# crowdbotp/socialways

Hardware: AMD Instinct MI355X
Metric: GAN train steps/sec (256 scenes x 8 agents x 8+12 T per GPU step; fp32; social block on) (higher is better)
Workload: dtype f32; 1 GPU; m1: 256 scenes x 8 agents x (8 obs + 12 pred) per GPU step = reference --batch-size 2048; use_social=True, n_unrolling_steps=1, info loss on; full=False, global_batch_scenes=256, parallelism=dp1, steps_per_graph_launch=32, settle_steps=992, rehearsal_regions=2, step_alg_bytes=5527040, inputs=z drawn on the host every step

## Files before the change

### include/socialways_hip.h

```cpp
#ifndef SOCIALWAYS_HIP_H
#define SOCIALWAYS_HIP_H
#include <stddef.h>
#include <stdint.h>

#ifdef __cplusplus
extern "C" {
#endif

#define SW_OK 0
#define SW_EARG -1
#define SW_ESHAPE -2
#define SW_EHIP -3

#define SW_H 64
#define SW_Z 32

enum { SW_GRP_ENC = 0, SW_GRP_EMB = 1, SW_GRP_ATT = 2, SW_GRP_DEC = 3, SW_GRP_DISC = 4 };

enum {
  SW_WS_GSAVE = 0,
  SW_WS_GDELTA = 1,
  SW_WS_DSAVE = 2,
  SW_WS_DDELTA = 3,
  SW_WS_WGRAD = 4,
// ... 33 lines not shown
                       const int* big_blocks , int NB, float* wh_ws, float* ml , void* stream);
int sw_social_pool_fwd_aux(const float* obsv, int To, const float* h, const int* scene_off, int S, int B, int Amax,
                           const float* emb_w, const float* att_w, float* S_out, float* attn, const int* big_blocks,
                           int NB, float* wh_ws, float* ml, const float* aux_src, float* aux_dst, long long aux_n,
                           void* stream);
int sw_social_features(const float* x4_last , int B, float* feat , void* stream);
int sw_embed_features(const float* feat , long long R, const float* emb_w, float* out ,
                      void* stream);
int sw_attention_pool_dense(const float* f , const float* h , const int* scene_off,
                            int S, int B, const float* att_w, float* S_out , void* stream);
int sw_rows_gemm(const float* x, int ldx, const float* w, int w_rs, int w_cs, const float* bias, long long R, int K, int N,
                 float* y, int ldy, int accumulate, void* stream);
int sw_linear_wgrad(const float* delta, int ldd, const float* act, int lda, int R, int N, int K, float* dW, int ldw,
                    float* db, float* wgrad_ws, int accumulate, void* stream);
int sw_embed_features_bwd(const float* feat , long long R, const float* emb_w, const float* dout ,
                          float* rows, float* dfeat, void* stream);
int sw_attention_dense_fwd(const float* f, const float* h, const float* wh, const int* scene_off, int S, int B, float* attn,
                           float* S_out, void* stream);
int sw_attention_dense_bwd(const float* f, const float* h, const float* wh, const float* attn, const float* dS,
                           const int* scene_off, int S, int B, float* dsig, float* df, float* dwh, float* dh, void* stream);
int sw_enc_lstm_wgrad(const float* enc_w, const float* act, const float* x4s, const float* h0, const float* dgates, int B,
                      int T, float* d_enc_w, float* wgrad_ws, float* tmp, void* stream);
int sw_dec_fc_wgrad(const float* dec_w, const float* gsave, const float* gdelta, const float* h, const float* s,
                    const float* z, int B, int To, float* d_dec_w, float* wgrad_ws, float* tmp, void* stream);

int sw_dec_fc_dz(const float* dec_w, const float* gdelta, int B, int To, float* dz, void* stream);

typedef struct sw_wgrad_batch sw_wgrad_batch;
sw_wgrad_batch* sw_wgrad_batch_new(void);
void sw_wgrad_batch_free(sw_wgrad_batch* h);

int sw_social_pool_bwd(const float* obsv, int To, const float* h, const int* scene_off,
                       const long long* pair_off, int S, int B, int Amax, long long P,
                       const float* emb_w, const float* att_w, const float* attn, const float* dS,
                       float* dh, float* d_emb_w, float* d_att_w, float* pair_ws, float* wgrad_ws,
                       const int* big_blocks , int NB, const float* wh_ws, const float* ml,
                       const float* S_pool, float* big_part_ws,
                       sw_wgrad_batch* defer ,
                       void* stream);

int sw_dec_rollout_fwd(const float* obsv , int To, const float* z ,
                       const float* S_pool , const float* hT, const float* cT,
                       const float* enc_w, const float* dec_w, int B, int Tp,
                       float* pred4 , float* h_end, float* c_end ,
                       float* gsave ,
                       const float* gt , float inv_ss, float* ade_part ,
                       void* stream);
int sw_dec_rollout_fwd_aux(const float* obsv, int To, const float* z, const float* S_pool, const float* hT,
                           const float* cT, const float* enc_w, const float* dec_w, int B, int Tp, float* pred4,
                           float* h_end, float* c_end, float* gsave, const float* gt, float inv_ss, float* ade_part,
                           const float* d_w , float* dsave , void* stream);
int sw_dec_sample_fwd(const float* obsv , int To, const float* z ,
                      const float* S_pool , const float* hT, const float* cT ,
                      const float* enc_w, const float* dec_w, int B, int K, int Tp, float* pred4, const float* gt ,
                      float inv_ss, float* err, void* stream);
int sw_sample_reduce(const float* err , int B, int K, float* per_agent , int* best ,
                     void* stream);
int sw_sample_rank(const float* score , const float* err , const int* best ,
                   int B, int K, int M, int* order , float* per_agent , void* stream);
int sw_scene_clearance(const float* pos, int pstride, const float* start , int sstride, const int* scene_off,
                       int S, int B, int K, int Tp, float inv_ss, float* clear , void* stream);
int sw_scene_reduce(const float* err , const float* clear , const int* scene_off, int S, int B,
                    int K, float coll_dist, float* per_scene , int* best , void* stream);
int sw_sample_nms(const float* pos, int pstride, const float* score , const int* scene_off , int S,
                  int B, int K, int Tp, int M, int metric, float inv_ss, float radius, const float* err ,
                  const int* best , int* order , int* count , float* weight ,
                  int* assign , float* per_row , void* stream);
int sw_dec_rollout_bwd(const float* dpred4 , const float* enc_w, const float* dec_w,
                       const float* gsave, int B, int To, int Tp, float* gdelta,
                       float* dhT, float* dcT, float* dS_pool , void* stream);
int sw_dec_rollout_bwd_aux(const float* dpred4, const float* enc_w, const float* dec_w, const float* gsave, int B,
                           int To, int Tp, float* gdelta, float* dhT, float* dcT, float* dS_pool,
                           const float* aux_src, float* aux_dst, const float* aux_mask, long long aux_n, void* stream);
int sw_gen_wgrad(const float* enc_w, const float* dec_w, const float* gsave, const float* gdelta, const float* z,
                 const float* S_pool, int B, int To, int Tp, float* d_enc_w, float* d_dec_w, int part,
                 float* wgrad_ws, float* tmp ,
                 sw_wgrad_batch* pending ,
                 void* stream);
int sw_gen_wgrad_adam(const float* enc_w, const float* dec_w, const float* gsave, const float* gdelta,
                      const float* z, const float* S_pool, int B, int To, int Tp, float* d_enc_w, float* d_dec_w,
                      float* wgrad_ws, float* tmp , sw_wgrad_batch* pending , float* adam_w,
                      float* adam_m, float* adam_v, const float* adam_g, long long adam_n, const float* adam_step,
                      double lr, double beta1, double beta2, double eps, void* stream);

int sw_disc_fwd(const float* obsv, int To, int x_mode, const float* const* pred4 ,
                int nb, const float* d_w, int B, int Tp, float* const* label ,
                float* const* code , float* dsave ,
                int save_lstm ,
                float* w_snapshot ,
                void* stream);
int sw_disc_bwd(const float* d_w, const float* dsave, const float* const* dlabel,
                const float* const* dcode, int nb, int B, int To, int Tp, float* ddelta,
                float* d_d_w, float* const* dpred4, float* wgrad_ws, void* stream);

int sw_disc_bwd_gan(const float* d_w, const float* dsave, const float* const* label,
                    const float* const* code, const float* targets, int t0, int t1, const float* z ,
                    float g_label, float g_code, int nb, int B, int To, int Tp, float* ddelta,
                    float* d_d_w, float* const* dpred4, float* wgrad_ws,
                    float* loss_part ,
                    void* stream);
int sw_disc_bwd_gan_adam(const float* d_w, const float* dsave, const float* const* label, const float* const* code,
                         const float* targets, int t0, int t1, const float* z, float g_label, float g_code, int nb,
                         int B, int To, int Tp, float* ddelta, float* d_d_w, float* const* dpred4, float* wgrad_ws,
                         float* loss_part, float* adam_w, float* adam_m, float* adam_v, const float* adam_step,
                         double lr, double beta1, double beta2, double eps, void* stream);

int sw_disc_update_supported(const float* d_w, int B, int To, int Tp);
int sw_disc_update(const float* obsv , int To, const float* const* pred4 , const float* d_w, int B,
                   int Tp, float* const* label, float* const* code, float* dsave, int obs_pre, float* w_snapshot ,
                   const float* targets, int t0, int t1, const float* z, float g_label, float g_code, float* ddelta,
                   float* d_d_w, float* wgrad_ws, float* loss_part , float* adam_w , float* adam_m,
                   float* adam_v, const float* adam_step, double lr, double beta1, double beta2, double eps, void* stream);

int sw_disc_dpred_supported(int Tp);
int sw_disc_dpred(const float* obsv, int To, int x_mode, const float* pred4 , const float* d_w, int B, int Tp,
                  const float* targets, int t_idx, const float* z , float g_label, float g_code,
                  float* dpred4 , float* label , float* code ,
                  float* loss_part , void* stream);

int sw_disc_score(const float* obsv, int To, int x_mode, const float* pred4 , const float* d_w, int B, int K,
                  int Tp, float* score , float* code , void* stream);

int sw_disc_score_ragged(const float* obsv, int To, int x_mode, const int* obs_len ,
                         const float* pred4 , const float* d_w, int B, int K, int Tp, float* score ,
                         float* code , void* stream);

int sw_disc_fwd_ragged(const float* obsv, int To, int x_mode, const int* obs_len ,
                       const float* const* pred4 , int nb, const float* d_w, int B, int Tp,
                       float* const* label , float* const* code , float* dsave ,
                       int save_lstm , float* w_snapshot , void* stream);
int sw_disc_dpred_ragged(const float* obsv, int To, int x_mode, const int* obs_len ,
                         const float* pred4 , const float* d_w, int B, int Tp, const float* targets, int t_idx,
                         const float* z , float g_label, float g_code, float* dpred4 ,
                         float* label , float* code , float* loss_part ,
                         void* stream);

#define SW_RED_BLOCKS 64
int sw_gan_loss(const float* label_a, const float* targets , int ia,
                const float* code_a, const float* z , const float* label_b, int ib, int B,
                float g_label, float g_code, float* out_sums , float* dlabel_a, float* dcode_a,
                float* dlabel_b, float* dcode_b, float* scratch , void* stream);

int sw_l2_grad(const float* pred4_hat , const float* gt , int B, int Tp, int row0, int row1,
               float scale, float* dpred4 , void* stream);

int sw_variety_grad(const float* pred4_hat_K , const float* gt , int K, int B, int Tp,
                    float scale, float* dpred4_K , int* kmin, float* l2min, void* stream);

int sw_traj_dist(const float* a , const float* b , int Na, int Nb, int nPed, int T,
                 int t0, float* D , void* stream);

#define SW_STAGE_HEADER 8
int sw_stage_step(const float* slot, int B, int To, int Tp, float* obsv_dst , float* pred_dst ,
                  float* pred4_dst , float* targets_dst , float* z_dst ,
                  float* steps_dst , int n_d_updates, void* stream);

int sw_gen_image_floats(void);
int sw_gen_images(const float* enc_w, const float* dec_w, const float* emb_w , const float* att_w ,
                  float* img, void* stream);
int sw_stage_step_img(const float* slot, int B, int To, int Tp, float* obsv_dst, float* pred_dst, float* pred4_dst,
                      float* targets_dst, float* z_dst, float* steps_dst, int n_d_updates, const float* enc_w,
                      const float* dec_w, const float* emb_w , const float* att_w , float* img,
                      const float* d_w , float* d_img , const int* d_tab , void* stream);
int sw_stage_step_zdev(const float* slot, int B, int To, int Tp, float* obsv_dst, float* pred_dst, float* pred4_dst,
                       float* targets_dst, float* z_dst, float* steps_dst, int n_d_updates, const float* enc_w,
                       const float* dec_w, const float* emb_w, const float* att_w, float* img, const float* d_w, float* d_img,
// ... 95 lines not shown
```

### socialways_amd/_lib.py

```python
import ctypes
import os

import torch

_HERE = os.path.dirname(os.path.abspath(__file__))
LIB_PATH = os.environ.get("SW_LIB_PATH") or os.path.join(_HERE, "libsocialways_hip.so")

GRP_ENC, GRP_EMB, GRP_ATT, GRP_DEC, GRP_DISC = 0, 1, 2, 3, 4
WS_GSAVE, WS_GDELTA, WS_DSAVE, WS_DDELTA, WS_WGRAD, WS_PAIRS = 0, 1, 2, 3, 4, 5
AMAX = 64
RED_BLOCKS = 64

_vp, _i, _f, _ll = ctypes.c_void_p, ctypes.c_int, ctypes.c_float, ctypes.c_longlong

PROTOTYPES = {
    "sw_version": (_i, []),
    "sw_last_error": (ctypes.c_char_p, []),
    "sw_param_count": (_i, [_i, _i]),
    "sw_param_offset": (_i, [_i, _i, _i]),
    "sw_param_tensors": (_i, [_i]),
    "sw_workspace_floats": (ctypes.c_size_t, [_i, _i, _i, _i, _i, _ll]),
    "sw_traj_4d": (_i, [_vp, _vp, _i, _i, _i, _vp, _vp, _vp]),
    "sw_enc_lstm_fwd": (_i, [_vp, _i, _vp, _vp, _vp, _i, _i, _vp, _vp, _vp, _vp, _vp, _i, _vp]),
    "sw_enc_lstm_fwd_aux": (_i, [_vp, _i, _vp, _vp, _vp, _i, _i, _vp, _vp, _vp, _vp, _vp, _i, _vp, _vp, _ll, _vp]),
    "sw_enc_lstm_fwd_ragged": (_i, [_vp, _i, _vp, _vp, _i, _i, _vp, _vp, _vp]),
    "sw_enc_lstm_fwd_ragged_save": (_i, [_vp, _i, _vp, _vp, _i, _i, _vp, _vp, _vp, _vp, _vp]),
    "sw_enc_lstm_bwd": (_i, [_vp, _vp, _vp, _vp, _vp, _vp, _i, _i, _i, _vp, _vp, _vp, _vp]),
    "sw_social_pool_fwd": (_i, [_vp, _i, _vp, _vp, _i, _i, _i, _vp, _vp, _vp, _vp, _vp, _i, _vp, _vp, _vp]),
    "sw_social_pool_fwd_aux": (_i, [_vp, _i, _vp, _vp, _i, _i, _i, _vp, _vp, _vp, _vp, _vp, _i, _vp, _vp, _vp, _vp, _ll, _vp]),
    "sw_social_features": (_i, [_vp, _i, _vp, _vp]),
    "sw_embed_features": (_i, [_vp, _ll, _vp, _vp, _vp]),
    "sw_attention_pool_dense": (_i, [_vp, _vp, _vp, _i, _i, _vp, _vp, _vp]),
    "sw_social_pool_bwd": (_i, [_vp, _i, _vp, _vp, _vp, _i, _i, _i, _ll, _vp, _vp, _vp, _vp, _vp, _vp, _vp,
                                _vp, _vp, _vp, _i, _vp, _vp, _vp, _vp, _vp, _vp]),
    "sw_dec_rollout_fwd": (_i, [_vp, _i, _vp, _vp, _vp, _vp, _vp, _vp, _i, _i, _vp, _vp, _vp, _vp, _vp, _f, _vp, _vp]),
    "sw_dec_rollout_fwd_aux": (_i, [_vp, _i, _vp, _vp, _vp, _vp, _vp, _vp, _i, _i, _vp, _vp, _vp, _vp, _vp, _f, _vp, _vp, _vp, _vp]),
    "sw_dec_sample_fwd": (_i, [_vp, _i, _vp, _vp, _vp, _vp, _vp, _vp, _i, _i, _i, _vp, _vp, _f, _vp, _vp]),
    "sw_sample_reduce": (_i, [_vp, _i, _i, _vp, _vp, _vp]),
    "sw_sample_rank": (_i, [_vp, _vp, _vp, _i, _i, _i, _vp, _vp, _vp]),
    "sw_scene_clearance": (_i, [_vp, _i, _vp, _i, _vp, _i, _i, _i, _i, _f, _vp, _vp]),
    "sw_scene_reduce": (_i, [_vp, _vp, _vp, _i, _i, _i, _f, _vp, _vp, _vp]),
    "sw_sample_nms": (_i, [_vp, _i, _vp, _vp, _i, _i, _i, _i, _i, _i, _f, _f, _vp, _vp, _vp, _vp, _vp, _vp, _vp, _vp]),
    "sw_dec_rollout_bwd": (_i, [_vp, _vp, _vp, _vp, _i, _i, _i, _vp, _vp, _vp, _vp, _vp]),
    "sw_dec_rollout_bwd_aux": (_i, [_vp, _vp, _vp, _vp, _i, _i, _i, _vp, _vp, _vp, _vp, _vp, _vp, _vp, _ll, _vp]),
    "sw_gen_wgrad": (_i, [_vp, _vp, _vp, _vp, _vp, _vp, _i, _i, _i, _vp, _vp, _i, _vp, _vp, _vp, _vp]),
    "sw_gen_wgrad_adam": (_i, [_vp, _vp, _vp, _vp, _vp, _vp, _i, _i, _i, _vp, _vp, _vp, _vp, _vp, _vp, _vp, _vp, _vp,
                               ctypes.c_longlong, _vp, ctypes.c_double, ctypes.c_double, ctypes.c_double, ctypes.c_double, _vp]),
    "sw_enc_lstm_bwd_aux": (_i, [_vp, _vp, _vp, _vp, _vp, _vp, _i, _i, _i, _vp, _vp, _vp, _vp, _vp, _vp, _ll, _vp]),
    "sw_dec_rollout_bwd_dfuse": (_i, [_vp, _vp, _vp, _vp, _i, _vp, _f, _f, _vp, _vp, _vp, _vp, _vp, _i, _i, _i, _vp, _vp, _vp, _vp,
                                      _vp]),
    "sw_rows_gemm": (_i, [_vp, _i, _vp, _i, _i, _vp, ctypes.c_longlong, _i, _i, _vp, _i, _i, _vp]),
    "sw_linear_wgrad": (_i, [_vp, _i, _vp, _i, _i, _i, _i, _vp, _i, _vp, _vp, _i, _vp]),
    "sw_embed_features_bwd": (_i, [_vp, ctypes.c_longlong, _vp, _vp, _vp, _vp, _vp]),
    "sw_attention_dense_fwd": (_i, [_vp, _vp, _vp, _vp, _i, _i, _vp, _vp, _vp]),
    "sw_attention_dense_bwd": (_i, [_vp, _vp, _vp, _vp, _vp, _vp, _i, _i, _vp, _vp, _vp, _vp, _vp]),
    "sw_enc_lstm_wgrad": (_i, [_vp, _vp, _vp, _vp, _vp, _i, _i, _vp, _vp, _vp, _vp]),
    "sw_dec_fc_dz": (_i, [_vp, _vp, _i, _i, _vp, _vp]),
    "sw_dec_fc_wgrad": (_i, [_vp, _vp, _vp, _vp, _vp, _vp, _i, _i, _vp, _vp, _vp, _vp]),
    "sw_wgrad_batch_new": (_vp, []),
    "sw_wgrad_batch_free": (None, [_vp]),
    "sw_disc_fwd": (_i, [_vp, _i, _i, _vp, _i, _vp, _i, _i, _vp, _vp, _vp, _i, _vp, _vp]),
    "sw_disc_bwd": (_i, [_vp, _vp, _vp, _vp, _i, _i, _i, _i, _vp, _vp, _vp, _vp, _vp]),
    "sw_disc_bwd_gan": (_i, [_vp, _vp, _vp, _vp, _vp, _i, _i, _vp, _f, _f, _i, _i, _i, _i, _vp, _vp, _vp, _vp, _vp, _vp]),
    "sw_disc_bwd_gan_adam": (_i, [_vp, _vp, _vp, _vp, _vp, _i, _i, _vp, _f, _f, _i, _i, _i, _i, _vp, _vp, _vp, _vp, _vp,
                                  _vp, _vp, _vp, _vp, ctypes.c_double, ctypes.c_double, ctypes.c_double, ctypes.c_double, _vp]),
    "sw_disc_update_supported": (_i, [_vp, _i, _i, _i]),
    "sw_disc_dpred_supported": (_i, [_i]),
    "sw_disc_update": (_i, [_vp, _i, _vp, _vp, _i, _i, _vp, _vp, _vp, _i, _vp, _vp, _i, _i, _vp, _f, _f, _vp, _vp, _vp, _vp,
                            _vp, _vp, _vp, _vp, ctypes.c_double, ctypes.c_double, ctypes.c_double, ctypes.c_double, _vp]),
    "sw_disc_dpred": (_i, [_vp, _i, _i, _vp, _vp, _i, _i, _vp, _i, _vp, _f, _f, _vp, _vp, _vp, _vp, _vp]),
    "sw_disc_score": (_i, [_vp, _i, _i, _vp, _vp, _i, _i, _i, _vp, _vp, _vp]),
    "sw_disc_score_ragged": (_i, [_vp, _i, _i, _vp, _vp, _vp, _i, _i, _i, _vp, _vp, _vp]),
    "sw_disc_fwd_ragged": (_i, [_vp, _i, _i, _vp, _vp, _i, _vp, _i, _i, _vp, _vp, _vp, _i, _vp, _vp]),
    "sw_disc_dpred_ragged": (_i, [_vp, _i, _i, _vp, _vp, _vp, _i, _i, _vp, _i, _vp, _f, _f, _vp, _vp, _vp, _vp, _vp]),
    "sw_gan_loss": (_i, [_vp, _vp, _i, _vp, _vp, _vp, _i, _i, _f, _f, _vp, _vp, _vp, _vp, _vp, _vp, _vp]),
    "sw_l2_grad": (_i, [_vp, _vp, _i, _i, _i, _i, _f, _vp, _vp]),
    "sw_variety_grad": (_i, [_vp, _vp, _i, _i, _i, _f, _vp, _vp, _vp, _vp]),
    "sw_traj_dist": (_i, [_vp, _vp, _i, _i, _i, _i, _i, _vp, _vp]),
    "sw_stage_step": (_i, [_vp, _i, _i, _i, _vp, _vp, _vp, _vp, _vp, _vp, _i, _vp]),
    "sw_gen_image_floats": (_i, []),
    "sw_gen_images": (_i, [_vp, _vp, _vp, _vp, _vp, _vp]),
    "sw_stage_step_img": (_i, [_vp, _i, _i, _i, _vp, _vp, _vp, _vp, _vp, _vp, _i, _vp, _vp, _vp, _vp, _vp, _vp, _vp, _vp, _vp]),
    "sw_stage_step_zdev": (_i, [_vp, _i, _i, _i, _vp, _vp, _vp, _vp, _vp, _vp, _i, _vp, _vp, _vp, _vp, _vp, _vp, _vp, _vp, _i, _vp]),
    "sw_disc_image_floats": (_i, [_i]),
    "sw_disc_image_table": (_i, [_i, _vp]),
    "sw_disc_images": (_i, [_vp, _vp, _vp, _i, _vp]),
    "sw_ade_fde": (_i, [_vp, _vp, _i, _i, _f, _vp, _vp, _vp]),
    "sw_lstm_point_fwd": (_i, [_vp, _vp, _i, _i, _vp, _vp, _vp, _vp]),
    "sw_lstm_point_bwd": (_i, [_vp, _vp, _vp, _vp, _vp, _i, _i, _vp, _vp, _vp]),
    "sw_act_fwd": (_i, [_vp, _ll, _i, _vp, _vp]),
    "sw_act_bwd": (_i, [_vp, _vp, _ll, _i, _vp, _vp]),
    "sw_sqdiff": (_i, [_vp, _i, _vp, _i, _vp, _i, _ll, _i, _f, _vp, _vp, _i, _vp]),
    "sw_pair_features": (_i, [_vp, _vp, _vp, _i, _vp, _vp]),
    "sw_attn_pairs_fwd": (_i, [_vp, _vp, _vp, _vp, _vp, _i, _i, _i, _i, _vp, _vp, _vp]),
    "sw_attn_pairs_bwd": (_i, [_vp, _vp, _vp, _vp, _vp, _vp, _vp, _i, _i, _i, _i, _vp, _vp, _vp, _vp, _vp]),
    "sw_adam_packed": (_i, [_vp, _vp, _vp, _vp, _ll, _vp, ctypes.c_double, ctypes.c_double, ctypes.c_double,
                            ctypes.c_double, _i, _vp]),
    "sw_wide_gemm": (_i, [_vp, _ll, _i, _vp, _ll, _i, _vp, _vp, _i, _vp, _i, _ll, _i, _i, _vp, _i, _i, _vp]),
    "sw_wide_lstm_fwd": (_i, [_vp, _i, _vp, _i, _vp, _vp, _vp, _vp, _vp, _i, _i, _vp, _vp, _vp, _i, _vp, _i, _vp]),
    "sw_wide_lstm_bwd": (_i, [_vp, _i, _vp, _i, _vp, _vp, _vp, _vp, _vp, _vp, _i, _i, _vp, _vp, _vp]),
    "sw_wide_out_fwd": (_i, [_vp, _i, _vp, _vp, _vp, _i, _vp, _i, _vp, _vp]),
    "sw_wide_out_bwd": (_i, [_vp, _i, _vp, _vp, _i, _vp, _i, _vp, _vp, _i, _vp, _vp]),
    "sw_wide_sum_steps": (_i, [_vp, _ll, _i, _i, _ll, _i, _vp, _i, _vp]),
    "sw_wide_wgrad": (_i, [_vp, _i, _vp, _vp]),
    "sw_wide_transpose": (_i, [_vp, _vp, _i, _i, _vp, _vp]),
    "sw_wide_dec_loop_supported": (_i, [_i]),
    "sw_wide_dec_loop_fwd": (_i, [_vp] * 13 + [_i] + [_vp] * 9 + [_i, _i, _i, _i, _vp]),
    "sw_wide_dec_loop_bwd": (_i, [_vp] * 18 + [_i, _i, _i, _i, _vp]),
    "sw_wide_disc_heads_supported": (_i, [_i, _i, _i]),
    "sw_wide_disc_heads_fwd": (_i, [_vp, _vp]),
    "sw_wide_disc_heads_bwd": (_i, [_vp, _vp]),
    "sw_wide_opimage": (_i, [_vp, _vp, _i, _ll, _vp, _vp]),
    "sw_wide_lstm_seq_supported": (_i, [_i]),
    "sw_wide_lstm_seq_fwd": (_i, [_vp, _vp, _vp, _vp, _vp, _i, _i, _i, _vp, _vp, _vp, _vp, _i, _vp]),
    "sw_wide_lstm_seq_bwd": (_i, [_vp, _i, _vp, _i, _vp, _vp, _vp, _vp, _vp, _i, _i, _i, _vp, _vp]),
    "sw_comm_bytes": (_ll, [_i, _ll]),
    "sw_comm_alloc": (_i, [_ll, _vp]),
    "sw_comm_free": (_i, [_vp]),
    "sw_comm_ipc_export": (_i, [_vp, _vp]),
    "sw_comm_ipc_import": (_i, [_vp, _vp]),
    "sw_comm_ipc_close": (_i, [_vp]),
    "sw_comm_status": (_i, [_vp, _vp]),
    "sw_allreduce_direct": (_i, [_vp, _i, _i, _ll, _vp, _ll, _vp]),
    "sw_allreduce_direct_adam": (_i, [_vp, _i, _i, _ll, _vp, _ll, _vp, _vp, _vp, _vp, ctypes.c_double, ctypes.c_double,
                                      ctypes.c_double, ctypes.c_double, _i, _vp]),
    "sw_noise_uniform": (_i, [ctypes.c_ulonglong, _i, ctypes.c_uint, _i, ctypes.c_uint, _i, ctypes.c_uint, _i, _i, _i, _vp, _vp]),
}

DEBUG_PROTOTYPES = {
    "sw_kernel_timing": (_i, [_i]),
# ... 81 lines not shown
```

### socialways_amd/csrc/sw_lstm.hip

```cpp
#include "../../include/socialways_hip.h"
#include "sw_lstm_dev.h"
#include <cstdlib>

template <int XMODE, bool ACT, bool Y, bool X4S>
__global__ __launch_bounds__(SW_THREADS) void enc_lstm_fwd_kernel(
    const float* __restrict__ x, const float* __restrict__ enc_w, const float* __restrict__ h0,
    const float* __restrict__ c0, int B, int T, float* __restrict__ hT, float* __restrict__ cT,
    float* __restrict__ y, float* __restrict__ act, float* __restrict__ x4s, int t0, const float* __restrict__ aux_src,
    float* __restrict__ aux_dst, long long aux_n, const float* __restrict__ gimg) {
  const int tiles = (B + SW_TILE - 1) / SW_TILE;
  const int extra = (int)gridDim.x - tiles;
  if ((int)blockIdx.x < extra) {
    const long long n4 = aux_n >> 2, stride = (long long)extra * SW_THREADS;
    long long i = (long long)blockIdx.x * SW_THREADS + threadIdx.x;
    for (; i + 3 * stride < n4; i += 4 * stride) {
      const f32x4 v0 = ld4(aux_src + 4 * i), v1 = ld4(aux_src + 4 * (i + stride));
      const f32x4 v2 = ld4(aux_src + 4 * (i + 2 * stride)), v3 = ld4(aux_src + 4 * (i + 3 * stride));
      st4(aux_dst + 4 * i, v0);
      st4(aux_dst + 4 * (i + stride), v1);
      st4(aux_dst + 4 * (i + 2 * stride), v2);
      st4(aux_dst + 4 * (i + 3 * stride), v3);
    }
    for (; i < n4; i += stride) st4(aux_dst + 4 * i, ld4(aux_src + 4 * i));
    return;
  }
  constexpr int HS = ACT ? SW_ALD : SW_HLD, HO = ACT ? 320 : 0;
  __shared__ __attribute__((aligned(16))) float hbuf[2][SW_TILE * HS];
  __shared__ __attribute__((aligned(16))) float wx_lds[256 * 4];
  __shared__ __attribute__((aligned(16))) float bx_lds[256];
  const int lane = sw_lane(), wave = sw_wave(), ln = lane & 15, lg = lane >> 4;
  const int u0 = wave * 16;
  const int a0 = ((int)blockIdx.x - extra) * SW_TILE;
  const int b = min(a0 + ln, B - 1);
  LstmW W;
  if (gimg) {
    lstm_load_img(W, gimg, wave, lane);
  } else {
    lstm_load_whh(W, enc_w + swp::ENC_WHH, u0, ln, lg);
    lstm_prep_rows(enc_w + swp::ENC_EMB_W, enc_w + swp::ENC_EMB_B, enc_w + swp::ENC_WIH, enc_w + swp::ENC_BIH,
                   enc_w + swp::ENC_BHH, true, wx_lds, bx_lds);
  }
  f32x4 c = {0.f, 0.f, 0.f, 0.f}, h = {0.f, 0.f, 0.f, 0.f};
  if (h0) h = ld4(h0 + (size_t)b * 64 + u0 + 4 * lg);
  if (c0) c = ld4(c0 + (size_t)b * 64 + u0 + 4 * lg);
  st4(&hbuf[0][ln * HS + HO + u0 + 4 * lg], h);
  sw_barrier();
  if (!gimg) lstm_load_wx(W, wx_lds, bx_lds, u0, ln, lg);

  float xa, xq = 0.f;
  auto load_x = [&](int t) {
    if constexpr (XMODE == 0) obs_x4_load(x, b, t, T, lg, xa, xq);
    else xa = x[((size_t)b * T + t) * 4 + lg];
  };
  load_x(0);
  asm volatile("" : "+v"(xa), "+v"(xq));
  float* yrow = Y ? y + (size_t)b * T * 64 + u0 + 4 * lg : nullptr;
  float* xrow = X4S ? x4s + ((size_t)t0 * B + b) * 4 + lg : nullptr;
  auto step = [&](int t, auto hp) {
    const float xb = XMODE == 0 ? xa - (lg >= 2 ? xq : 0.f) : xa;
    load_x(min(t + 1, T - 1));
    f32x4 gate[4];
    lstm_cell<decltype(hp)::value>(W, xb, &hbuf[t & 1][ln * HS + HO + 4 * lg], gate, c, h);
    if constexpr (ACT) lstm_put_act_tile(hbuf[(t + 1) & 1], gate, c, h, ln, lg, u0);
    else st4(&hbuf[(t + 1) & 1][ln * HS + u0 + 4 * lg], h);
    if constexpr (Y) {
      st4(yrow, h);
      yrow += 64;
    }
    if constexpr (X4S) {
      *xrow = xb;
      xrow += (size_t)B * 4;
    }
    sw_barrier();
    if constexpr (ACT) lstm_store_act_tile(hbuf[(t + 1) & 1], act + (size_t)(t0 + t) * B * 384, a0, B, wave, lane);
    asm volatile("" : "+v"(xa), "+v"(xq));
  };
  if (h0) step(0, std::true_type{});
  else step(0, std::false_type{});
  for (int t = 1; t < T; ++t) step(t, std::true_type{});
  st4(hT + (size_t)b * 64 + u0 + 4 * lg, h);
  st4(cT + (size_t)b * 64 + u0 + 4 * lg, c);
}

__global__ __launch_bounds__(512) void enc_lstm_fwd8_kernel(
    const float* __restrict__ x, const float* __restrict__ h0, const float* __restrict__ c0, int B, int T,
    float* __restrict__ hT, float* __restrict__ cT, float* __restrict__ act, float* __restrict__ x4s, int t0,
    const float* __restrict__ aux_src, float* __restrict__ aux_dst, long long aux_n, const float* __restrict__ gimg) {
  const int tiles = (B + SW_TILE - 1) / SW_TILE;
  const int extra = (int)gridDim.x - tiles;
  if ((int)blockIdx.x < extra) {
    const long long n4 = aux_n >> 2, stride = (long long)extra * 512;
    long long i = (long long)blockIdx.x * 512 + threadIdx.x;
    for (; i + stride < n4; i += 2 * stride) {
      const f32x4 v0 = ld4(aux_src + 4 * i), v1 = ld4(aux_src + 4 * (i + stride));
      st4(aux_dst + 4 * i, v0);
      st4(aux_dst + 4 * (i + stride), v1);
    }
    for (; i < n4; i += stride) st4(aux_dst + 4 * i, ld4(aux_src + 4 * i));
    return;
  }
  __shared__ __attribute__((aligned(16))) float hbuf[2][SW_TILE * SW_ALD];
  const int lane = sw_lane(), wave = sw_wave(), ln = lane & 15, lg = lane >> 4;
  const int ub = 8 * wave + 2 * lg;
  const int a0 = ((int)blockIdx.x - extra) * SW_TILE;
  const int b = min(a0 + ln, B - 1);
  f32x4 whh[2][4], bias[2];
  float wx[2];
#pragma unroll
  for (int tl = 0; tl < 2; ++tl) {
#pragma unroll
    for (int j = 0; j < 4; ++j) whh[tl][j] = ld4(gimg + swimg::OP_WHH8 + ((((size_t)wave * 2 + tl) * 4 + j) * 64 + lane) * 4);
    const int rowA = (2 * tl + ((ln & 3) >> 1)) * 64 + 8 * wave + 2 * (ln >> 2) + (ln & 1);
    wx[tl] = gimg[swimg::WX + rowA * 4 + lg];
#pragma unroll
    for (int r = 0; r < 4; ++r) bias[tl][r] = gimg[swimg::BX + (2 * tl + (r >> 1)) * 64 + ub + (r & 1)];
  }
  float2 c = {0.f, 0.f}, h = {0.f, 0.f};
  if (h0) h = *reinterpret_cast<const float2*>(h0 + (size_t)b * 64 + ub);
  if (c0) c = *reinterpret_cast<const float2*>(c0 + (size_t)b * 64 + ub);
  *reinterpret_cast<float2*>(&hbuf[0][ln * SW_ALD + 320 + ub]) = h;
  sw_barrier();
  float xa, xq = 0.f;
  obs_x4_load(x, b, 0, T, lg, xa, xq);
  asm volatile("" : "+v"(xa), "+v"(xq));
  float* xrow = x4s + ((size_t)t0 * B + b) * 4 + lg;
  auto step = [&](int t, auto hp) {
    const float xb = xa - (lg >= 2 ? xq : 0.f);
    obs_x4_load(x, b, min(t + 1, T - 1), T, lg, xa, xq);
    f32x4 acc0 = SW_MFMA(wx[0], xb, bias[0]), acc1 = SW_MFMA(wx[1], xb, bias[1]);
    if constexpr (decltype(hp)::value) {
      const float* hrow = &hbuf[t & 1][ln * SW_ALD + 320 + 4 * lg];
      f32x4 bq[4];
#pragma unroll
      for (int j = 0; j < 4; ++j) bq[j] = ld4(hrow + 16 * j);
#pragma unroll
      for (int j = 0; j < 4; ++j)
#pragma unroll
        for (int r = 0; r < 4; ++r) {
          acc0 = SW_MFMA(whh[0][j][r], bq[j][r], acc0);
          acc1 = SW_MFMA(whh[1][j][r], bq[j][r], acc1);
        }
    }
    float2 gi, gf, gg, go;
#pragma unroll
    for (int e = 0; e < 2; ++e) {
      const float i_ = sw_sigmoid(acc0[e]), f_ = sw_sigmoid(acc0[2 + e]), g_ = sw_tanh(acc1[e]), o_ = sw_sigmoid(acc1[2 + e]);
      const float cp = e ? c.y : c.x;
      const float cn = fmaf(f_, cp, i_ * g_);
      const float hn = o_ * sw_tanh(cn);
      if (e) { gi.y = i_; gf.y = f_; gg.y = g_; go.y = o_; c.y = cn; h.y = hn; }
      else   { gi.x = i_; gf.x = f_; gg.x = g_; go.x = o_; c.x = cn; h.x = hn; }
    }
    float* row = &hbuf[(t + 1) & 1][ln * SW_ALD + ub];
    *reinterpret_cast<float2*>(row) = gi;
    *reinterpret_cast<float2*>(row + 64) = gf;
    *reinterpret_cast<float2*>(row + 128) = gg;
    *reinterpret_cast<float2*>(row + 192) = go;
    *reinterpret_cast<float2*>(row + 256) = c;
    *reinterpret_cast<float2*>(row + 320) = h;
    *xrow = xb;
    xrow += (size_t)B * 4;
    sw_barrier();
    {
      float* rows_t = act + (size_t)(t0 + t) * B * 384;
#pragma unroll
      for (int k = 0; k < 3; ++k) {
        const int f = k * 512 + (int)threadIdx.x, a = f / 96, c4 = f - a * 96;
        const f32x4 v = ld4(&hbuf[(t + 1) & 1][a * SW_ALD + 4 * c4]);
        st4g(rows_t + (size_t)min(a0 + a, B - 1) * 384 + 4 * c4, v);
      }
    }
    asm volatile("" : "+v"(xa), "+v"(xq));
  };
  if (h0) step(0, std::true_type{});
  else step(0, std::false_type{});
  for (int t = 1; t < T; ++t) step(t, std::true_type{});
  *reinterpret_cast<float2*>(hT + (size_t)b * 64 + ub) = h;
  *reinterpret_cast<float2*>(cT + (size_t)b * 64 + ub) = c;
}

template <bool DY>
__global__ __launch_bounds__(SW_THREADS) void enc_lstm_bwd_kernel(
    const float* __restrict__ whh, const float* __restrict__ act, const float* __restrict__ c0,
    const float* __restrict__ dhT, const float* __restrict__ dcT, const float* __restrict__ dy, int B, int T,
    int t0, float* __restrict__ dgates, float* __restrict__ dh0, float* __restrict__ dc0, const float* __restrict__ gimg,
    const float* __restrict__ aux_src, float* __restrict__ aux_dst, const float* __restrict__ aux_mask, long long aux_n) {
  if (sw_aux_masked_copy(B, aux_src, aux_dst, aux_mask, aux_n)) return;
  __shared__ __attribute__((aligned(16))) float dgbuf[2][SW_TILE * SW_GLD];
  const int lane = sw_lane(), wave = sw_wave(), ln = lane & 15, lg = lane >> 4;
  const int u0 = wave * 16;
  const int a0 = blockIdx.x * SW_TILE;
  const int b = min(a0 + ln, B - 1);
  LstmWT W;
  lstm_load_whhT(W, gimg, swimg::OP_WHHT, whh, wave, lane);
  const float* act_b = act + ((size_t)t0 * B + b) * 384 + u0 + 4 * lg;
  f32x4 dh = ld4(dhT ? dhT + (size_t)b * 64 + u0 + 4 * lg : act_b);
  f32x4 dc = ld4(dcT ? dcT + (size_t)b * 64 + u0 + 4 * lg : act_b);
  if (!dhT) dh = f32x4{0.f, 0.f, 0.f, 0.f};
  if (!dcT) dc = f32x4{0.f, 0.f, 0.f, 0.f};
  const float* cstart = t0 > 0 ? act_b - (size_t)B * 384 + 256 : c0 ? c0 + (size_t)b * 64 + u0 + 4 * lg : nullptr;
  const LstmBptt S{act_b, cstart, dgbuf[0], dgates + ((size_t)t0 * B + a0) * 256, nullptr, a0, B};
  const float* dyp = DY ? dy + ((size_t)b * T + T - 1) * 64 + u0 + 4 * lg : nullptr;
  lstm_bptt_rows<true>(W, S, T, dh, dc, [&](f32x4& d) {
    if constexpr (DY) {
      d += ld4(dyp);
      dyp -= 64;
    }
  });
  if (dh0) st4(dh0 + (size_t)b * 64 + u0 + 4 * lg, dh);
  if (dc0) st4(dc0 + (size_t)b * 64 + u0 + 4 * lg, dc);
}

__global__ void traj4d_kernel(const float* __restrict__ obsv, const float* __restrict__ pred, int B, int To,
                              int Tp, float* __restrict__ o4, float* __restrict__ p4) {
  int i = blockIdx.x * blockDim.x + threadIdx.x;
  int n_o = B * To, n_p = pred ? B * Tp : 0;
  if (i < n_o) {
    int b = i / To, t = i - b * To;
    f32x4 v;
    v[0] = obs_x4(obsv, b, t, To, 0);
    v[1] = obs_x4(obsv, b, t, To, 1);
    v[2] = obs_x4(obsv, b, t, To, 2);
    v[3] = obs_x4(obsv, b, t, To, 3);
    st4(o4 + (size_t)i * 4, v);
  } else if (i < n_o + n_p) {
    int k = i - n_o, b = k / Tp, t = k - b * Tp;
    const float* p = pred + ((size_t)b * Tp + t) * 2;
    const float* q = t == 0 ? obsv + ((size_t)b * To + To - 1) * 2 : p - 2;
    f32x4 v = {p[0], p[1], p[0] - q[0], p[1] - q[1]};
    st4(p4 + (size_t)k * 4, v);
  }
}

extern "C" int sw_traj_4d(const float* obsv, const float* pred, int B, int To, int Tp, float* obsv4,
                          float* pred4, void* stream) {
  if (!obsv || !obsv4 || B < 0 || To < 2 || (pred && (!pred4 || Tp < 1))) return SW_EARG;
  if (B == 0) return SW_OK;
  int n = B * To + (pred ? B * Tp : 0);
  SW_LAUNCH(traj4d_kernel, dim3((n + 255) / 256), dim3(256), 0, (hipStream_t)stream, obsv, pred, B,
                     To, Tp, obsv4, pred4);
  SW_CHECK_LAUNCH("traj4d_kernel");
  return SW_OK;
}

extern "C" int sw_enc_lstm_fwd_aux(const float* x, int x_mode, const float* enc_w, const float* h0,
                                   const float* c0, int B, int T, float* hT, float* cT, float* y, float* act,
                                   float* x4s, int t0, const float* aux_src, float* aux_dst, long long aux_n,
                                   void* stream) {
  if (!x || !enc_w || !hT || !cT || B < 0 || T < 1 || t0 < 0 || (x_mode != 0 && x_mode != 1)) return SW_EARG;
  if (aux_n < 0 || (aux_n & 3) || (aux_n > 0 && (!aux_src || !aux_dst))) return SW_EARG;
  if (x_mode == 0 && T < 2) return SW_ESHAPE;
  if (B == 0) return SW_OK;
  const float* gimg = sw_gen_images_for(enc_w, nullptr);
  const int tiles = (B + SW_TILE - 1) / SW_TILE;
  int extra = aux_n > 0 ? (int)((aux_n / 4 + SW_THREADS - 1) / SW_THREADS) : 0;
  if (extra > 64) extra = 64;
  static const int enc8_env = getenv("SW_ENC8") ? atoi(getenv("SW_ENC8")) : -1;
  const bool enc8 = enc8_env >= 0 ? enc8_env != 0 : tiles <= 256;
  if (enc8 && gimg && x_mode == 0 && act && x4s && !y) {
    SW_LAUNCH(enc_lstm_fwd8_kernel, dim3(tiles + extra), dim3(512), 0, (hipStream_t)stream, x, h0, c0, B, T, hT, cT, act, x4s, t0,
              aux_src, aux_dst, aux_n, gimg);
    SW_CHECK_LAUNCH("enc_lstm_fwd8_kernel");
    return SW_OK;
  }
#define SW_ENC_FWD(XM, A, Y_, X4)                                                                                   \
  SW_LAUNCH((enc_lstm_fwd_kernel<XM, A, Y_, X4>), dim3(tiles + extra), dim3(SW_THREADS), 0, (hipStream_t)stream,    \
            x, enc_w, h0, c0, B, T, hT, cT, y, act, x4s, t0, aux_src, aux_dst, aux_n, gimg)
  switch ((x_mode ? 8 : 0) | (act ? 4 : 0) | (y ? 2 : 0) | (x4s ? 1 : 0)) {
    case 0: SW_ENC_FWD(0, false, false, false); break;
    case 1: SW_ENC_FWD(0, false, false, true); break;
    case 2: SW_ENC_FWD(0, false, true, false); break;
    case 3: SW_ENC_FWD(0, false, true, true); break;
    case 4: SW_ENC_FWD(0, true, false, false); break;
    case 5: SW_ENC_FWD(0, true, false, true); break;
    case 6: SW_ENC_FWD(0, true, true, false); break;
    case 7: SW_ENC_FWD(0, true, true, true); break;
    case 8: SW_ENC_FWD(1, false, false, false); break;
    case 9: SW_ENC_FWD(1, false, false, true); break;
    case 10: SW_ENC_FWD(1, false, true, false); break;
    case 11: SW_ENC_FWD(1, false, true, true); break;
    case 12: SW_ENC_FWD(1, true, false, false); break;
    case 13: SW_ENC_FWD(1, true, false, true); break;
    case 14: SW_ENC_FWD(1, true, true, false); break;
    default: SW_ENC_FWD(1, true, true, true); break;
  }
#undef SW_ENC_FWD
  SW_CHECK_LAUNCH("enc_lstm_fwd_kernel");
  return SW_OK;
}
extern "C" int sw_enc_lstm_fwd(const float* x, int x_mode, const float* enc_w, const float* h0,
                               const float* c0, int B, int T, float* hT, float* cT, float* y, float* act,
                               float* x4s, int t0, void* stream) {
  return sw_enc_lstm_fwd_aux(x, x_mode, enc_w, h0, c0, B, T, hT, cT, y, act, x4s, t0, nullptr, nullptr, 0, stream);
}

template <int XMODE>
__global__ __launch_bounds__(SW_THREADS) void enc_lstm_fwd_ragged_kernel(
    const float* __restrict__ x, const float* __restrict__ enc_w, const int* __restrict__ obs_len, int B, int T,
    float* __restrict__ hT, float* __restrict__ cT, const float* __restrict__ gimg) {
  __shared__ __attribute__((aligned(16))) float hbuf[2 * SW_TILE * SW_HLD];
  __shared__ __attribute__((aligned(16))) float wx_lds[256 * 4];
  __shared__ __attribute__((aligned(16))) float bx_lds[256];
  const int lane = sw_lane(), wave = sw_wave(), ln = lane & 15, lg = lane >> 4;
  const int u0 = wave * 16;
  const int b = min((int)blockIdx.x * SW_TILE + ln, B - 1);
  LstmW W;
  if (gimg) {
    lstm_load_img(W, gimg, wave, lane);
  } else {
    lstm_load_whh(W, enc_w + swp::ENC_WHH, u0, ln, lg);
    lstm_prep_rows(enc_w + swp::ENC_EMB_W, enc_w + swp::ENC_EMB_B, enc_w + swp::ENC_WIH, enc_w + swp::ENC_BIH,
                   enc_w + swp::ENC_BHH, true, wx_lds, bx_lds);
  }
  const int s = obs_start(obs_len, b, T, XMODE);
  f32x4 c = {0.f, 0.f, 0.f, 0.f}, h = {0.f, 0.f, 0.f, 0.f};
  st4(&hbuf[ln * SW_HLD + u0 + 4 * lg], h);
  sw_barrier();
  if (!gimg) lstm_load_wx(W, wx_lds, bx_lds, u0, ln, lg);
  lstm_obs_loop_ragged<XMODE>(W, hbuf, x, T, b, s, c, h);
  st4(hT + (size_t)b * 64 + u0 + 4 * lg, h);
  st4(cT + (size_t)b * 64 + u0 + 4 * lg, c);
}

extern "C" int sw_enc_lstm_fwd_ragged(const float* x, int x_mode, const float* enc_w, const int* obs_len, int B, int T,
                                      float* hT, float* cT, void* stream) {
  if (!x || !enc_w || !hT || !cT || B < 0 || T < 1 || (x_mode != 0 && x_mode != 1) || (x_mode == 0 && T < 2)) return SW_EARG;
  if (B == 0) return SW_OK;
  const float* gimg = sw_gen_images_for(enc_w, nullptr);
  const int tiles = (B + SW_TILE - 1) / SW_TILE;
  if (x_mode == 0)
    SW_LAUNCH(enc_lstm_fwd_ragged_kernel<0>, dim3(tiles), dim3(SW_THREADS), 0, (hipStream_t)stream, x, enc_w, obs_len, B, T, hT, cT,
              gimg);
  else
    SW_LAUNCH(enc_lstm_fwd_ragged_kernel<1>, dim3(tiles), dim3(SW_THREADS), 0, (hipStream_t)stream, x, enc_w, obs_len, B, T, hT, cT,
              gimg);
  SW_CHECK_LAUNCH("enc_lstm_fwd_ragged_kernel");
  return SW_OK;
}

template <int XMODE>
__global__ __launch_bounds__(SW_THREADS) void enc_lstm_fwd_ragged_save_kernel(
    const float* __restrict__ x, const float* __restrict__ enc_w, const int* __restrict__ obs_len, int B, int T,
    float* __restrict__ hT, float* __restrict__ cT, float* __restrict__ act, float* __restrict__ x4s,
    const float* __restrict__ gimg) {
  __shared__ __attribute__((aligned(16))) float hbuf[2 * SW_TILE * SW_ALD];
  __shared__ __attribute__((aligned(16))) float wx_lds[256 * 4];
  __shared__ __attribute__((aligned(16))) float bx_lds[256];
  const int lane = sw_lane(), wave = sw_wave(), ln = lane & 15, lg = lane >> 4;
  const int u0 = wave * 16;
  const int a0 = (int)blockIdx.x * SW_TILE;
  const int b = min(a0 + ln, B - 1);
  LstmW W;
  if (gimg) {
    lstm_load_img(W, gimg, wave, lane);
  } else {
    lstm_load_whh(W, enc_w + swp::ENC_WHH, u0, ln, lg);
    lstm_prep_rows(enc_w + swp::ENC_EMB_W, enc_w + swp::ENC_EMB_B, enc_w + swp::ENC_WIH, enc_w + swp::ENC_BIH,
                   enc_w + swp::ENC_BHH, true, wx_lds, bx_lds);
  }
  const int s = obs_start(obs_len, b, T, XMODE);
  f32x4 c = {0.f, 0.f, 0.f, 0.f}, h = {0.f, 0.f, 0.f, 0.f};
  st4(&hbuf[ln * SW_ALD + 320 + u0 + 4 * lg], h);
  sw_barrier();
  if (!gimg) lstm_load_wx(W, wx_lds, bx_lds, u0, ln, lg);
  lstm_obs_loop_ragged<XMODE, SAVE_TILE>(W, hbuf, x, T, b, s, c, h, act, x4s, B, a0);
  st4(hT + (size_t)b * 64 + u0 + 4 * lg, h);
  st4(cT + (size_t)b * 64 + u0 + 4 * lg, c);
}

extern "C" int sw_enc_lstm_fwd_ragged_save(const float* x, int x_mode, const float* enc_w, const int* obs_len, int B, int T,
                                           float* hT, float* cT, float* act, float* x4s, void* stream) {
  if (!x || !enc_w || !hT || !cT || !act || !x4s || B < 0 || T < 1 || (x_mode != 0 && x_mode != 1) || (x_mode == 0 && T < 2))
// ... 40 lines not shown
```

### socialways_amd/csrc/sw_lstm_dev.h

```cpp
#pragma once
#include <type_traits>
#include "sw_common.h"

#define SW_HLD 68
#define SW_GLD 260

struct LstmW {
  f32x4 whh[4][4];
  float wx[4];
  f32x4 bias[4];
};

__device__ __forceinline__ void lstm_prep_rows(const float* We, const float* be, const float* Wih,
                                               const float* bih, const float* bhh, bool composed,
                                               float* wx_lds, float* bx_lds) {
  int row = threadIdx.x;
  if (composed) {
    f32x4 w[16];
    const float* wr = Wih + (size_t)row * 64;
#pragma unroll
    for (int e = 0; e < 16; ++e) w[e] = ld4(wr + 4 * e);
    float a0 = 0.f, a1 = 0.f, a2 = 0.f, a3 = 0.f, ab = 0.f;
#pragma unroll
    for (int e = 0; e < 16; ++e) {
// ... 313 lines not shown
}

__device__ __forceinline__ int obs_start(const int* __restrict__ obs_len, int b, int T, int xmode) {
  const int n = obs_len ? min(max(obs_len[b], xmode == 0 ? 2 : 1), T) : T;
  return T - n;
}
__device__ __forceinline__ void obs_x4_load_from(const float* pos, int b, int t, int s, int T, int comp, float& a, float& q) {
  const float* p = pos + (size_t)b * T * 2;
  const int c = comp & 1, te = max(t, s), tt = te == s ? s + 1 : te;
  const bool vel = comp >= 2;
  a = p[(vel ? tt : te) * 2 + c];
  q = p[(vel ? tt - 1 : te) * 2 + c];
}
enum { SAVE_NONE = 0, SAVE_ROWS = 1, SAVE_TILE = 2 };
template <int XMODE, int SAVE = SAVE_NONE>
__device__ __forceinline__ void lstm_obs_loop_ragged(const LstmW& W, float* hbuf, const float* __restrict__ x, int T, int b, int s,
                                                     f32x4& c, f32x4& h, float* __restrict__ act = nullptr,
                                                     float* __restrict__ x4s = nullptr, int B = 0, int a0 = 0) {
  const int lane = sw_lane(), wave = sw_wave(), ln = lane & 15, lg = lane >> 4;
  const int u0 = wave * 16;
  constexpr int HS = SAVE == SAVE_TILE ? SW_ALD : SW_HLD, HO = SAVE == SAVE_TILE ? 320 : 0;
  float xa, xq = 0.f;
  auto load_x = [&](int t) {
    if constexpr (XMODE == 0) obs_x4_load_from(x, b, t, s, T, lg, xa, xq);
    else xa = x[((size_t)b * T + max(t, s)) * 4 + lg];
  };
  load_x(0);
  asm volatile("" : "+v"(xa), "+v"(xq));
  float* arow = SAVE == SAVE_ROWS ? act + (size_t)b * 384 + u0 + 4 * lg : nullptr;
  float* xrow = SAVE != SAVE_NONE ? x4s + (size_t)b * 4 + lg : nullptr;
  for (int t = 0; t < T; ++t) {
    const float xb = XMODE == 0 ? xa - (lg >= 2 ? xq : 0.f) : xa;
    load_x(min(t + 1, T - 1));
    f32x4 gate[4];
    lstm_cell(W, xb, &hbuf[(t & 1) * 16 * HS + ln * HS + HO + 4 * lg], gate, c, h);
    const bool on = t >= s;
#pragma unroll
    for (int r = 0; r < 4; ++r) {
      c[r] = on ? c[r] : 0.f;
      h[r] = on ? h[r] : 0.f;
    }
    if constexpr (SAVE != SAVE_NONE) {
#pragma unroll
      for (int g = 0; g < 4; ++g)
#pragma unroll
        for (int r = 0; r < 4; ++r) gate[g][r] = on ? gate[g][r] : 0.f;
      *xrow = on ? xb : 0.f;
      xrow += (size_t)B * 4;
    }
    if constexpr (SAVE == SAVE_TILE) lstm_put_act_tile(hbuf + ((t + 1) & 1) * 16 * HS, gate, c, h, ln, lg, u0);
    else st4(&hbuf[((t + 1) & 1) * 16 * HS + ln * HS + u0 + 4 * lg], h);
    if constexpr (SAVE == SAVE_ROWS) {
#pragma unroll
      for (int g = 0; g < 4; ++g) st4g(arow + g * 64, gate[g]);
      st4g(arow + 256, c);
      st4g(arow + 320, h);
      arow += (size_t)B * 384;
    }
    sw_barrier();
    if constexpr (SAVE == SAVE_TILE) lstm_store_act_tile(hbuf + ((t + 1) & 1) * 16 * HS, act + (size_t)t * B * 384, a0, B, wave, lane);
    asm volatile("" : "+v"(xa), "+v"(xq));
  }
}

__device__ __forceinline__ void disc_obs_lstm_tile(float* smem, const float* __restrict__ obsv, int To, int x_mode,
                                                   const float* wih, const float* whh, const float* bih, const float* bhh,
                                                   int B, int a0, float* __restrict__ act, float* __restrict__ x4s) {
  float* hbuf = smem;
  float* wx_lds = smem + 2 * 16 * SW_HLD;
  float* bx_lds = wx_lds + 1024;
  const int lane = sw_lane(), wave = sw_wave(), ln = lane & 15, lg = lane >> 4;
  const int u0 = wave * 16;
  const int b = min(a0 + ln, B - 1);
  LstmW W;
  lstm_load_whh(W, whh, u0, ln, lg);
  lstm_prep_rows(nullptr, nullptr, wih, bih, bhh, false, wx_lds, bx_lds);
  f32x4 c = {0.f, 0.f, 0.f, 0.f}, h = {0.f, 0.f, 0.f, 0.f};
  st4(&hbuf[ln * SW_HLD + u0 + 4 * lg], h);
  sw_barrier();
  lstm_load_wx(W, wx_lds, bx_lds, u0, ln, lg);
  if (x_mode == 0) lstm_obs_loop<0, true>(W, hbuf, obsv, To, B, b, c, h, act, x4s);
  else lstm_obs_loop<1, true>(W, hbuf, obsv, To, B, b, c, h, act, x4s);
}
```

### socialways_amd/csrc/sw_misc.hip

```cpp
#include "../../include/socialways_hip.h"
#include "sw_common.h"
#include "sw_lstm_dev.h"
#include <stdlib.h>
#include "sw_wgrad.h"
#include <stdio.h>
#include <string.h>

static thread_local char g_err[256] = "";
void sw_set_error(const char* what, hipError_t e) {
  snprintf(g_err, sizeof(g_err), "%s: %s", what, hipGetErrorString(e));
}
extern "C" const char* sw_last_error(void) { return g_err; }

int sw_set_lds(const void* fn, int bytes, int& have) {
  if (have >= bytes) return SW_OK;
  hipError_t e = hipFuncSetAttribute(fn, hipFuncAttributeMaxDynamicSharedMemorySize, bytes);
  if (e != hipSuccess) {
    sw_set_error("hipFuncSetAttribute(MaxDynamicSharedMemorySize)", e);
    return SW_EHIP;
  }
  have = bytes;
  return SW_OK;
}

// ... 102 lines not shown
    const DiscImages di = sw_disc_images_for(w, disc_Tp);
    ad.img = const_cast<float*>(di.img);
    ad.tab = di.tab;
  }
  int blocks = (int)((n + 255) / 256);
  if (blocks > 512) blocks = 512;
  SW_LAUNCH(adam_packed_kernel, dim3(blocks), dim3(256), 0, (hipStream_t)stream, ad, n);
  SW_CHECK_LAUNCH("adam_packed_kernel");
  return SW_OK;
}
extern "C" int sw_version(void) { return 3; }

size_t sw_dsave_floats(int B, int To, int Tp, int nb);
size_t sw_ddelta_floats(int B, int To, int Tp, int nb);

static int group_offsets(int grp, int Tp, int* off, int* count) {
  using namespace swp;
  switch (grp) {
    case SW_GRP_ENC: {
      const int o[] = {ENC_EMB_W, ENC_EMB_B, ENC_WIH, ENC_WHH, ENC_BIH, ENC_BHH};
      memcpy(off, o, sizeof(o));
      *count = ENC_N;
      return 6;
    }
    case SW_GRP_EMB: {
      const int o[] = {EMB_W0, EMB_B0, EMB_W1, EMB_B1, EMB_W2, EMB_B2};
      memcpy(off, o, sizeof(o));
      *count = EMB_N;
      return 6;
    }
    case SW_GRP_ATT: {
      const int o[] = {ATT_W, ATT_B};
      memcpy(off, o, sizeof(o));
      *count = ATT_N;
      return 2;
    }
    case SW_GRP_DEC: {
      const int o[] = {DEC_W1, DEC_B1, DEC_W2, DEC_B2, DEC_W3, DEC_B3, DEC_W4, DEC_B4};
      memcpy(off, o, sizeof(o));
      *count = DEC_N;
      return 8;
    }
    case SW_GRP_DISC: {
      if (Tp < 1) return -1;
      Disc d = disc(Tp);
      const int o[] = {d.wih,  d.whh,  d.bih,  d.bhh,  d.of0w, d.of0b, d.of1w, d.of1b, d.pe0w, d.pe0b,
                       d.pe1w, d.pe1b, d.cl0w, d.cl0b, d.cl1w, d.cl1b, d.la0w, d.la0b, d.la1w, d.la1b};
      memcpy(off, o, sizeof(o));
      *count = d.n;
      return 20;
    }
  }
  return -1;
}
extern "C" int sw_param_tensors(int grp) {
  int off[32], n;
  return group_offsets(grp, 1, off, &n);
}
extern "C" int sw_param_count(int grp, int Tp) {
  int off[32], n = -1;
  if (group_offsets(grp, Tp, off, &n) < 0) return SW_EARG;
  return n;
}
extern "C" int sw_param_offset(int grp, int idx, int Tp) {
  int off[32], n;
  int k = group_offsets(grp, Tp, off, &n);
  if (k < 0 || idx < 0 || idx >= k) return SW_EARG;
  return off[idx];
}

extern "C" size_t sw_workspace_floats(int ws_id, int B, int To, int Tp, int nb, long long P) {
  if (B < 0 || To < 1 || Tp < 1) return 0;
  switch (ws_id) {
    case SW_WS_GSAVE: return gsave_layout(B, To, Tp).total;
    case SW_WS_GDELTA: return gdelta_layout(B, To, Tp).total;
    case SW_WS_DSAVE: return sw_dsave_floats(B, To, Tp, nb < 1 ? 1 : nb);
    case SW_WS_DDELTA: return sw_ddelta_floats(B, To, Tp, nb < 1 ? 1 : nb);
    case SW_WS_WGRAD: return SW_WG_WS_FLOATS;
    case SW_WS_PAIRS: return (size_t)B * 200 + (size_t)(P < 0 ? 0 : P) * 196;
  }
  return 0;
}

#define SW_DEC_COMPOSE_BLOCKS 13
__device__ __forceinline__ void compose_bwd_block(const int blk, const float* __restrict__ enc_w,
                                                  const float* __restrict__ dWx, const float* __restrict__ dbx,
                                                  float* __restrict__ d_enc_w, const float* __restrict__ dec_w,
                                                  const float* __restrict__ Ms, float* __restrict__ d_dec_w,
                                                  const WgAdam& ad, const float* __restrict__ snap) {
  using namespace swp;
  float bc1 = 1.f, bc2s = 1.f;
  if (ad.w) wg_adam_bc(ad, bc1, bc2s);
  auto put = [&](float* dst, float g) {
    *dst = g;
    if (ad.w) wg_adam1(ad, bc1, bc2s, dst, g);
  };
  if (blk >= 128) {
    const int o = (blk - 128) * 256 + threadIdx.x;
    const float* M = Ms;
    const float* sv = Ms + 160;
    const float* W3 = snap ? snap + swimg::RAW_W3 : dec_w + DEC_W3;
    const float* W4 = snap ? snap + swimg::RAW_W4 : dec_w + DEC_W4;
    const float* b3 = snap ? snap + swimg::RAW_B3 : dec_w + DEC_B3;
    if (o < 3200) {
      const int m = o / 80, k = o - m * 80;
      put(d_dec_w + DEC_W3 + o, fmaf(W4[m], M[k], W4[40 + m] * M[80 + k]));
    } else if (o < 3240) {
      const int m = o - 3200;
      put(d_dec_w + DEC_B3 + m, fmaf(W4[m], sv[0], W4[40 + m] * sv[1]));
    } else if (o < 3320) {
      const int c = (o - 3240) / 40, m = (o - 3240) - c * 40;
      float v = sv[c] * b3[m];
      for (int k = 0; k < 80; ++k) v = fmaf(M[c * 80 + k], W3[m * 80 + k], v);
      put(d_dec_w + DEC_W4 + c * 40 + m, v);
    } else if (o < 3322) {
      put(d_dec_w + DEC_B4 + (o - 3320), sv[o - 3320]);
    }
    return;
  }
  const float* We = snap ? snap + swimg::RAW_WE : enc_w + ENC_EMB_W;
  const float* be = snap ? snap + swimg::RAW_BE : enc_w + ENC_EMB_B;
  const float* Wih = snap ? snap + swimg::RAW_WIH : enc_w + ENC_WIH;
  const int t = threadIdx.x;
  if (blk < 64) {
    int i = blk * 256 + t;
    int row = i >> 6, e = i & 63;
    f32x4 g = ld4(dWx + row * 4), w = ld4(We + e * 4);
    float v = dbx[row] * be[e];
    v = fmaf(g[0], w[0], v); v = fmaf(g[1], w[1], v); v = fmaf(g[2], w[2], v); v = fmaf(g[3], w[3], v);
    put(d_enc_w + ENC_WIH + i, v);
    if (blk == 0) {
      put(d_enc_w + ENC_BIH + t, dbx[t]);
      put(d_enc_w + ENC_BHH + t, dbx[t]);
    }
    return;
  }
  __shared__ float red[5][256];
  const int e = blk - 64;
  float w = Wih[t * 64 + e];
  f32x4 g = ld4(dWx + t * 4);
  red[0][t] = w * g[0]; red[1][t] = w * g[1]; red[2][t] = w * g[2]; red[3][t] = w * g[3]; red[4][t] = w * dbx[t];
  __syncthreads();
  for (int o = 128; o > 0; o >>= 1) {
    if (t < o) {
#pragma unroll
      for (int c = 0; c < 5; ++c) red[c][t] += red[c][t + o];
    }
    __syncthreads();
  }
  if (t < 4) put(d_enc_w + ENC_EMB_W + e * 4 + t, red[t][0]);
  if (t == 4) put(d_enc_w + ENC_EMB_B + e, red[4][0]);
}

__global__ __launch_bounds__(256) void enc_compose_bwd_kernel(const float* __restrict__ enc_w,
                                                              const float* __restrict__ dWx,
                                                              const float* __restrict__ dbx,
                                                              float* __restrict__ d_enc_w,
                                                              const float* __restrict__ dec_w,
                                                              const float* __restrict__ Ms,
                                                              float* __restrict__ d_dec_w, WgAdam ad,
                                                              const float* __restrict__ snap) {
  compose_bwd_block((int)blockIdx.x, enc_w, dWx, dbx, d_enc_w, dec_w, Ms, d_dec_w, ad, snap);
}
__global__ __launch_bounds__(256) void compose_bwd_part_kernel(const float* __restrict__ enc_w, const float* __restrict__ dWx,
                                                               const float* __restrict__ dbx, float* __restrict__ d_enc_w,
                                                               const float* __restrict__ dec_w, const float* __restrict__ Ms,
                                                               float* __restrict__ d_dec_w, int block0) {
  compose_bwd_block((int)blockIdx.x + block0, enc_w, dWx, dbx, d_enc_w, dec_w, Ms, d_dec_w, WgAdam(), nullptr);
}

static int gen_wgrad_impl(const float* enc_w, const float* dec_w, const float* gsave, const float* gdelta, const float* z,
                          const float* S_pool, int B, int To, int Tp, float* d_enc_w, float* d_dec_w, int part,
                          float* wgrad_ws, float* tmp, sw_wgrad_batch* pending, void* stream, WgAdam ad,
                          const float* snap) {
  if (!enc_w || !dec_w || !gsave || !gdelta || !z || !S_pool || !d_enc_w || !d_dec_w || !wgrad_ws || !tmp || B < 1 || To < 2 ||
      Tp < 1 || part < 0 || part > 2)
    return SW_EARG;
  using namespace swp;
  const GSave gs = gsave_layout(B, To, Tp);
  const GDelta gd = gdelta_layout(B, To, Tp);
  const int Ta = To + Tp - 1;
  float* dWx = tmp;
  float* dbx = tmp + 1024;
  float* dM = tmp + 1280;
  hipStream_t st = (hipStream_t)stream;
  WgBatch wb;
  if (pending) {
    wb = *wg_pending(pending);
    *wg_pending(pending) = WgBatch();
  }
  int rc_add = 0;
  const int t_lo = part == 1 ? To : 0, t_hi = part == 2 ? To : Ta;
  const int acc = part == 2 ? 1 : 0;
  if (t_hi > t_lo)
    rc_add |= wg_add_tail(wb, gdelta + gd.dgates + (size_t)t_lo * B * 256, 256,
                          gsave + gs.act + ((ptrdiff_t)t_lo - 1) * B * 384 + 320, 384, (t_hi - t_lo) * B, 256, 64,
                          d_enc_w + ENC_WHH, 64, gsave + gs.x4s + (size_t)t_lo * B * 4, 4, 4, dWx, 4,
                          t_lo < 1 ? B : 0 , dbx, nullptr, acc);
  if (part != 2) {
    rc_add |= wg_add(wb, gdelta + gd.dz1, 160, gsave + gs.act + (size_t)(To - 1) * B * 384 + 320, 384, Tp * B, 160, 64,
                     d_dec_w + DEC_W1, 160, nullptr, nullptr, 0);
    rc_add |= wg_add(wb, gdelta + gd.du, 160, S_pool, 64, B, 160, 64, d_dec_w + DEC_W1 + 64, 160, nullptr, nullptr, 0);
    rc_add |= wg_add(wb, gdelta + gd.du, 160, z, 32, B, 160, 32, d_dec_w + DEC_W1 + 128, 160, d_dec_w + DEC_B1, nullptr, 0);
    rc_add |= wg_add(wb, gdelta + gd.dz2, 80, gsave + gs.a1, 160, Tp * B, 80, 160, d_dec_w + DEC_W2, 160, d_dec_w + DEC_B2,
                     nullptr, 0);
    rc_add |= wg_add(wb, gdelta + gd.dv, 4, gsave + gs.a2, 80, Tp * B, 2, 80, dM, 80, dM + 160, nullptr, 0);
  }
  if (rc_add) return SW_ESHAPE;
  if (int rc = ad.w ? wg_launch_adam(wb, wgrad_ws, ad, st) : wg_launch(wb, wgrad_ws, st)) return rc;
  if (part != 1) {
    SW_LAUNCH(enc_compose_bwd_kernel, dim3(128 + SW_DEC_COMPOSE_BLOCKS), dim3(256), 0, st, enc_w, dWx, dbx, d_enc_w,
                       dec_w, dM, d_dec_w, ad, snap);
    SW_CHECK_LAUNCH("enc_compose_bwd_kernel");
  }
  return SW_OK;
}
extern "C" int sw_gen_wgrad(const float* enc_w, const float* dec_w, const float* gsave, const float* gdelta, const float* z,
                            const float* S_pool, int B, int To, int Tp, float* d_enc_w, float* d_dec_w, int part,
                            float* wgrad_ws, float* tmp, sw_wgrad_batch* pending, void* stream) {
  return gen_wgrad_impl(enc_w, dec_w, gsave, gdelta, z, S_pool, B, To, Tp, d_enc_w, d_dec_w, part, wgrad_ws, tmp, pending,
                        stream, WgAdam(), nullptr);
}
extern "C" int sw_gen_wgrad_adam(const float* enc_w, const float* dec_w, const float* gsave, const float* gdelta,
                                 const float* z, const float* S_pool, int B, int To, int Tp, float* d_enc_w, float* d_dec_w,
                                 float* wgrad_ws, float* tmp, sw_wgrad_batch* pending, float* adam_w, float* adam_m,
                                 float* adam_v, const float* adam_g, long long adam_n, const float* adam_step, double lr,
                                 double beta1, double beta2, double eps, void* stream) {
  if (!adam_w || !adam_m || !adam_v || !adam_g || !adam_step || adam_n < 1 || !enc_w || !dec_w || !d_enc_w || !d_dec_w)
    return SW_EARG;
  if (enc_w - adam_w != d_enc_w - adam_g || dec_w - adam_w != d_dec_w - adam_g || enc_w < adam_w ||
      dec_w + swp::DEC_N > adam_w + adam_n || enc_w + swp::ENC_N > adam_w + adam_n || dec_w < adam_w)
    return SW_EARG;
  const float* img = sw_gen_images_for(enc_w, dec_w);
  if (!img) return SW_EARG;
  WgAdam ad;
  ad.w = adam_w; ad.m = adam_m; ad.v = adam_v; ad.g0 = adam_g; ad.step = adam_step; ad.n = (size_t)adam_n;
  ad.lr = lr; ad.beta1 = beta1; ad.beta2 = beta2; ad.eps = eps;
  return gen_wgrad_impl(enc_w, dec_w, gsave, gdelta, z, S_pool, B, To, Tp, d_enc_w, d_dec_w, 0, wgrad_ws, tmp, pending, stream,
                        ad, img);
}

extern "C" int sw_enc_lstm_wgrad(const float* enc_w, const float* act, const float* x4s, const float* h0, const float* dgates,
                                 int B, int T, float* d_enc_w, float* wgrad_ws, float* tmp, void* stream) {
  if (!enc_w || !act || !x4s || !dgates || !d_enc_w || !wgrad_ws || !tmp || B < 1 || T < 1) return SW_EARG;
  using namespace swp;
  hipStream_t st = (hipStream_t)stream;
  float* dWx = tmp;
  float* dbx = tmp + 1024;
  WgBatch wb;
  if (wg_add_tail(wb, dgates, 256, act - (ptrdiff_t)B * 384 + 320, 384, T * B, 256, 64, d_enc_w + ENC_WHH, 64, x4s, 4, 4, dWx, 4,
                  B, dbx, nullptr, 0))
    return SW_ESHAPE;
  if (int rc = wg_launch(wb, wgrad_ws, st)) return rc;
  if (h0) {
    WgBatch w0;
    if (wg_add(w0, dgates, 256, h0, 64, B, 256, 64, d_enc_w + ENC_WHH, 64, nullptr, nullptr, 1)) return SW_ESHAPE;
    if (int rc = wg_launch(w0, wgrad_ws, st)) return rc;
  }
  SW_LAUNCH(compose_bwd_part_kernel, dim3(128), dim3(256), 0, st, enc_w, dWx, dbx, d_enc_w, nullptr, nullptr, nullptr, 0);
  SW_CHECK_LAUNCH("compose_bwd_part_kernel");
  return SW_OK;
}
extern "C" int sw_dec_fc_wgrad(const float* dec_w, const float* gsave, const float* gdelta, const float* h, const float* s,
                               const float* z, int B, int To, float* d_dec_w, float* wgrad_ws, float* tmp, void* stream) {
  if (!dec_w || !gsave || !gdelta || !h || !z || !d_dec_w || !wgrad_ws || !tmp || B < 1 || To < 2) return SW_EARG;
  using namespace swp;
  hipStream_t st = (hipStream_t)stream;
  const GSave gs = gsave_layout(B, To, 1);
  const GDelta gd = gdelta_layout(B, To, 1);
  float* dM = tmp + 1280;
  WgBatch wb;
  int rc = 0;
  rc |= wg_add(wb, gdelta + gd.dz1, 160, h, 64, B, 160, 64, d_dec_w + DEC_W1, 160, nullptr, nullptr, 0);
  if (s) rc |= wg_add(wb, gdelta + gd.dz1, 160, s, 64, B, 160, 64, d_dec_w + DEC_W1 + 64, 160, nullptr, nullptr, 0);
  rc |= wg_add(wb, gdelta + gd.dz1, 160, z, 32, B, 160, 32, d_dec_w + DEC_W1 + 128, 160, d_dec_w + DEC_B1, nullptr, 0);
  rc |= wg_add(wb, gdelta + gd.dz2, 80, gsave + gs.a1, 160, B, 80, 160, d_dec_w + DEC_W2, 160, d_dec_w + DEC_B2, nullptr, 0);
  rc |= wg_add(wb, gdelta + gd.dv, 4, gsave + gs.a2, 80, B, 2, 80, dM, 80, dM + 160, nullptr, 0);
  if (rc) return SW_ESHAPE;
  if (int r2 = wg_launch(wb, wgrad_ws, st)) return r2;
  if (!s) {
    if (hipMemset2DAsync(d_dec_w + DEC_W1 + 64, 160 * sizeof(float), 0, 64 * sizeof(float), 160, st) != hipSuccess) return SW_EHIP;
  }
  SW_LAUNCH(compose_bwd_part_kernel, dim3(SW_DEC_COMPOSE_BLOCKS), dim3(256), 0, st, nullptr, nullptr, nullptr, nullptr,
                     dec_w, dM, d_dec_w, 128);
  SW_CHECK_LAUNCH("compose_bwd_part_kernel");
  return SW_OK;
}

__device__ __forceinline__ void block_sum3(float& a, float& b, float& c, float (*red)[16]) {
#pragma unroll
  for (int o = 32; o > 0; o >>= 1) {
    a += __shfl_xor(a, o);
    b += __shfl_xor(b, o);
    c += __shfl_xor(c, o);
  }
  int w = threadIdx.x >> 6, l = threadIdx.x & 63;
  if (l == 0) { red[0][w] = a; red[1][w] = b; red[2][w] = c; }
  __syncthreads();
  if (w == 0) {
    a = l < 16 ? red[0][l] : 0.f;
    b = l < 16 ? red[1][l] : 0.f;
    c = l < 16 ? red[2][l] : 0.f;
#pragma unroll
    for (int o = 8; o > 0; o >>= 1) {
      a += __shfl_xor(a, o);
      b += __shfl_xor(b, o);
      c += __shfl_xor(c, o);
    }
  }
}

__global__ __launch_bounds__(1024) void gan_loss_kernel(
    const float* __restrict__ label_a, const float* __restrict__ targets, int ia, const float* __restrict__ code_a,
    const float* __restrict__ z, const float* __restrict__ label_b, int ib, int B, float g_label, float g_code,
    float* __restrict__ out, float* __restrict__ dlabel_a, float* __restrict__ dcode_a, float* __restrict__ dlabel_b,
    float* __restrict__ dcode_b) {
  __shared__ float red[3][16];
  const float t_a = targets[ia], t_b = targets[ib];
  float s0 = 0.f, s1 = 0.f, s2 = 0.f;
  for (int b = blockIdx.x * blockDim.x + threadIdx.x; b < B; b += gridDim.x * blockDim.x) {
    float e = label_a[b] - t_a;
    s0 = fmaf(e, e, s0);
// ... 213 lines not shown
                                                           int* __restrict__ order, float* __restrict__ per_agent) {
  extern __shared__ __attribute__((aligned(16))) float rank_s[];
  const int wave = threadIdx.x >> 6, lane = threadIdx.x & 63;
  const int a = min((int)blockIdx.x * 4 + wave, B - 1);
  const bool live = (int)blockIdx.x * 4 + wave < B;
  float* s = rank_s + wave * K;
  for (int k = lane; k < K; k += 64) s[k] = score[(size_t)k * B + a];
  __syncthreads();
  const float2* e = reinterpret_cast<const float2*>(err);
  const float inf = __builtin_inff();
  float ma = inf, mf = inf;
  int k0 = -1, rb = 0;
  const int kb = best ? best[a] : -1;
  for (int k = lane; k < K; k += 64) {
    const float v = s[k];
    int r = 0;
    for (int j = 0; j < K; ++j) {
      const float u = s[j];
      r += (u > v || (u == v && j < k)) ? 1 : 0;
    }
    if (r < M) {
      if (live) order[(size_t)a * M + r] = k;
      if (per_agent) {
        const float2 ek = e[(size_t)k * B + a];
        ma = fminf(ma, ek.x);
        mf = fminf(mf, ek.y);
      }
    }
    if (r == 0) k0 = k;
    if (k == kb) rb = r;
  }
  if (!per_agent) return;
#pragma unroll
  for (int o = 32; o > 0; o >>= 1) {
    ma = fminf(ma, __shfl_xor(ma, o));
    mf = fminf(mf, __shfl_xor(mf, o));
    k0 = max(k0, __shfl_xor(k0, o));
    rb = max(rb, __shfl_xor(rb, o));
  }
  if (lane == 0 && live) {
    const float2 e0 = e[(size_t)max(k0, 0) * B + a];
    float* p = per_agent + (size_t)a * 5;
    p[0] = e0.x; p[1] = e0.y; p[2] = ma; p[3] = mf; p[4] = (float)rb;
  }
}
extern "C" int sw_sample_rank(const float* score, const float* err, const int* best, int B, int K, int M, int* order,
                              float* per_agent, void* stream) {
  if (!score || !order || B < 0 || K < 1 || M < 1 || M > K || (per_agent && !err)) return SW_EARG;
  if (K > SW_RANK_MAXK) return SW_ESHAPE;
  if (B == 0) return SW_OK;
  SW_LAUNCH(sample_rank_kernel, dim3((B + 3) / 4), dim3(256), 4 * K * sizeof(float), (hipStream_t)stream, score, err, best, B, K,
            M, order, per_agent);
  SW_CHECK_LAUNCH("sample_rank_kernel");
  return SW_OK;
}

__global__ __launch_bounds__(256) void traj_dist_kernel(const float* __restrict__ a, const float* __restrict__ b, int Na,
                                                         int Nb, int nPed, int T, int t0, float* __restrict__ D) {
  const long long n = (long long)nPed * Na * Nb;
  for (long long e = (long long)blockIdx.x * 256 + threadIdx.x; e < n; e += (long long)gridDim.x * 256) {
    const int j = (int)(e % Nb), i = (int)((e / Nb) % Na), k = (int)(e / ((long long)Nb * Na));
    const float2* pa = reinterpret_cast<const float2*>(a) + ((size_t)i * nPed + k) * T;
    const float2* pb = reinterpret_cast<const float2*>(b) + ((size_t)j * nPed + k) * T;
    float s = 0.f;
    for (int t = t0; t < T; ++t) {
      float2 x = pa[t], y = pb[t];
      float dx = x.x - y.x, dy = x.y - y.y;
      s += sqrtf(dx * dx + dy * dy);
    }
    D[e] = s / (float)(T - t0);
  }
}
extern "C" int sw_traj_dist(const float* a, const float* b, int Na, int Nb, int nPed, int T, int t0, float* D,
                            void* stream) {
  if (!a || !b || !D || Na < 1 || Nb < 1 || nPed < 1 || T < 1 || t0 < 0 || t0 >= T) return SW_EARG;
  long long n = (long long)nPed * Na * Nb;
  int blocks = (int)((n + 255) / 256);
  if (blocks > 2048) blocks = 2048;
  SW_LAUNCH(traj_dist_kernel, dim3(blocks), dim3(256), 0, (hipStream_t)stream, a, b, Na, Nb, nPed, T, t0, D);
  SW_CHECK_LAUNCH("traj_dist_kernel");
  return SW_OK;
}

#define SW_IMG_BLOCKS 64
__device__ __forceinline__ void gen_images_block(const float* __restrict__ enc_w, const float* __restrict__ dec_w,
                                                 const float* __restrict__ emb_w, const float* __restrict__ att_w,
                                                 float* __restrict__ img, int blk) {
  using namespace swp;
  if (blk == 0) {
    lstm_prep_rows(enc_w + ENC_EMB_W, enc_w + ENC_EMB_B, enc_w + ENC_WIH, enc_w + ENC_BIH, enc_w + ENC_BHH, true,
                   img + swimg::WX, img + swimg::BX);
    return;
  }
  if (blk == 1) {
    const int t = threadIdx.x;
    if (t < 160) {
      const int c = t / 80, k = t - c * 80;
      const float* w4 = dec_w + DEC_W4 + c * 40;
      float v0 = 0.f, v1 = 0.f, v2 = 0.f, v3 = 0.f;
#pragma unroll
      for (int m = 0; m < 40; m += 4) {
        v0 = fmaf(w4[m], dec_w[DEC_W3 + m * 80 + k], v0);
        v1 = fmaf(w4[m + 1], dec_w[DEC_W3 + (m + 1) * 80 + k], v1);
        v2 = fmaf(w4[m + 2], dec_w[DEC_W3 + (m + 2) * 80 + k], v2);
        v3 = fmaf(w4[m + 3], dec_w[DEC_W3 + (m + 3) * 80 + k], v3);
      }
      img[swimg::W43 + c * 80 + k] = (v0 + v1) + (v2 + v3);
    } else if (t < 162) {
      const int c = t - 160;
      float v = dec_w[DEC_B4 + c];
#pragma unroll
      for (int m = 0; m < 40; m += 4) {
        const f32x4 w = ld4(dec_w + DEC_W4 + c * 40 + m), bb = ld4(dec_w + DEC_B3 + m);
        v = fmaf(w[0], bb[0], fmaf(w[1], bb[1], fmaf(w[2], bb[2], fmaf(w[3], bb[3], v))));
      }
      img[swimg::W43 + 160 + c] = v;
    }
    return;
  }
  const int nth = (SW_IMG_BLOCKS - 2) * 256, tid = (blk - 2) * 256 + threadIdx.x;
  for (int i = tid; i < (swimg::RAW_END - swimg::RAW_WIH) / 4; i += nth) {
    const int o = swimg::RAW_WIH + 4 * i;
    const float* src = o < swimg::RAW_WE   ? enc_w + ENC_WIH + (o - swimg::RAW_WIH)
                       : o < swimg::RAW_BE ? enc_w + ENC_EMB_W + (o - swimg::RAW_WE)
                       : o < swimg::RAW_W3 ? enc_w + ENC_EMB_B + (o - swimg::RAW_BE)
                       : o < swimg::RAW_B3 ? dec_w + DEC_W3 + (o - swimg::RAW_W3)
                       : o < swimg::RAW_W4 ? dec_w + DEC_B3 + (o - swimg::RAW_B3)
                                           : dec_w + DEC_W4 + (o - swimg::RAW_W4);
    st4(img + o, ld4(src));
  }
  auto op_image = [&](int dst0, const float* W, int ldw, int c0, int KJ, int ntile) {
    for (int f = tid; f < ntile * KJ * 64; f += nth) {
      const int t = f / (KJ * 64), rem = f - t * (KJ * 64), j = rem >> 6, l = rem & 63;
      st4(img + dst0 + 4 * (size_t)f, ld4(W + (size_t)(16 * t + (l & 15)) * ldw + c0 + 16 * j + 4 * (l >> 4)));
    }
  };
  auto op_image_T = [&](int dst0, const float* W, int ldw, int KJ, int ntile) {
    for (int f = tid; f < ntile * KJ * 64; f += nth) {
      const int t = f / (KJ * 64), rem = f - t * (KJ * 64), j = rem >> 6, l = rem & 63;
      const float* col = W + (size_t)(16 * j + 4 * (l >> 4)) * ldw + 16 * t + (l & 15);
      st4(img + dst0 + 4 * (size_t)f, f32x4{col[0], col[ldw], col[2 * ldw], col[3 * ldw]});
    }
  };
  op_image(swimg::OP_WHH, enc_w + ENC_WHH, 64, 0, 4, 16);
  op_image(swimg::OP_W1H, dec_w + DEC_W1, 160, 0, 4, 10);
  op_image(swimg::OP_W1SZ, dec_w + DEC_W1, 160, 64, 6, 10);
  op_image(swimg::OP_W2, dec_w + DEC_W2, 160, 0, 10, 5);
  op_image_T(swimg::OP_WHHT, enc_w + ENC_WHH, 64, 16, 4);
  op_image_T(swimg::OP_W2T, dec_w + DEC_W2, 160, 5, 10);
  op_image_T(swimg::OP_W1HT, dec_w + DEC_W1, 160, 10, 4);
  for (int f = tid; f < 8 * 2 * 4 * 64; f += nth) {
    const int l = f & 63, j = (f >> 6) & 3, tile = (f >> 8) & 1, w = f >> 9, m = l & 15;
    const int row = (2 * tile + ((m & 3) >> 1)) * 64 + 8 * w + 2 * (m >> 2) + (m & 1);
    st4(img + swimg::OP_WHH8 + 4 * (size_t)f, ld4(enc_w + ENC_WHH + (size_t)row * 64 + 16 * j + 4 * (l >> 4)));
  }
  if (emb_w) {
    op_image(swimg::OP_E1, emb_w + EMB_W1, 32, 0, 2, 4);
    op_image(swimg::OP_E2, emb_w + EMB_W2, 64, 0, 4, 4);
    op_image_T(swimg::OP_E1T, emb_w + EMB_W1, 32, 4, 2);
    op_image_T(swimg::OP_E2T, emb_w + EMB_W2, 64, 4, 4);
    op_image_T(swimg::OP_ATT_T, att_w + ATT_W, 64, 4, 4);
  }
}
__global__ __launch_bounds__(256) void gen_images_kernel(const float* __restrict__ enc_w, const float* __restrict__ dec_w,
                                                          const float* __restrict__ emb_w, const float* __restrict__ att_w,
                                                          float* __restrict__ img) {
  gen_images_block(enc_w, dec_w, emb_w, att_w, img, blockIdx.x);
}
static thread_local const float *g_img_enc = nullptr, *g_img_dec = nullptr, *g_img_emb = nullptr, *g_img_att = nullptr,
                                *g_img = nullptr;
const float* sw_soc_images_for(const float* emb_w, const float* att_w) {
  return (g_img && emb_w && emb_w == g_img_emb && att_w == g_img_att) ? g_img : nullptr;
}
const float* sw_gen_images_for(const float* enc_w, const float* dec_w) {
  return (g_img && enc_w == g_img_enc && (!dec_w || dec_w == g_img_dec)) ? g_img : nullptr;
}
extern "C" int sw_gen_image_floats(void) { return swimg::N; }
static void gen_images_register(const float* enc_w, const float* dec_w, const float* emb_w, const float* att_w,
                                const float* img) {
  g_img_enc = enc_w; g_img_dec = dec_w; g_img_emb = emb_w; g_img_att = att_w; g_img = img;
}
extern "C" int sw_gen_images(const float* enc_w, const float* dec_w, const float* emb_w, const float* att_w, float* img,
                             void* stream) {
  if (!img) {
    gen_images_register(nullptr, nullptr, nullptr, nullptr, nullptr);
    return SW_OK;
  }
  if (!enc_w || !dec_w || ((emb_w != nullptr) != (att_w != nullptr))) return SW_EARG;
  SW_LAUNCH(gen_images_kernel, dim3(SW_IMG_BLOCKS), dim3(256), 0, (hipStream_t)stream, enc_w, dec_w, emb_w, att_w, img);
  SW_CHECK_LAUNCH("gen_images_kernel");
  gen_images_register(enc_w, dec_w, emb_w, att_w, img);
  return SW_OK;
}

__global__ __launch_bounds__(256) void stage_step_kernel(const float* __restrict__ slot, int B, int To, int Tp,
                                                          float* __restrict__ obsv_dst, float* __restrict__ pred_dst,
                                                          float* __restrict__ pred4_dst, float* __restrict__ targets_dst,
                                                          float* __restrict__ z_dst, float* __restrict__ steps_dst,
                                                          int n_d_updates, const float* __restrict__ enc_w,
                                                          const float* __restrict__ dec_w, const float* __restrict__ emb_w,
                                                          const float* __restrict__ att_w, float* __restrict__ img,
                                                          int img_blocks, const float* __restrict__ d_w,
                                                          float* __restrict__ d_img, const int* __restrict__ d_tab, int d_n,
                                                          int dimg_blocks, int z_device) {
  if ((int)blockIdx.x >= (int)gridDim.x - img_blocks) {
    gen_images_block(enc_w, dec_w, emb_w, att_w, img, (int)blockIdx.x - ((int)gridDim.x - img_blocks));
    return;
  }
  if ((int)blockIdx.x >= (int)gridDim.x - img_blocks - dimg_blocks) {
    disc_images_scatter(d_w, d_img, d_tab, d_n, (int)blockIdx.x - ((int)gridDim.x - img_blocks - dimg_blocks), dimg_blocks);
    return;
  }
  const unsigned long long* ptrs = reinterpret_cast<const unsigned long long*>(slot);
  const float* obsv = reinterpret_cast<const float*>(ptrs[0]);
  const float* pred = reinterpret_cast<const float*>(ptrs[1]);
  const int gid = blockIdx.x * 256 + threadIdx.x, gsz = ((int)gridDim.x - img_blocks - dimg_blocks) * 256;
  if (z_dst) {
    const float* zs = z_device ? reinterpret_cast<const float*>(ptrs[4]) : slot + 8;
    for (int i = gid; i < B * SW_Z / 4; i += gsz) st4(z_dst + 4 * (size_t)i, ld4(zs + 4 * (size_t)i));
  }
  if (gid < 2) targets_dst[gid] = slot[4 + gid];
  if (steps_dst && gid <= n_d_updates) steps_dst[gid] = gid < n_d_updates ? slot[6] + 1.0f + (float)gid : slot[7] + 1.0f;
  for (int i = gid; i < B * To; i += gsz)
    *reinterpret_cast<float2*>(obsv_dst + 2 * (size_t)i) = *reinterpret_cast<const float2*>(obsv + 2 * (size_t)i);
  for (int k = gid; k < B * Tp; k += gsz) {
    const int b = k / Tp, t = k - b * Tp;
    const float2 p = *reinterpret_cast<const float2*>(pred + 2 * (size_t)k);
    const float2 q = *reinterpret_cast<const float2*>(t == 0 ? obsv + ((size_t)b * To + To - 1) * 2 : pred + 2 * (size_t)k - 2);
    *reinterpret_cast<float2*>(pred_dst + 2 * (size_t)k) = p;
    st4(pred4_dst + 4 * (size_t)k, f32x4{p.x, p.y, p.x - q.x, p.y - q.y});
  }
}
#define SW_DIMG_BLOCKS 16
extern "C" int sw_stage_step_zdev(const float* slot, int B, int To, int Tp, float* obsv_dst, float* pred_dst,
                                  float* pred4_dst, float* targets_dst, float* z_dst, float* steps_dst, int n_d_updates,
                                  const float* enc_w, const float* dec_w, const float* emb_w, const float* att_w, float* img,
                                  const float* d_w, float* d_img, const int* d_tab, int z_device, void* stream) {
  if (z_device && !z_dst) return SW_EARG;
  if (!slot || !obsv_dst || !pred_dst || !pred4_dst || !targets_dst || B < 1 || To < 2 || Tp < 1 ||
      n_d_updates < 0 || n_d_updates > 254)
    return SW_EARG;
  if (img && (!enc_w || !dec_w || ((emb_w != nullptr) != (att_w != nullptr)))) return SW_EARG;
  if (d_img && (!d_w || !d_tab || Tp > 64)) return SW_EARG;
  int n = z_dst ? B * SW_Z / 4 : B * (To > Tp ? To : Tp);
  int blocks = (n + 255) / 256;
  if (blocks > 1024) blocks = 1024;
  const int ib = img ? SW_IMG_BLOCKS : 0, db = d_img ? SW_DIMG_BLOCKS : 0;
  SW_LAUNCH(stage_step_kernel, dim3(blocks + ib + db), dim3(256), 0, (hipStream_t)stream, slot, B, To, Tp, obsv_dst,
                     pred_dst, pred4_dst, targets_dst, z_dst, steps_dst, n_d_updates, enc_w, dec_w, emb_w, att_w, img, ib,
                     d_w, d_img, d_tab, d_img ? swp::disc(Tp).n : 0, db, z_device ? 1 : 0);
  SW_CHECK_LAUNCH("stage_step_kernel");
  if (img) gen_images_register(enc_w, dec_w, emb_w, att_w, img);
  if (d_img) sw_disc_images_register(d_w, d_img, d_tab, Tp);
  return SW_OK;
}
extern "C" int sw_stage_step_img(const float* slot, int B, int To, int Tp, float* obsv_dst, float* pred_dst,
                                 float* pred4_dst, float* targets_dst, float* z_dst, float* steps_dst, int n_d_updates,
                                 const float* enc_w, const float* dec_w, const float* emb_w, const float* att_w, float* img,
                                 const float* d_w, float* d_img, const int* d_tab, void* stream) {
  return sw_stage_step_zdev(slot, B, To, Tp, obsv_dst, pred_dst, pred4_dst, targets_dst, z_dst, steps_dst, n_d_updates, enc_w,
                            dec_w, emb_w, att_w, img, d_w, d_img, d_tab, 0, stream);
}
extern "C" int sw_stage_step(const float* slot, int B, int To, int Tp, float* obsv_dst, float* pred_dst,
                             float* pred4_dst, float* targets_dst, float* z_dst, float* steps_dst, int n_d_updates,
                             void* stream) {
  return sw_stage_step_img(slot, B, To, Tp, obsv_dst, pred_dst, pred4_dst, targets_dst, z_dst, steps_dst, n_d_updates, nullptr,
                           nullptr, nullptr, nullptr, nullptr, nullptr, nullptr, nullptr, stream);
}
```

### socialways_amd/ops.py

```python
import os

import numpy as np
import torch

from . import _lib as L
from .data import check_obs_len


class SceneIndex:

    def __init__(self, sub_batches, B, device):
        sb = np.asarray(sub_batches, dtype=np.int64).reshape(-1, 2)
        if len(sb) == 0:
            sb = np.array([[0, B]], dtype=np.int64)
        if sb[0, 0] != 0 or sb[-1, 1] != B or (sb[1:, 0] != sb[:-1, 1]).any():
            raise ValueError("sub_batches must tile [0, B) contiguously")
        n = sb[:, 1] - sb[:, 0]
        if (n <= 0).any():
            raise ValueError("empty scene in sub_batches")
        self.S = len(sb)
        self.B = int(B)
        small = n <= L.AMAX
        self.amax = int(n[small].max()) if small.any() else 0
        pairs = np.where((n > 1) & small, n * n, 0)
# ... 8 lines not shown
        self.big_blocks = torch.tensor(recs, dtype=torch.int32).reshape(-1, 8).to(device) if recs else None
        poff = np.concatenate([[0], np.cumsum(pairs)]).astype(np.int64)
        self.P = int(poff[-1])
        off = np.concatenate([sb[:, 0], [B]]).astype(np.int32)
        self.scene_off = torch.from_numpy(off).to(device)
        self.pair_off = torch.from_numpy(poff).to(device)
        self.sizes = n

    _cache = {}

    @classmethod
    def get(cls, sub_batches, B, device):
        sb = np.ascontiguousarray(np.asarray(sub_batches, dtype=np.int64))
        key = (sb.tobytes(), int(B), str(device))
        hit = cls._cache.get(key)
        if hit is None:
            if len(cls._cache) > 4096:
                cls._cache.clear()
            hit = cls._cache[key] = cls(sb, B, device)
            hit.key = key
        return hit


class Workspaces:

    def __init__(self, device):
        self.device = device
        self.buf = {}
        self._wgb = None
        self.retired = []
        self.version = 0

    @property
    def wgrad_batch(self):
        if self._wgb is None:
            lib = L.load()
            self._wgb, self._free = lib.sw_wgrad_batch_new(), lib.sw_wgrad_batch_free
        return self._wgb

    def __del__(self):
        if getattr(self, "_wgb", None):
            self._free(self._wgb)
            self._wgb = None

    def get(self, name, nfloats):
        t = self.buf.get(name)
        if t is None or t.numel() < nfloats:
            if t is not None:
                self.retired.append(t)
                self.version += 1
            n = max(int(nfloats), 1) if t is None else max(int(nfloats), int(1.25 * t.numel()))
            t = torch.empty(n, dtype=torch.float32, device=self.device)
            self.buf[name] = t
        return t

    def release_retired(self):
        self.retired.clear()


_default_ws = {}


def default_ws(device):
    key = str(device)
    if key not in _default_ws:
        _default_ws[key] = Workspaces(device)
    return _default_ws[key]


class GenCtx:
    __slots__ = ("obsv", "noise", "scenes", "hT", "cT", "S", "attn", "gsave", "B", "To", "Tp", "use_social", "wh", "ml")


def _ragged_arg(obs_len, B, device, noise_src=None, d_obs=None):
    if obs_len is None:
        return None
    if noise_src is not None:
        raise ValueError("obs_len: the ragged encoder launch pulls no z - noise_src must be None (the caller copies z)")
    if d_obs is not None:
        raise ValueError("obs_len: there is no precomputed observation pass for ragged rows - d_obs must be None")
    return _check_obs_len_tensor(obs_len, B, device)


def _enc_save(obsv, enc_w, B, To, hT, cT, gsave, x4s_ptr, obs_len, aux, st):
    if obs_len is None:
        L.call("sw_enc_lstm_fwd_aux", L.ptr(obsv), 0, L.ptr(enc_w), None, None, B, To, L.ptr(hT), L.ptr(cT), None,
               L.ptr(gsave), x4s_ptr, 0, aux[0], aux[1], aux[2], st)
    elif gsave is None:
        L.call("sw_enc_lstm_fwd_ragged", L.ptr(obsv), 0, L.ptr(enc_w), L.ptr(obs_len), B, To, L.ptr(hT), L.ptr(cT), st)
    else:
        L.call("sw_enc_lstm_fwd_ragged_save", L.ptr(obsv), 0, L.ptr(enc_w), L.ptr(obs_len), B, To, L.ptr(hT), L.ptr(cT),
               L.ptr(gsave), x4s_ptr, st)


def gen_forward(enc_w, emb_w, att_w, dec_w, obsv, noise, scenes, n_next, use_social, save, ws=None, tag="g", ade=None,
                noise_src=None, d_obs=None, obs_len=None):
    obs_len = _ragged_arg(obs_len, obsv.shape[0], obsv.device, noise_src, d_obs)
    L.require_gpu(obsv)
    obsv = obsv.contiguous()
    noise = noise.contiguous()
    B, To = obsv.shape[0], obsv.shape[1]
    if noise.shape != (B, 32):
        raise ValueError("noise must be (B, 32)")
    dev = obsv.device
    st = L.stream()
    hT = torch.empty(B, 64, device=dev)
    cT = torch.empty(B, 64, device=dev)
    pred4 = torch.empty(B, n_next, 4, device=dev)
    gsave = None
    if save:
        nfl = L.workspace_floats(L.WS_GSAVE, B, To, n_next)
        gsave = ws.get(tag + ".gsave", nfl) if ws is not None else torch.empty(nfl, device=dev)
    x4s_off = (To + n_next - 1) * B * 384
    z_in_enc, z_in_soc, n_enc = noise_src, None, noise.numel() if noise_src else 0
    _enc_save(obsv, enc_w, B, To, hT, cT, gsave, (gsave.data_ptr() + 4 * x4s_off) if save else None, obs_len,
              (z_in_enc, L.ptr(noise) if z_in_enc else None, n_enc), st)
    attn = wh = ml = None
    if use_social:
        S = torch.empty(B, 64, device=dev)
        attn = torch.empty(B, L.AMAX, device=dev) if save else None
        if scenes.NB:
            wh = torch.empty(B * 132, device=dev)
            ml = torch.empty(B, 2, device=dev) if save else None
        L.call("sw_social_pool_fwd_aux", L.ptr(obsv), To, L.ptr(hT), L.ptr(scenes.scene_off), scenes.S, B, scenes.amax,
               L.ptr(emb_w), L.ptr(att_w), L.ptr(S), L.ptr(attn), L.ptr(scenes.big_blocks), scenes.NB, L.ptr(wh), L.ptr(ml),
               z_in_soc, (noise.data_ptr() + 4 * n_enc) if z_in_soc else None, (noise.numel() - n_enc) if z_in_soc else 0, st)
    else:
        S = torch.zeros(B, 64, device=dev)
    L.call("sw_dec_rollout_fwd_aux", L.ptr(obsv), To, L.ptr(noise), L.ptr(S), L.ptr(hT), L.ptr(cT), L.ptr(enc_w),
           L.ptr(dec_w), B, n_next, L.ptr(pred4), None, None, L.ptr(gsave),
           L.ptr(ade[0]) if ade else None, float(ade[1]) if ade else 0.0, L.ptr(ade[2]) if ade else None,
           L.ptr(d_obs[0]) if d_obs else None, L.ptr(d_obs[1]) if d_obs else None, st)
    if not save:
        return pred4, None
    ctx = GenCtx()
    ctx.obsv, ctx.noise, ctx.scenes, ctx.hT, ctx.cT, ctx.S, ctx.attn = obsv, noise, scenes, hT, cT, S, attn
    ctx.gsave, ctx.B, ctx.To, ctx.Tp, ctx.use_social = gsave, B, To, n_next, use_social
    ctx.wh, ctx.ml = wh, ml
    return pred4, ctx


DFUSE = True


def gen_backward(enc_w, emb_w, att_w, dec_w, ctx, dpred4, d_enc, d_emb, d_att, d_dec, ws=None, tag="g", aux=None, adam=None,
                 dfuse=None):
    dev = ctx.obsv.device
    ws = ws or default_ws(dev)
    B, To, Tp = ctx.B, ctx.To, ctx.Tp
    gdelta = ws.get(tag + ".gdelta", L.workspace_floats(L.WS_GDELTA, B, To, Tp))
    wgrad = ws.get("wgrad", L.workspace_floats(L.WS_WGRAD, B, To, Tp))
    tmp = ws.get(tag + ".dwx", 2048)
    dhT = torch.empty(B, 64, device=dev)
    dcT = torch.empty(B, 64, device=dev)
    dS = torch.empty(B, 64, device=dev)
    aux_late = None
    if dfuse is not None:
        d_w, pred_hat, targets, t_idx, z, g_label, g_code, loss_part = dfuse
        dscr = ws.get(tag + ".dpred", B * Tp * 4)
        L.call("sw_dec_rollout_bwd_dfuse", L.ptr(ctx.obsv), L.ptr(pred_hat), L.ptr(d_w), L.ptr(targets), int(t_idx), L.ptr(z),
               g_label, g_code, L.ptr(loss_part), L.ptr(dscr), L.ptr(enc_w), L.ptr(dec_w), L.ptr(ctx.gsave), B, To, Tp,
               L.ptr(gdelta), L.ptr(dhT), L.ptr(dcT), L.ptr(dS), L.stream())
        aux_late = aux
    else:
        dpred4 = dpred4.contiguous()
        L.call("sw_dec_rollout_bwd_aux", L.ptr(dpred4), L.ptr(enc_w), L.ptr(dec_w), L.ptr(ctx.gsave), B, To, Tp,
               L.ptr(gdelta), L.ptr(dhT), L.ptr(dcT), L.ptr(dS), L.ptr(aux[0]) if aux else None, L.ptr(aux[1]) if aux else None,
               L.ptr(aux[2]) if aux else None, aux[1].numel() if aux else 0, L.stream())
    pending = None
    if ctx.use_social and (ctx.scenes.P > 0 or ctx.scenes.NB > 0):
        sc = ctx.scenes
        pending = ws.wgrad_batch
        pws = ws.get("pairs", L.workspace_floats(L.WS_PAIRS, B, To, Tp, 1, sc.P))
        bigp = ws.get("bigpart", sc.big_rows * 132) if sc.NB else None
        L.call("sw_social_pool_bwd", L.ptr(ctx.obsv), To, L.ptr(ctx.hT), L.ptr(sc.scene_off), L.ptr(sc.pair_off), sc.S,
               B, sc.amax, sc.P, L.ptr(emb_w), L.ptr(att_w), L.ptr(ctx.attn), L.ptr(dS), L.ptr(dhT), L.ptr(d_emb),
               L.ptr(d_att), L.ptr(pws), L.ptr(wgrad), L.ptr(sc.big_blocks), sc.NB, L.ptr(ctx.wh), L.ptr(ctx.ml),
               L.ptr(ctx.S), L.ptr(bigp), pending, L.stream())
    else:
        d_emb.zero_()
        d_att.zero_()
    L.call("sw_enc_lstm_bwd_aux", L.ptr(enc_w), L.ptr(ctx.gsave), None, L.ptr(dhT), L.ptr(dcT), None, B, To, 0,
           L.ptr(gdelta), None, None, L.ptr(aux_late[0]) if aux_late else None, L.ptr(aux_late[1]) if aux_late else None,
           L.ptr(aux_late[2]) if aux_late else None, aux_late[1].numel() if aux_late else 0, L.stream())
    if adam is not None:
        w_all, g_all, m, v, step, lr, b1, b2, eps = adam
        L.call("sw_gen_wgrad_adam", L.ptr(enc_w), L.ptr(dec_w), L.ptr(ctx.gsave), L.ptr(gdelta), L.ptr(ctx.noise), L.ptr(ctx.S),
               B, To, Tp, L.ptr(d_enc), L.ptr(d_dec), L.ptr(wgrad), L.ptr(tmp), pending, L.ptr(w_all), L.ptr(m), L.ptr(v),
               L.ptr(g_all), w_all.numel(), L.ptr(step), lr, b1, b2, eps, L.stream())
        return
    L.call("sw_gen_wgrad", L.ptr(enc_w), L.ptr(dec_w), L.ptr(ctx.gsave), L.ptr(gdelta), L.ptr(ctx.noise), L.ptr(ctx.S), B, To, Tp,
           L.ptr(d_enc), L.ptr(d_dec), 0, L.ptr(wgrad), L.ptr(tmp), pending, L.stream())


class GenCtxK:
    __slots__ = ("one", "K", "obsv_k", "noise_k", "S_k", "gsave_k")


def gen_forward_k(enc_w, emb_w, att_w, dec_w, obsv, noise_k, scenes, n_next, use_social, K, ws, tag="gv", obs_len=None):
    obs_len = _ragged_arg(obs_len, obsv.shape[0], obsv.device)
    L.require_gpu(obsv)
    obsv = obsv.contiguous()
    noise_k = noise_k.contiguous()
    B, To = obsv.shape[0], obsv.shape[1]
    KB = K * B
    if noise_k.shape != (KB, 32):
        raise ValueError("noise must be (K * B, 32)")
    dev = obsv.device
    st = L.stream()
    hT, cT = torch.empty(B, 64, device=dev), torch.empty(B, 64, device=dev)
    gsave_1 = ws.get(tag + ".gsave1", L.workspace_floats(L.WS_GSAVE, B, To, n_next))
    gsave_k = ws.get(tag + ".gsave", L.workspace_floats(L.WS_GSAVE, KB, To, n_next))
    Ta = To + n_next - 1
    _enc_save(obsv, enc_w, B, To, hT, cT, gsave_1, gsave_1.data_ptr() + 4 * Ta * B * 384, obs_len, (None, None, 0), st)
    attn = wh = ml = None
    if use_social:
        S = torch.empty(B, 64, device=dev)
        attn = torch.empty(B, L.AMAX, device=dev)
        if scenes.NB:
            wh, ml = torch.empty(B * 132, device=dev), torch.empty(B, 2, device=dev)
        L.call("sw_social_pool_fwd_aux", L.ptr(obsv), To, L.ptr(hT), L.ptr(scenes.scene_off), scenes.S, B, scenes.amax,
               L.ptr(emb_w), L.ptr(att_w), L.ptr(S), L.ptr(attn), L.ptr(scenes.big_blocks), scenes.NB, L.ptr(wh), L.ptr(ml),
               None, None, 0, st)
    else:
        S = torch.zeros(B, 64, device=dev)
    obsv_k, hT_k, cT_k, S_k = obsv.repeat(K, 1, 1), hT.repeat(K, 1), cT.repeat(K, 1), S.repeat(K, 1)
    row = gsave_1[(To - 1) * B * 384: To * B * 384].view(1, B, 384)
    gsave_k[(To - 1) * KB * 384: To * KB * 384].view(K, B, 384).copy_(row.expand(K, B, 384))
    pred4 = torch.empty(KB, n_next, 4, device=dev)
    L.call("sw_dec_rollout_fwd_aux", L.ptr(obsv_k), To, L.ptr(noise_k), L.ptr(S_k), L.ptr(hT_k), L.ptr(cT_k), L.ptr(enc_w),
           L.ptr(dec_w), KB, n_next, L.ptr(pred4), None, None, L.ptr(gsave_k), None, 0.0, None, None, None, st)
    one = GenCtx()
    one.obsv, one.noise, one.scenes, one.hT, one.cT, one.S, one.attn = obsv, noise_k[:B], scenes, hT, cT, S, attn
    one.gsave, one.B, one.To, one.Tp, one.use_social, one.wh, one.ml = gsave_1, B, To, n_next, use_social, wh, ml
    ctx = GenCtxK()
    ctx.one, ctx.K, ctx.obsv_k, ctx.noise_k, ctx.S_k, ctx.gsave_k = one, K, obsv_k, noise_k, S_k, gsave_k
    return pred4, ctx


def gen_backward_k(enc_w, emb_w, att_w, dec_w, ctx, dpred4_k, d_enc, d_emb, d_att, d_dec, ws, tag="gv", aux=None):
    one, K = ctx.one, ctx.K
    dev = dpred4_k.device
    B, To, Tp = one.B, one.To, one.Tp
    KB = K * B
    dpred4_k = dpred4_k.contiguous()
    gdelta_k = ws.get(tag + ".gdelta", L.workspace_floats(L.WS_GDELTA, KB, To, Tp))
    gdelta_1 = ws.get(tag + ".gdelta1", L.workspace_floats(L.WS_GDELTA, B, To, Tp))
    wgrad = ws.get("wgrad", L.workspace_floats(L.WS_WGRAD, B, To, Tp))
    tmp = ws.get(tag + ".dwx", 2048)
    dh_k, dc_k, dS_k = (torch.empty(KB, 64, device=dev) for _ in range(3))
    L.call("sw_dec_rollout_bwd_aux", L.ptr(dpred4_k), L.ptr(enc_w), L.ptr(dec_w), L.ptr(ctx.gsave_k), KB, To, Tp,
           L.ptr(gdelta_k), L.ptr(dh_k), L.ptr(dc_k), L.ptr(dS_k), L.ptr(aux[0]) if aux else None,
           L.ptr(aux[1]) if aux else None, L.ptr(aux[2]) if aux else None, aux[1].numel() if aux else 0, L.stream())
    dhT, dcT, dS = (t.view(K, B, 64).sum(0) for t in (dh_k, dc_k, dS_k))
    L.call("sw_gen_wgrad", L.ptr(enc_w), L.ptr(dec_w), L.ptr(ctx.gsave_k), L.ptr(gdelta_k), L.ptr(ctx.noise_k), L.ptr(ctx.S_k),
           KB, To, Tp, L.ptr(d_enc), L.ptr(d_dec), 1, L.ptr(wgrad), L.ptr(tmp), None, L.stream())
    pending = None
    if one.use_social and (one.scenes.P > 0 or one.scenes.NB > 0):
        sc = one.scenes
        pending = ws.wgrad_batch
        pws = ws.get("pairs", L.workspace_floats(L.WS_PAIRS, B, To, Tp, 1, sc.P))
        bigp = ws.get("bigpart", sc.big_rows * 132) if sc.NB else None
        L.call("sw_social_pool_bwd", L.ptr(one.obsv), To, L.ptr(one.hT), L.ptr(sc.scene_off), L.ptr(sc.pair_off), sc.S,
               B, sc.amax, sc.P, L.ptr(emb_w), L.ptr(att_w), L.ptr(one.attn), L.ptr(dS), L.ptr(dhT), L.ptr(d_emb),
               L.ptr(d_att), L.ptr(pws), L.ptr(wgrad), L.ptr(sc.big_blocks), sc.NB, L.ptr(one.wh), L.ptr(one.ml),
               L.ptr(one.S), L.ptr(bigp), pending, L.stream())
    else:
        d_emb.zero_()
        d_att.zero_()
    L.call("sw_enc_lstm_bwd", L.ptr(enc_w), L.ptr(one.gsave), None, L.ptr(dhT), L.ptr(dcT), None, B, To, 0,
           L.ptr(gdelta_1), None, None, L.stream())
    L.call("sw_gen_wgrad", L.ptr(enc_w), L.ptr(dec_w), L.ptr(one.gsave), L.ptr(gdelta_1), L.ptr(one.noise), L.ptr(one.S), B, To, Tp,
# ... 369 lines not shown
```

### socialways_amd/trainer.py

```python
import copy
import os
import sys
from types import SimpleNamespace

import numpy as np
import torch
import torch.optim as opt

from . import _lib as L
from . import ops
from .data import shard_scenes
from .model import Discriminator, Generator, get_traj_4d, predict_cv, refuse_obs_len
from .noise import EVAL, TRAIN, DeviceNoise


class PackedAdam:

    MIN_CHUNK, MAX_CHUNKS = 2048, 30

    def __init__(self, flat, gflat, slices, lr, betas=(0.9, 0.999), eps=1e-8, capturable=False, disc_tp=0):
        self.slices = slices
        self.flat = flat
        self.gflat = gflat
        self.native = flat.is_cuda
# ... 143 lines not shown
        if dn is not None and not isinstance(dn, DeviceNoise):
            raise TypeError("noise must be a DeviceNoise or None, got %s" % type(dn).__name__)
        return dn

    def _pad_z(self, z):
        return z if z.shape[-1] == self.Z_COLS else torch.nn.functional.pad(z, (0, self.Z_COLS - z.shape[-1]))

    def __init__(self, n_next, hidden_size=64, lr_g=1e-4, lr_d=1e-3, n_unrolling_steps=1, use_social=True,
                 use_info_loss=True, loss_info_w=0.5, n_latent_codes=2, device="cuda", process_group=None,
                 fused_adam=True, use_graph=None, use_l2_loss=False, use_variety_loss=False, loss_l2_w=0.5, variety_k=20):
        self.device = L.indexed_device(device)
        self.n_next = n_next
        self.noise_len = hidden_size // 2
        self.n_unrolling_steps = n_unrolling_steps
        self.use_info_loss = use_info_loss
        self.loss_info_w = loss_info_w
        if use_variety_loss not in (False, True, "fixed"):
            raise ValueError("use_variety_loss: False, True (train.py:527-536 as written) or 'fixed'")
        self.use_l2_loss, self.use_variety_loss, self.loss_l2_w = use_l2_loss, use_variety_loss, loss_l2_w
        self.variety_k = int(variety_k)
        self.last_variety = None
        self.G = Generator(hidden_size, 1, use_social=use_social, device=self.device)
        self.G.unify()
        self.world = 1 if process_group is None else torch.distributed.get_world_size(process_group)
        if use_graph is None:
            use_graph = self.device.type == "cuda" and fused_adam
        self.use_graph = bool(use_graph)
        self.max_graphs = int(os.environ.get("SW_MAX_GRAPHS", "8"))
        self._graphs = {}
        self._force_dist = os.environ.get("SW_FORCE_DIST", "") == "1"
        self._fuse_d_adam = True
        self._fuse_g_adam = True
        gc_env = os.environ.get("SW_GRAPH_COLLECTIVES", "")
        self._graph_collectives = True if gc_env == "1" else False if gc_env == "0" else None
        packed = fused_adam and self.device.type == "cuda"
        if packed:
            self.predictor_optimizer = PackedAdam(self.G._flat_all, self.G._gflat_all, self.G.packed_slices(), lr_g)
        else:
            self.predictor_optimizer = opt.Adam(self.G.predictor_params(), lr=lr_g, betas=(0.9, 0.999))
        self.D = Discriminator(n_next, hidden_size, n_latent_codes, device=self.device)
        if packed:
            self.D_optimizer = PackedAdam(self.D._flat, self.D._gflat,
                                          [(off, k, tuple(p.shape)) + (self.D._true[i] if self.D._true is not None else ())
                                           for i, ((off, k), p) in enumerate(zip(self.D._slices, self.D.parameters()))], lr_d,
                                          disc_tp=n_next)
        else:
            self.D_optimizer = opt.Adam(self.D.parameters(), lr=lr_d, betas=(0.9, 0.999))
        self.pg = process_group
        self.rank = 0 if process_group is None else torch.distributed.get_rank(process_group)
        self.epoch = 0
        if self.pg is not None and self.world > 1:
            self.sync_replicas()
        self._direct, self.exchange_probe = None, None
        mode = os.environ.get("SW_ALLREDUCE", "")
        if (self.pg is not None and (self.world > 1 or self._force_dist) and self.device.type == "cuda"
                and mode in ("direct", "auto")):
            from . import comm
            buckets = [self.D._gflat.numel(), self.G._gflat_all.numel()]
            if mode == "direct":
                self._direct = comm.DirectAllReduce(self.pg, self.device, max(buckets))
                if os.environ.get("SW_ALLREDUCE_CHECK", "1") != "0" and not self._direct.check(buckets):
                    self._direct.close()
                    self._direct = None
                    raise L.SocialWaysHipError("SW_ALLREDUCE=direct: the exchange disagrees with the process group's all-reduce "
                                               "on this node (or a wait timed out); use SW_ALLREDUCE=auto or unset it")
            else:
                self._direct, self.exchange_probe = comm.probe(self.pg, self.device, buckets)
            if self._direct is not None and self._graph_collectives is None:
                self._graph_collectives = bool(self.use_graph)
        self.ws = ops.Workspaces(self.device)
        self._ws_version = 0
        self._gimg = torch.empty(L.load().sw_gen_image_floats(), device=self.device) if self.device.type == "cuda" else None
        self._dimg = self._dtab = None
        if self.device.type == "cuda":
            lib = L.load()
            tab = np.empty((self.D._flat.numel(), 2), dtype=np.int32)
            if lib.sw_disc_image_table(n_next, tab.ctypes.data) != 0:
                raise L.SocialWaysHipError("sw_disc_image_table(%d)" % n_next)
            self._dtab = torch.from_numpy(tab).to(self.device)
            self._dimg = torch.zeros(lib.sw_disc_image_floats(n_next), device=self.device)
        self._lin_mask = None
        self._lin_maskf = None
        self._noise_src = None

    @property
    def use_social(self):
        return self.G.use_social

    def sync_replicas(self):
        dist = torch.distributed
        src = dist.get_global_rank(self.pg, 0)
        bufs = [self.G._flat_all, self.D._flat]
        for o in (self.predictor_optimizer, self.D_optimizer):
            if isinstance(o, PackedAdam):
                bufs += [o.m, o.v]
            else:
                for st in o.state.values():
                    bufs += [st["exp_avg"], st["exp_avg_sq"]]
        for b in bufs:
            dist.broadcast(b, src, group=self.pg)
        ts = torch.tensor([float(getattr(o, "t", 0)) for o in (self.predictor_optimizer, self.D_optimizer)] + [float(self.epoch)],
                          device=self.device if dist.get_backend(self.pg) == "nccl" else "cpu")
        dist.broadcast(ts, src, group=self.pg)
        for o, t in zip((self.predictor_optimizer, self.D_optimizer), ts.tolist()):
            if isinstance(o, PackedAdam):
                o.t = int(t)
                o.step_t.fill_(float(o.t))
        self.epoch = int(ts[2].item())

    def sync_rng(self):
        dist = torch.distributed
        obj = [(np.random.get_state(), torch.get_rng_state())] if self.rank == 0 else [None]
        dist.broadcast_object_list(obj, src=dist.get_global_rank(self.pg, 0), group=self.pg,
                                   device=self.device if dist.get_backend(self.pg) == "nccl" else None)
        if self.rank != 0:
            np.random.set_state(obj[0][0])
            torch.set_rng_state(obj[0][1])

    def _allreduce(self, flat):
        if self.pg is not None and (self.world > 1 or self._force_dist):
            d = self._direct
            if (d is not None and flat.is_cuda and flat.dtype == torch.float32 and flat.is_contiguous()
                    and 1024 <= flat.numel() <= d.max_floats):
                d(flat)
            else:
                torch.distributed.all_reduce(flat, op=torch.distributed.ReduceOp.SUM, group=self.pg)

    def _exchange_adam(self, opt, flat):
        return (self._direct is not None and (self.world > 1 or self._force_dist) and isinstance(opt, PackedAdam) and opt.native
                and opt.fusable and flat.numel() >= 1024)

    def _probe_graph_collectives(self):
        import ctypes
        import threading
        dev, W = self.device, self.world
        if torch.distributed.get_backend(self.pg) != "nccl":
            return False
        ok = 0.0
        guard = threading.Timer(180.0, lambda: (sys.stderr.write("socialways_amd: captured all-reduce probe hung; "
                                                                 "set SW_GRAPH_COLLECTIVES=0\n"), os._exit(3)))
        guard.daemon = True
        guard.start()
        x = torch.full((1024,), float(self.rank + 1), device=dev)
        y = torch.zeros_like(x)
        self._allreduce(y)
        torch.cuda.synchronize()
        side = torch.cuda.Stream(device=dev)
        try:
            g = torch.cuda.CUDAGraph()
            with torch.cuda.stream(side):
                g.capture_begin(capture_error_mode="thread_local")
                try:
                    y.copy_(x)
                    self._allreduce(y)
                except Exception:
                    try:
                        g.capture_end()
                    except Exception:
                        pass
                    hip, junk = ctypes.CDLL("libamdhip64.so"), ctypes.c_void_p()
                    hip.hipStreamEndCapture(ctypes.c_void_p(side.cuda_stream), ctypes.byref(junk))
                    hip.hipGetLastError()
                    raise
                g.capture_end()
                for _ in range(2):
                    g.replay()
# ... 20 lines not shown
        self._graphs.clear()
        self.ws.release_retired()
        self._ws_version = self.ws.version

    def close(self):
        self.release_graphs()
        d, self._direct = self._direct, None
        if d is not None:
            d.close()

    def _z_resident(self, batches):
        return all(nz.is_cuda and nz.dtype == torch.float32 and nz.is_contiguous() and nz.device == self.device
                   and tuple(nz.shape) == (b[0].shape[0], self.Z_COLS) for b in batches for nz in (b[4],))

    def _graph_key(self, scenes, To, ss, Bg, K, zdev=False):
        og, od = self.predictor_optimizer.param_groups[0], self.D_optimizer.param_groups[0]
        return (scenes.key, To, float(ss), float(Bg), self._row0, K, self.n_unrolling_steps, self.use_info_loss,
                self.loss_info_w, self.use_l2_loss, self.use_variety_loss, self.loss_l2_w, self.variety_k,
                og["lr"], tuple(og["betas"]), og["eps"], og.get("weight_decay", 0), od["lr"], tuple(od["betas"]), od["eps"],
                od.get("weight_decay", 0), bool(zdev))

    def _graphs_current(self):
        if self._ws_version != self.ws.version:
            self.release_graphs()

    def step(self, obsv, pred, sub_batches, zeros_val, ones_val, noise, ss=1.0, global_B=None, out=None, global_row0=0,
             variety_noise=None, obs_len=None):
        self._resolve_collectives()
        B = obsv.shape[0]
        self._obs_len = None
        if obs_len is not None:
            if obsv.shape[2] != 2:
                raise ValueError("step(obs_len=...) takes positions (B, To, 2)")
            obs_len = ops.obs_len_arg(obs_len, B, obsv.shape[1], 2, self.device)
        Bg = float(global_B if global_B is not None else B)
        dev = self.device
        self._row0 = int(global_row0)
        if self.use_variety_loss is True and Bg < 20:
            raise ValueError("use_variety_loss indexes agent 19 of the packed batch (train.py:531): batch of %d" % Bg)
        self._vnoise = None
        if self.use_variety_loss == "fixed":
            vn = variety_noise if variety_noise is not None else torch.rand((self.variety_k - 1) * B, self.noise_len)
            if vn.dim() != 2 or vn.shape[0] != (self.variety_k - 1) * B or vn.shape[1] not in (self.noise_len, self.Z_COLS):
                raise ValueError("variety_noise must be ((variety_k - 1) * B, %d)" % self.noise_len)
            self._vnoise = self._pad_z(vn.to(dev, non_blocking=True)).contiguous()
        part = None
        if not self._graphs and self.ws.retired:
            self.ws.release_retired()
        if self.use_graph and self.use_variety_loss != "fixed" and obs_len is None:
            scenes = ops.SceneIndex.get(sub_batches, B, dev)
            self._graphs_current()
            zdev = self._z_resident([(obsv, pred, zeros_val, ones_val, noise)])
            if self._graph_key(scenes, obsv.shape[1], ss, Bg, 1, zdev) in self._graphs or len(self._graphs) < self.max_graphs:
                part = self._step_graph([(obsv, pred, zeros_val, ones_val, noise)], sub_batches, float(ss), Bg)[0]
        if part is None:
            part = torch.zeros(self.n_unrolling_steps + 3, (B + 15) // 16, 3, device=dev)
            scenes = ops.SceneIndex.get(sub_batches, B, dev)
            noise = self._pad_z(noise.to(dev, non_blocking=True)).contiguous()
            targets = torch.tensor([float(zeros_val), float(ones_val)], dtype=torch.float32).to(dev, non_blocking=True)
            self._obs_len = obs_len
            try:
                self._step_impl(obsv.contiguous(), pred.contiguous(), None, scenes, targets, noise, float(ss), Bg, part)
            finally:
                self._obs_len = None
        if out is False:
            return part
        return part.sum(1, dtype=torch.float64)

    def step_many(self, batches, sub_batches, ss=1.0, global_B=None, out=None, global_row0=0):
        self._resolve_collectives()
        if not self.use_graph or len(batches) == 1 or self.use_variety_loss:
            return [self.step(o, p, sub_batches, zv, ov, nz, ss, global_B, out, global_row0) for o, p, zv, ov, nz in batches]
        B = batches[0][0].shape[0]
        Bg = float(global_B if global_B is not None else B)
        self._row0 = int(global_row0)
        scenes = ops.SceneIndex.get(sub_batches, B, self.device)
        self._graphs_current()
        key = self._graph_key(scenes, batches[0][0].shape[1], ss, Bg, len(batches), self._z_resident(batches))
        if key not in self._graphs and len(self._graphs) >= self.max_graphs:
            return [self.step(o, p, sub_batches, zv, ov, nz, ss, global_B, out, global_row0) for o, p, zv, ov, nz in batches]
        parts = self._step_graph(batches, sub_batches, float(ss), Bg)
        return parts if out is False else [q.sum(1, dtype=torch.float64) for q in parts]

    def _step_graph(self, batches, sub_batches, ss, Bg):
        K = len(batches)
        B, To, Tp = batches[0][0].shape[0], batches[0][0].shape[1], self.n_next
        dev = self.device
        scenes = ops.SceneIndex.get(sub_batches, B, dev)
        zdev = self._z_resident(batches)
        key = self._graph_key(scenes, To, ss, Bg, K, zdev)
        st = self._graphs.get(key)
        HDR = 8
        if st is None:
            st = self._graphs[key] = dict(
                n=0, graph=None, flip=0, scenes=scenes, obsv=torch.empty(B, To, 2, device=dev),
                pred=torch.empty(B, Tp, 2, device=dev), pred4=torch.empty(B, Tp, 4, device=dev),
                targets=torch.empty(4, device=dev), noise=torch.zeros(B, self.Z_COLS, device=dev),
                steps=torch.zeros(self.n_unrolling_steps + 2, device=dev),
                outs=[torch.zeros(self.n_unrolling_steps + 3, (B + 15) // 16, 3, device=dev) for _ in range(K)],
                slots=[[torch.zeros(HDR + B * self.Z_COLS, dtype=torch.float32).pin_memory() for _ in range(K)]
                       for _ in range(2)],
                done=[torch.cuda.Event(), torch.cuda.Event()], keep=[None, None])
        k = (st["flip"] ^ 1) if st["graph"] is not None else 0
        st["done"][k].synchronize()
        packed = isinstance(self.D_optimizer, PackedAdam)
        keep = []
        for j, (obsv, pred, zeros_val, ones_val, noise) in enumerate(batches):
            obsv, pred = obsv.contiguous(), pred.contiguous()
            keep.append((obsv, pred))
            hn = st["slots"][k][j].numpy()
            hn[:4].view(np.uint64)[:] = (obsv.data_ptr(), pred.data_ptr())
            hn[4], hn[5] = float(zeros_val), float(ones_val)
            if packed:
                hn[6], hn[7] = float(self.D_optimizer.t), float(self.predictor_optimizer.t)
                self.D_optimizer.t += self.n_unrolling_steps + 1
                self.predictor_optimizer.t += 1
            if zdev:
                hn[HDR:HDR + 2].view(np.uint64)[:] = noise.data_ptr()
                keep.append(noise)
                continue
            np.copyto(hn[HDR:].reshape(B, self.Z_COLS)[:, :self.noise_len], (noise.cpu() if noise.is_cuda else noise).numpy())
        st["keep"][k] = keep

        def stage(kk, j):
            slot = st["slots"][kk][j]
            L.call("sw_stage_step_zdev", slot.data_ptr(), B, To, Tp, L.ptr(st["obsv"]), L.ptr(st["pred"]),
                   L.ptr(st["pred4"]), L.ptr(st["targets"]), L.ptr(st["noise"]) if zdev else None, L.ptr(st["steps"]),
                   self.n_unrolling_steps + 1,
                   L.ptr(self.G.encoder._flat), L.ptr(self.G.decoder._flat), L.ptr(self.G.feature_embedder._flat),
                   L.ptr(self.G.attention._flat), L.ptr(self._gimg),
                   L.ptr(self.D._flat) if self._dimg is not None else None, L.ptr(self._dimg), L.ptr(self._dtab), int(zdev),
                   L.stream())
            self._noise_src = None if zdev else slot.data_ptr() + 4 * HDR

        def args(j):
            return (st["obsv"], st["pred"], st["pred4"], scenes, st["targets"], st["noise"], ss, Bg, st["outs"][j],
                    st["steps"] if packed else None)

        def body(kk):
            for j in range(K):
                yield from self._step_gen(*args(j), pre=lambda j=j: stage(kk, j))
        if st["graph"] is not None:
            st["flip"] = k
            for g, buf in st["graph"][k]:
                g.replay()
                if buf is not None:
                    self._allreduce(buf)
        elif st["n"] < 2:
            st["n"] += 1
            for j in range(K):
                stage(0, j)
                self._step_impl(*args(j))
        else:
            torch.cuda.synchronize()
            pool, sets = None, []
            for kk in range(2):
                gen = body(kk)
                graphs, fin = [], False
                while not fin:
                    g = torch.cuda.CUDAGraph()
                    with torch.cuda.graph(g, pool=pool, capture_error_mode="thread_local"):
                        while True:
                            try:
                                buf = next(gen)
                            except StopIteration:
                                buf, fin = None, True
                            if fin:
                                break
                            if self.world > 1 or self._force_dist:
                                if not self._graph_collectives:
                                    break
                                self._allreduce(buf)
                    graphs.append((g, buf))
                    pool = g.pool()
                sets.append(graphs)
            st["graph"], st["flip"] = sets, 0
            for g, buf in sets[0]:
                g.replay()
                if buf is not None:
                    self._allreduce(buf)
        st["done"][k].record()
        return st["outs"]

    def _step_impl(self, obsv, pred, pred4, scenes, targets, noise, ss, Bg, out, steps=None):
        for buf in self._step_gen(obsv, pred, pred4, scenes, targets, noise, ss, Bg, out, steps):
            self._allreduce(buf)
        return out

    def _step_gen(self, obsv, pred, pred4, scenes, targets, noise, ss, Bg, out, steps=None, pre=None):
        G, D = self.G, self.D
        B, Tp = obsv.shape[0], self.n_next
        dev = self.device
        ws = self.ws
        U = self.n_unrolling_steps
        g_label = 1.0 / Bg
        g_code = (self.loss_info_w if self.use_info_loss else 0.0) / (2.0 * Bg)
        if pre is not None:
            pre()
        else:
            if self._gimg is not None:
                L.call("sw_gen_images", L.ptr(G.encoder._flat), L.ptr(G.decoder._flat), L.ptr(G.feature_embedder._flat),
                       L.ptr(G.attention._flat), L.ptr(self._gimg), L.stream())
            self._disc_images()
        try:
            yield from self._step_body(obsv, pred, pred4, scenes, targets, noise, ss, Bg, out, steps)
        finally:
            if self._gimg is not None:
                L.call("sw_gen_images", None, None, None, None, None, None)
            if self._dimg is not None:
                L.call("sw_disc_images", None, None, None, 0, None)

    def _disc_images(self):
        if self._dimg is not None:
            L.call("sw_disc_images", L.ptr(self.D._flat), L.ptr(self._dimg), L.ptr(self._dtab), self.n_next, L.stream())

    def _step_body(self, obsv, pred, pred4, scenes, targets, noise, ss, Bg, out, steps):
        G, D = self.G, self.D
        B, Tp = obsv.shape[0], self.n_next
        dev = self.device
        ws = self.ws
        U = self.n_unrolling_steps
        g_label = 1.0 / Bg
        g_code = (self.loss_info_w if self.use_info_loss else 0.0) / (2.0 * Bg)
        noise_src, self._noise_src = self._noise_src, None
        ol = getattr(self, "_obs_len", None)
        if pred4 is None:
            pred4 = torch.empty(B, Tp, 4, device=dev)
            o4_scratch = ws.get("o4", B * obsv.shape[1] * 4)
            L.call("sw_traj_4d", L.ptr(obsv), L.ptr(pred), B, obsv.shape[1], Tp, L.ptr(o4_scratch), L.ptr(pred4), L.stream())
        enc, emb, att, dec = G.encoder, G.feature_embedder, G.attention, G.decoder
        KV = self.variety_k if self.use_variety_loss == "fixed" else 1
        if KV > 1:
            pred_hat_k, gctx = ops.gen_forward_k(enc._flat, emb._flat, att._flat, dec._flat, obsv,
                                                 torch.cat([noise, self._vnoise]), scenes, Tp, G.use_social, KV, ws=ws, obs_len=ol)
            pred_hat = pred_hat_k[:B]
            out[U + 2].zero_()
            L.call("sw_ade_fde", L.ptr(pred_hat), L.ptr(pred), B, Tp, 1.0 / float(ss), L.ptr(out[U + 2]),
                   L.ptr(ws.get("ade_scratch", 3 * L.RED_BLOCKS)), L.stream())
            d_pre = None
        else:
            d_pre = ops.d_obs_buffer(ws, B, obsv.shape[1], Tp) if obsv.shape[2] == 2 and ol is None else None
            pred_hat, gctx = ops.gen_forward(enc._flat, emb._flat, att._flat, dec._flat, obsv, noise, scenes, Tp,
                                             G.use_social, save=True, ws=ws, ade=(pred, 1.0 / float(ss), out[U + 2]),
                                             noise_src=noise_src, d_obs=(D._flat, d_pre) if d_pre is not None else None,
                                             obs_len=ol)
        d_gflat = D.grad_views()
        backup = None
        for u in range(self.n_unrolling_steps + 1):
            if u == 1:
                backup = ws.get("d_backup", D._flat.numel())
            fuse = (self._fuse_d_adam and isinstance(self.D_optimizer, PackedAdam) and self.D_optimizer.fusable
                    and not (self.world > 1 or self._force_dist))
            adam = self.D_optimizer.fused_args(None if steps is None else steps[u]) if fuse else None
            if ol is None and obsv.shape[2] == 2 and ops.disc_update_supported(D._flat, B, obsv.shape[1], Tp):
                ops.disc_update(D._flat, obsv, [pred_hat, pred4], targets, (0, 1), noise, g_label, g_code, d_gflat, ws,
                                obs_pre=(u == 0 and d_pre is not None), w_snapshot=backup if u == 1 else None,
                                loss_part=out[u], adam=adam)
            else:
                labels, codes, dctx = ops.disc_forward(D._flat, obsv, [pred_hat, pred4], save=True, ws=ws,
                                                       save_lstm=2 if (u == 0 and d_pre is not None) else 1,
                                                       w_snapshot=backup if u == 1 else None, obs_len=ol)
                ops.disc_backward_gan(D._flat, dctx, labels, codes, targets, (0, 1), noise, g_label, g_code, d_gflat, (), ws=ws,
                                      loss_part=out[u], adam=adam)
            if self._exchange_adam(self.D_optimizer, d_gflat):
                self._direct.adam(d_gflat, self.D_optimizer, None if steps is None else steps[u])
                continue
            yield d_gflat
            if not fuse:
                self.D_optimizer.step() if steps is None else self.D_optimizer.step(steps[u])
                if not getattr(self.D_optimizer, "keeps_images", False):
                    self._disc_images()
        dfuse = None
        one_pass = ops.disc_dpred_supported(Tp)
        if (ops.DFUSE and one_pass and KV == 1 and not self.use_l2_loss and self.use_variety_loss is False
                and obsv.shape[2] == 2 and ol is None):
            dfuse = (D._flat, pred_hat, targets, 1, noise, g_label, g_code, out[U + 1])
        dpred = None
        if dfuse is None and one_pass:
            dpred = ops.disc_dpred(D._flat, obsv, pred_hat, targets, 1, noise, g_label, g_code, loss_part=out[U + 1], obs_len=ol)
        elif dfuse is None:
            labels, codes, dctx = ops.disc_forward(D._flat, obsv, [pred_hat], save=True, ws=ws, save_lstm=0, obs_len=ol)
            dpred = ops.disc_backward_gan(D._flat, dctx, labels, codes, targets, (1,), noise, g_label, g_code, None, (True,),
                                          ws=ws, loss_part=out[U + 1])[0]
        if self.use_l2_loss:
            L.call("sw_l2_grad", L.ptr(pred_hat), L.ptr(pred), B, Tp, 0, B, self.loss_l2_w / (Bg * Tp), L.ptr(dpred), L.stream())
        if self.use_variety_loss is True:
            r = 19 - self._row0
            if 0 <= r < B:
                L.call("sw_l2_grad", L.ptr(pred_hat), L.ptr(pred), B, Tp, r, r + 1, self.loss_l2_w / Tp, L.ptr(dpred), L.stream())
        if KV > 1:
            dk = torch.zeros(KV * B, Tp, 4, device=dev)
            dk[:B].copy_(dpred)
            l2min, kmin = torch.empty(B, device=dev), torch.empty(B, dtype=torch.int32, device=dev)
            L.call("sw_variety_grad", L.ptr(pred_hat_k), L.ptr(pred), KV, B, Tp, self.loss_l2_w / (Bg * Tp), L.ptr(dk),
                   L.ptr(kmin), L.ptr(l2min), L.stream())
            self.last_variety = (l2min, kmin)
            dpred = dk
        restore = None
        if self.n_unrolling_steps > 0:
            if self._lin_maskf is None:
                self._lin_maskf = D.linear_mask().float().contiguous()
            restore = (backup[:D._flat.numel()], D._flat, self._lin_maskf)
        G.grad_views()
        fuse = (KV == 1 and self._fuse_g_adam and self._gimg is not None and isinstance(self.predictor_optimizer, PackedAdam)
                and self.predictor_optimizer.fusable and not (self.world > 1 or self._force_dist)
                and (not G.use_social or gctx.scenes.P > 0 or gctx.scenes.NB > 0))
        adam = None
        if fuse:
            opt = self.predictor_optimizer
            adam = (G._flat_all, G._gflat_all) + opt.fused_args(None if steps is None else steps[U + 1])
        if KV > 1:
            ops.gen_backward_k(enc._flat, emb._flat, att._flat, dec._flat, gctx, dpred, enc._gflat, emb._gflat, att._gflat,
                               dec._gflat, ws=ws, aux=restore)
        else:
            ops.gen_backward(enc._flat, emb._flat, att._flat, dec._flat, gctx, dpred, enc._gflat, emb._gflat, att._gflat,
                             dec._gflat, ws=ws, aux=restore, tag="g", adam=adam, dfuse=dfuse)
        if self._exchange_adam(self.predictor_optimizer, G._gflat_all):
            self._direct.adam(G._gflat_all, self.predictor_optimizer, None if steps is None else steps[U + 1])
        else:
            yield G._gflat_all
            if not fuse:
                self.predictor_optimizer.step() if steps is None else self.predictor_optimizer.step(steps[U + 1])
        self.last_pred_hat = pred_hat
        self.last_pred_hat_k = pred_hat_k if KV > 1 else None

    def losses_from(self, out, B_global, Tp=None, ss=1.0):
        o = out.detach().double().cpu().numpy()
        if o.ndim == 2:
            o = o[None]
        Bg = np.asarray(B_global, dtype=np.float64).reshape(-1, 1)
        U = self.n_unrolling_steps + 1
        Tp = Tp or self.n_next
        cols = []
        for u in range(U):
            cols += [o[:, u, 0:1] / Bg, o[:, u, 1:2] / (2 * Bg), o[:, u, 2:3] / Bg]
        cols += [o[:, U + 1, 2:3] * (ss * ss) / (2 * Tp * Bg), o[:, U, 0:1] / Bg, o[:, U, 1:2] / (2 * Bg)]
        return np.concatenate(cols, axis=1)

    def train_epoch(self, data, batch_size, draw=None):
        _refuse_ragged(data, "train_epoch()", "its graph-captured steps have no ragged form - train on the ragged windows with "
                       "train_epoch_ragged(), or on full windows (create_dataset) and evaluate the ragged ones with "
                       "evaluate*() / evaluate_history()")
        return self._train_epoch(data, batch_size, draw, None)

    def train_epoch_ragged(self, data, batch_size, draw=None):
        ol = getattr(data, "obs_len", None)
        if ol is None:
            raise L.SocialWaysHipError("train_epoch_ragged() needs a dataset with obs_len (create_dataset_ragged, "
                                       "SceneDataset(obs_len=...)): train a dataset of full windows with train_epoch()")
        return self._train_epoch(data, batch_size, draw, ol)

    def _train_epoch(self, data, batch_size, draw, obs_len):
        outs, sizes = [], []
        pend, pend_key = [], None
        dn = self._device_noise(None) if draw is None else None
        if self.world > 1 and draw is None:
            self.sync_rng()
        if self._direct is not None and self.world > 1:
            torch.distributed.barrier(group=self.pg)

        def flush():
            nonlocal pend, pend_key
            if pend:
                items = [p[0] for p in pend]
                if dn is not None:
                    r0 = pend[0][3]
                    z = dn.fill(items[0][0].shape[0], self.noise_len, domain=TRAIN, step=pend[0][4], n_steps=len(pend), row0=r0,
                                ld=self.Z_COLS, device=self.device)
                    items = [it[:4] + (z[j, 0],) for j, it in enumerate(items)]
                outs.extend(self.step_many(items, pend[0][1], data.ss, global_B=pend[0][2], global_row0=pend[0][3]))
                pend, pend_key = [], None
        for a, b, sb in data.packed_steps(batch_size):
            bs = b - a
            vn = step_i = None
            if draw is None:
                zv = np.random.uniform(0, 0.1)
                ov = np.random.uniform(0.9, 1.0)
                if dn is None:
                    noise = torch.rand(bs, self.noise_len)
                else:
                    noise, step_i = None, dn.step
                    dn.step += 1
            else:
                zv, ov, noise, *extra = draw(bs)
                vn = extra[0] if extra else None
            fixed = self.use_variety_loss == "fixed"
            if fixed and vn is None and dn is None:
                vn = torch.rand(self.variety_k - 1, bs, self.noise_len)
            sizes.append((bs, len(sb)))
            r0, r1, sbl = 0, bs, sb
            if self.world > 1:
                lo, hi = shard_scenes(sb, self.world)[self.rank]
                if hi <= lo:
                    flush()
                    outs.append(self._empty_step())
                    continue
                r0, r1 = int(sb[lo, 0]), int(sb[hi - 1, 1])
                sbl = sb[lo:hi] - r0
            item = (data.obsv[a + r0:a + r1], data.pred[a + r0:a + r1], zv, ov, noise[r0:r1] if noise is not None else None)
# ... 362 lines not shown
```

Before: 2801 steps/s.

## Fold next-step input staging and weight-image rebuild into fused generator Adam tail

Adds a tail variant of the fused generator wgrad+Adam launch that also rebuilds the generator and discriminator weight images and stages the next sub-step's inputs into a double-buffered set. A separate staging/image launch per sub-step inside the graph is no longer needed. The encoder forward kernel gains extra rider blocks that recompute its input projection from the raw weights and regenerate image slices, so the next step can tolerate stale images. This removes launch and serialization overhead in exchange for more complex cross-step dependencies and a risk of reading stale weights.

```diff
diff --git a/include/socialways_hip.h b/include/socialways_hip.h
--- a/include/socialways_hip.h
+++ b/include/socialways_hip.h
@@ -139,6 +139,19 @@
                       float* wgrad_ws, float* tmp , sw_wgrad_batch* pending , float* adam_w,
                       float* adam_m, float* adam_v, const float* adam_g, long long adam_n, const float* adam_step,
                       double lr, double beta1, double beta2, double eps, void* stream);
+int sw_gen_wgrad_adam_tail(const float* enc_w, const float* dec_w, const float* gsave, const float* gdelta,
+                           const float* z, const float* S_pool, int B, int To, int Tp, float* d_enc_w, float* d_dec_w,
+                           float* wgrad_ws, float* tmp , sw_wgrad_batch* pending , float* adam_w,
+                           float* adam_m, float* adam_v, const float* adam_g, long long adam_n, const float* adam_step,
+                           double lr, double beta1, double beta2, double eps, const float* emb_w, const float* att_w,
+                           float* img, const float* d_w, float* d_img, const int* d_tab,
+                           const float* slot_next, float* obsv_dst, float* pred_dst, float* pred4_dst, float* targets_dst,
+                           float* z_dst, float* steps_dst, int n_d_updates, int z_device, void* stream);
+int sw_enc_lstm_fwd_aux_img(const float* x, int x_mode, const float* enc_w, const float* h0, const float* c0, int B, int T,
+                            float* hT, float* cT, float* y, float* act, float* x4s, int t0, const float* aux_src,
+                            float* aux_dst, long long aux_n, const float* dec_w, float* img, void* stream);
+int sw_images_register(const float* enc_w, const float* dec_w, const float* emb_w , const float* att_w ,
+                       const float* img, const float* d_w, const float* d_img, const int* d_tab, int Tp);
 
 int sw_disc_fwd(const float* obsv, int To, int x_mode, const float* const* pred4 ,
                 int nb, const float* d_w, int B, int Tp, float* const* label ,
diff --git a/socialways_amd/_lib.py b/socialways_amd/_lib.py
--- a/socialways_amd/_lib.py
+++ b/socialways_amd/_lib.py
@@ -46,6 +46,11 @@
     "sw_gen_wgrad": (_i, [_vp, _vp, _vp, _vp, _vp, _vp, _i, _i, _i, _vp, _vp, _i, _vp, _vp, _vp, _vp]),
     "sw_gen_wgrad_adam": (_i, [_vp, _vp, _vp, _vp, _vp, _vp, _i, _i, _i, _vp, _vp, _vp, _vp, _vp, _vp, _vp, _vp, _vp,
                                ctypes.c_longlong, _vp, ctypes.c_double, ctypes.c_double, ctypes.c_double, ctypes.c_double, _vp]),
+    "sw_gen_wgrad_adam_tail": (_i, [_vp, _vp, _vp, _vp, _vp, _vp, _i, _i, _i, _vp, _vp, _vp, _vp, _vp, _vp, _vp, _vp, _vp,
+                                    ctypes.c_longlong, _vp, ctypes.c_double, ctypes.c_double, ctypes.c_double, ctypes.c_double,
+                                    _vp, _vp, _vp, _vp, _vp, _vp, _vp, _vp, _vp, _vp, _vp, _vp, _vp, _i, _i, _vp]),
+    "sw_enc_lstm_fwd_aux_img": (_i, [_vp, _i, _vp, _vp, _vp, _i, _i, _vp, _vp, _vp, _vp, _vp, _i, _vp, _vp, _ll, _vp, _vp, _vp]),
+    "sw_images_register": (_i, [_vp, _vp, _vp, _vp, _vp, _vp, _vp, _vp, _i]),
     "sw_enc_lstm_bwd_aux": (_i, [_vp, _vp, _vp, _vp, _vp, _vp, _i, _i, _i, _vp, _vp, _vp, _vp, _vp, _vp, _ll, _vp]),
     "sw_dec_rollout_bwd_dfuse": (_i, [_vp, _vp, _vp, _vp, _i, _vp, _f, _f, _vp, _vp, _vp, _vp, _vp, _i, _i, _i, _vp, _vp, _vp, _vp,
                                       _vp]),
diff --git a/socialways_amd/csrc/sw_lstm.hip b/socialways_amd/csrc/sw_lstm.hip
--- a/socialways_amd/csrc/sw_lstm.hip
+++ b/socialways_amd/csrc/sw_lstm.hip
@@ -1,6 +1,7 @@
 #include "../../include/socialways_hip.h"
 #include "sw_lstm_dev.h"
 #include <cstdlib>
+#define SW_ENC_IMG_RIDERS 6
 
 template <int XMODE, bool ACT, bool Y, bool X4S>
 __global__ __launch_bounds__(SW_THREADS) void enc_lstm_fwd_kernel(
@@ -85,9 +86,19 @@
 __global__ __launch_bounds__(512) void enc_lstm_fwd8_kernel(
     const float* __restrict__ x, const float* __restrict__ h0, const float* __restrict__ c0, int B, int T,
     float* __restrict__ hT, float* __restrict__ cT, float* __restrict__ act, float* __restrict__ x4s, int t0,
-    const float* __restrict__ aux_src, float* __restrict__ aux_dst, long long aux_n, const float* __restrict__ gimg) {
-  const int tiles = (B + SW_TILE - 1) / SW_TILE;
-  const int extra = (int)gridDim.x - tiles;
+    const float* __restrict__ aux_src, float* __restrict__ aux_dst, long long aux_n, const float* __restrict__ gimg,
+    const float* enc_w, const float* dec_w, float* img_out, int img_riders) {
+  const int tiles = (B + SW_TILE - 1) / SW_TILE;
+  const int extra = (int)gridDim.x - tiles - img_riders;
+  if ((int)blockIdx.x >= extra + tiles) {
+    const int r = (int)blockIdx.x - extra - tiles;
+    if (r < 2) {
+      if (threadIdx.x < 256) gen_images_block(enc_w, dec_w, nullptr, nullptr, img_out, r, false);
+    } else {
+      gen_images_raw(enc_w, dec_w, img_out, swimg::RAW_WIH, swimg::RAW_END, (r - 2) * 512 + (int)threadIdx.x, (img_riders - 2) * 512);
+    }
+    return;
+  }
   if ((int)blockIdx.x < extra) {
     const long long n4 = aux_n >> 2, stride = (long long)extra * 512;
     long long i = (long long)blockIdx.x * 512 + threadIdx.x;
@@ -110,10 +121,25 @@
   for (int tl = 0; tl < 2; ++tl) {
 #pragma unroll
     for (int j = 0; j < 4; ++j) whh[tl][j] = ld4(gimg + swimg::OP_WHH8 + ((((size_t)wave * 2 + tl) * 4 + j) * 64 + lane) * 4);
-    const int rowA = (2 * tl + ((ln & 3) >> 1)) * 64 + 8 * wave + 2 * (ln >> 2) + (ln & 1);
-    wx[tl] = gimg[swimg::WX + rowA * 4 + lg];
-#pragma unroll
-    for (int r = 0; r < 4; ++r) bias[tl][r] = gimg[swimg::BX + (2 * tl + (r >> 1)) * 64 + ub + (r & 1)];
+  }
+  auto load_wx = [&](const float* wxs, const float* bxs) {
+#pragma unroll
+    for (int tl = 0; tl < 2; ++tl) {
+      const int rowA = (2 * tl + ((ln & 3) >> 1)) * 64 + 8 * wave + 2 * (ln >> 2) + (ln & 1);
+      wx[tl] = wxs[rowA * 4 + lg];
+#pragma unroll
+      for (int r = 0; r < 4; ++r) bias[tl][r] = bxs[(2 * tl + (r >> 1)) * 64 + ub + (r & 1)];
+    }
+  };
+  if (img_riders > 0) {
+    float* wxl = &hbuf[1][0];
+    if (threadIdx.x < 256)
+      lstm_prep_rows(enc_w + swp::ENC_EMB_W, enc_w + swp::ENC_EMB_B, enc_w + swp::ENC_WIH, enc_w + swp::ENC_BIH,
+                     enc_w + swp::ENC_BHH, true, wxl, wxl + 1024);
+    sw_barrier();
+    load_wx(wxl, wxl + 1024);
+  } else {
+    load_wx(gimg + swimg::WX, gimg + swimg::BX);
   }
   float2 c = {0.f, 0.f}, h = {0.f, 0.f};
   if (h0) h = *reinterpret_cast<const float2*>(h0 + (size_t)b * 64 + ub);
@@ -243,10 +269,10 @@
   return SW_OK;
 }
 
-extern "C" int sw_enc_lstm_fwd_aux(const float* x, int x_mode, const float* enc_w, const float* h0,
-                                   const float* c0, int B, int T, float* hT, float* cT, float* y, float* act,
-                                   float* x4s, int t0, const float* aux_src, float* aux_dst, long long aux_n,
-                                   void* stream) {
+static int enc_lstm_fwd_aux_impl(const float* x, int x_mode, const float* enc_w, const float* h0,
+                                 const float* c0, int B, int T, float* hT, float* cT, float* y, float* act,
+                                 float* x4s, int t0, const float* aux_src, float* aux_dst, long long aux_n,
+                                 const float* dec_w, float* img, void* stream) {
   if (!x || !enc_w || !hT || !cT || B < 0 || T < 1 || t0 < 0 || (x_mode != 0 && x_mode != 1)) return SW_EARG;
   if (aux_n < 0 || (aux_n & 3) || (aux_n > 0 && (!aux_src || !aux_dst))) return SW_EARG;
   if (x_mode == 0 && T < 2) return SW_ESHAPE;
@@ -257,12 +283,14 @@
   if (extra > 64) extra = 64;
   static const int enc8_env = getenv("SW_ENC8") ? atoi(getenv("SW_ENC8")) : -1;
   const bool enc8 = enc8_env >= 0 ? enc8_env != 0 : tiles <= 256;
+  const int img_riders = img ? SW_ENC_IMG_RIDERS : 0;
   if (enc8 && gimg && x_mode == 0 && act && x4s && !y) {
-    SW_LAUNCH(enc_lstm_fwd8_kernel, dim3(tiles + extra), dim3(512), 0, (hipStream_t)stream, x, h0, c0, B, T, hT, cT, act, x4s, t0,
-              aux_src, aux_dst, aux_n, gimg);
+    SW_LAUNCH(enc_lstm_fwd8_kernel, dim3(tiles + extra + img_riders), dim3(512), 0, (hipStream_t)stream, x, h0, c0, B, T, hT, cT,
+              act, x4s, t0, aux_src, aux_dst, aux_n, gimg, enc_w, dec_w, img, img_riders);
     SW_CHECK_LAUNCH("enc_lstm_fwd8_kernel");
     return SW_OK;
   }
+  if (img) return SW_EARG;
 #define SW_ENC_FWD(XM, A, Y_, X4)                                                                                   \
   SW_LAUNCH((enc_lstm_fwd_kernel<XM, A, Y_, X4>), dim3(tiles + extra), dim3(SW_THREADS), 0, (hipStream_t)stream,    \
             x, enc_w, h0, c0, B, T, hT, cT, y, act, x4s, t0, aux_src, aux_dst, aux_n, gimg)
@@ -288,6 +316,21 @@
   SW_CHECK_LAUNCH("enc_lstm_fwd_kernel");
   return SW_OK;
 }
+extern "C" int sw_enc_lstm_fwd_aux(const float* x, int x_mode, const float* enc_w, const float* h0,
+                                   const float* c0, int B, int T, float* hT, float* cT, float* y, float* act,
+                                   float* x4s, int t0, const float* aux_src, float* aux_dst, long long aux_n,
+                                   void* stream) {
+  return enc_lstm_fwd_aux_impl(x, x_mode, enc_w, h0, c0, B, T, hT, cT, y, act, x4s, t0, aux_src, aux_dst, aux_n, nullptr, nullptr,
+                               stream);
+}
+extern "C" int sw_enc_lstm_fwd_aux_img(const float* x, int x_mode, const float* enc_w, const float* h0, const float* c0, int B,
+                                       int T, float* hT, float* cT, float* y, float* act, float* x4s, int t0,
+                                       const float* aux_src, float* aux_dst, long long aux_n, const float* dec_w, float* img,
+                                       void* stream) {
+  if (!img || !dec_w || !enc_w || img != sw_gen_images_for(enc_w, dec_w)) return SW_EARG;
+  return enc_lstm_fwd_aux_impl(x, x_mode, enc_w, h0, c0, B, T, hT, cT, y, act, x4s, t0, aux_src, aux_dst, aux_n, dec_w, img,
+                               stream);
+}
 extern "C" int sw_enc_lstm_fwd(const float* x, int x_mode, const float* enc_w, const float* h0,
                                const float* c0, int B, int T, float* hT, float* cT, float* y, float* act,
                                float* x4s, int t0, void* stream) {
diff --git a/socialways_amd/csrc/sw_lstm_dev.h b/socialways_amd/csrc/sw_lstm_dev.h
--- a/socialways_amd/csrc/sw_lstm_dev.h
+++ b/socialways_amd/csrc/sw_lstm_dev.h
@@ -419,3 +419,89 @@
   if (x_mode == 0) lstm_obs_loop<0, true>(W, hbuf, obsv, To, B, b, c, h, act, x4s);
   else lstm_obs_loop<1, true>(W, hbuf, obsv, To, B, b, c, h, act, x4s);
 }
+
+#define SW_IMG_BLOCKS 64
+__device__ __forceinline__ void gen_images_raw(const float* enc_w, const float* dec_w, float* img, int o_lo, int o_hi, int tid,
+                                               int nth) {
+  using namespace swp;
+  for (int i = tid; i < (o_hi - o_lo) / 4; i += nth) {
+    const int o = o_lo + 4 * i;
+    const float* src = o < swimg::RAW_WE   ? enc_w + ENC_WIH + (o - swimg::RAW_WIH)
+                       : o < swimg::RAW_BE ? enc_w + ENC_EMB_W + (o - swimg::RAW_WE)
+                       : o < swimg::RAW_W3 ? enc_w + ENC_EMB_B + (o - swimg::RAW_BE)
+                       : o < swimg::RAW_B3 ? dec_w + DEC_W3 + (o - swimg::RAW_W3)
+                       : o < swimg::RAW_W4 ? dec_w + DEC_B3 + (o - swimg::RAW_B3)
+                                           : dec_w + DEC_W4 + (o - swimg::RAW_W4);
+    st4(img + o, ld4(src));
+  }
+}
+__device__ __forceinline__ void gen_images_block(const float* __restrict__ enc_w, const float* __restrict__ dec_w,
+                                                 const float* __restrict__ emb_w, const float* __restrict__ att_w,
+                                                 float* __restrict__ img, int blk, bool raw) {
+  using namespace swp;
+  if (blk == 0) {
+    lstm_prep_rows(enc_w + ENC_EMB_W, enc_w + ENC_EMB_B, enc_w + ENC_WIH, enc_w + ENC_BIH, enc_w + ENC_BHH, true,
+                   img + swimg::WX, img + swimg::BX);
+    return;
+  }
+  if (blk == 1) {
+    const int t = threadIdx.x;
+    if (t < 160) {
+      const int c = t / 80, k = t - c * 80;
+      const float* w4 = dec_w + DEC_W4 + c * 40;
+      float v0 = 0.f, v1 = 0.f, v2 = 0.f, v3 = 0.f;
+#pragma unroll
+      for (int m = 0; m < 40; m += 4) {
+        v0 = fmaf(w4[m], dec_w[DEC_W3 + m * 80 + k], v0);
+        v1 = fmaf(w4[m + 1], dec_w[DEC_W3 + (m + 1) * 80 + k], v1);
+        v2 = fmaf(w4[m + 2], dec_w[DEC_W3 + (m + 2) * 80 + k], v2);
+        v3 = fmaf(w4[m + 3], dec_w[DEC_W3 + (m + 3) * 80 + k], v3);
+      }
+      img[swimg::W43 + c * 80 + k] = (v0 + v1) + (v2 + v3);
+    } else if (t < 162) {
+      const int c = t - 160;
+      float v = dec_w[DEC_B4 + c];
+#pragma unroll
+      for (int m = 0; m < 40; m += 4) {
+        const f32x4 w = ld4(dec_w + DEC_W4 + c * 40 + m), bb = ld4(dec_w + DEC_B3 + m);
+        v = fmaf(w[0], bb[0], fmaf(w[1], bb[1], fmaf(w[2], bb[2], fmaf(w[3], bb[3], v))));
+      }
+      img[swimg::W43 + 160 + c] = v;
+    }
+    return;
+  }
+  const int nth = (SW_IMG_BLOCKS - 2) * 256, tid = (blk - 2) * 256 + threadIdx.x;
+  if (raw) gen_images_raw(enc_w, dec_w, img, swimg::RAW_WIH, swimg::RAW_END, tid, nth);
+  auto op_image = [&](int dst0, const float* W, int ldw, int c0, int KJ, int ntile) {
+    for (int f = tid; f < ntile * KJ * 64; f += nth) {
+      const int t = f / (KJ * 64), rem = f - t * (KJ * 64), j = rem >> 6, l = rem & 63;
+      st4(img + dst0 + 4 * (size_t)f, ld4(W + (size_t)(16 * t + (l & 15)) * ldw + c0 + 16 * j + 4 * (l >> 4)));
+    }
+  };
+  auto op_image_T = [&](int dst0, const float* W, int ldw, int KJ, int ntile) {
+    for (int f = tid; f < ntile * KJ * 64; f += nth) {
+      const int t = f / (KJ * 64), rem = f - t * (KJ * 64), j = rem >> 6, l = rem & 63;
+      const float* col = W + (size_t)(16 * j + 4 * (l >> 4)) * ldw + 16 * t + (l & 15);
+      st4(img + dst0 + 4 * (size_t)f, f32x4{col[0], col[ldw], col[2 * ldw], col[3 * ldw]});
+    }
+  };
+  op_image(swimg::OP_WHH, enc_w + ENC_WHH, 64, 0, 4, 16);
+  op_image(swimg::OP_W1H, dec_w + DEC_W1, 160, 0, 4, 10);
+  op_image(swimg::OP_W1SZ, dec_w + DEC_W1, 160, 64, 6, 10);
+  op_image(swimg::OP_W2, dec_w + DEC_W2, 160, 0, 10, 5);
+  op_image_T(swimg::OP_WHHT, enc_w + ENC_WHH, 64, 16, 4);
+  op_image_T(swimg::OP_W2T, dec_w + DEC_W2, 160, 5, 10);
+  op_image_T(swimg::OP_W1HT, dec_w + DEC_W1, 160, 10, 4);
+  for (int f = tid; f < 8 * 2 * 4 * 64; f += nth) {
+    const int l = f & 63, j = (f >> 6) & 3, tile = (f >> 8) & 1, w = f >> 9, m = l & 15;
+    const int row = (2 * tile + ((m & 3) >> 1)) * 64 + 8 * w + 2 * (m >> 2) + (m & 1);
+    st4(img + swimg::OP_WHH8 + 4 * (size_t)f, ld4(enc_w + ENC_WHH + (size_t)row * 64 + 16 * j + 4 * (l >> 4)));
+  }
+  if (emb_w) {
+    op_image(swimg::OP_E1, emb_w + EMB_W1, 32, 0, 2, 4);
+    op_image(swimg::OP_E2, emb_w + EMB_W2, 64, 0, 4, 4);
+    op_image_T(swimg::OP_E1T, emb_w + EMB_W1, 32, 4, 2);
+    op_image_T(swimg::OP_E2T, emb_w + EMB_W2, 64, 4, 4);
+    op_image_T(swimg::OP_ATT_T, att_w + ATT_W, 64, 4, 4);
+  }
+}
diff --git a/socialways_amd/csrc/sw_misc.hip b/socialways_amd/csrc/sw_misc.hip
--- a/socialways_amd/csrc/sw_misc.hip
+++ b/socialways_amd/csrc/sw_misc.hip
@@ -208,7 +208,70 @@
   return 0;
 }
 
+__device__ __forceinline__ void stage_inputs_block(const float* __restrict__ slot, int B, int To, int Tp,
+                                                   float* __restrict__ obsv_dst, float* __restrict__ pred_dst,
+                                                   float* __restrict__ pred4_dst, float* __restrict__ targets_dst,
+                                                   float* __restrict__ z_dst, float* __restrict__ steps_dst, int n_d_updates,
+                                                   int z_device, int blk, int nblk) {
+  const unsigned long long* ptrs = reinterpret_cast<const unsigned long long*>(slot);
+  const float* obsv = reinterpret_cast<const float*>(ptrs[0]);
+  const float* pred = reinterpret_cast<const float*>(ptrs[1]);
+  const int gid = blk * 256 + threadIdx.x, gsz = nblk * 256;
+  if (z_dst) {
+    const float* zs = z_device ? reinterpret_cast<const float*>(ptrs[4]) : slot + 8;
+    for (int i = gid; i < B * SW_Z / 4; i += gsz) st4(z_dst + 4 * (size_t)i, ld4(zs + 4 * (size_t)i));
+  }
+  if (gid < 2) targets_dst[gid] = slot[4 + gid];
+  if (steps_dst && gid <= n_d_updates) steps_dst[gid] = gid < n_d_updates ? slot[6] + 1.0f + (float)gid : slot[7] + 1.0f;
+  for (int i = gid; i < B * To; i += gsz)
+    *reinterpret_cast<float2*>(obsv_dst + 2 * (size_t)i) = *reinterpret_cast<const float2*>(obsv + 2 * (size_t)i);
+  for (int k = gid; k < B * Tp; k += gsz) {
+    const int b = k / Tp, t = k - b * Tp;
+    const float2 p = *reinterpret_cast<const float2*>(pred + 2 * (size_t)k);
+    const float2 q = *reinterpret_cast<const float2*>(t == 0 ? obsv + ((size_t)b * To + To - 1) * 2 : pred + 2 * (size_t)k - 2);
+    *reinterpret_cast<float2*>(pred_dst + 2 * (size_t)k) = p;
+    st4(pred4_dst + 4 * (size_t)k, f32x4{p.x, p.y, p.x - q.x, p.y - q.y});
+  }
+}
+
 #define SW_DEC_COMPOSE_BLOCKS 13
+#define SW_DIMG_BLOCKS 16
+#define SW_TAIL_STAGE_BLOCKS 32
+struct StepTail {
+  float* img = nullptr;
+  const float* emb_w = nullptr;
+  const float* att_w = nullptr;
+  long long enc_off = 0, dec_off = 0, emb_off = 0, att_off = 0;
+  const float* d_w = nullptr;
+  float* d_img = nullptr;
+  const int* d_tab = nullptr;
+  int d_n = 0;
+  const float* slot = nullptr;
+  int B = 0, To = 0, Tp = 0, n_d_updates = 0, z_device = 0, stage_blocks = 0;
+  float *obsv_dst = nullptr, *pred_dst = nullptr, *pred4_dst = nullptr, *targets_dst = nullptr, *z_dst = nullptr,
+        *steps_dst = nullptr;
+};
+__device__ __forceinline__ void step_tail_rider(int r, const WgAdam& ad, const StepTail& tl) {
+  if (tl.img) {
+    if (r < SW_IMG_BLOCKS - 2) {
+      gen_images_block(ad.w + tl.enc_off, ad.w + tl.dec_off, tl.emb_w ? ad.w + tl.emb_off : nullptr,
+                       tl.att_w ? ad.w + tl.att_off : nullptr, tl.img, r + 2, false);
+      return;
+    }
+    r -= SW_IMG_BLOCKS - 2;
+  }
+  if (tl.d_img) {
+    if (r < SW_DIMG_BLOCKS) {
+      disc_images_scatter(tl.d_w, tl.d_img, tl.d_tab, tl.d_n, r, SW_DIMG_BLOCKS);
+      return;
+    }
+    r -= SW_DIMG_BLOCKS;
+  }
+  if (tl.slot && r < tl.stage_blocks)
+    stage_inputs_block(tl.slot, tl.B, tl.To, tl.Tp, tl.obsv_dst, tl.pred_dst, tl.pred4_dst, tl.targets_dst, tl.z_dst,
+                       tl.steps_dst, tl.n_d_updates, tl.z_device, r, tl.stage_blocks);
+}
+
 __device__ __forceinline__ void compose_bwd_block(const int blk, const float* __restrict__ enc_w,
                                                   const float* __restrict__ dWx, const float* __restrict__ dbx,
                                                   float* __restrict__ d_enc_w, const float* __restrict__ dec_w,
@@ -285,8 +348,13 @@
                                                               const float* __restrict__ dec_w,
                                                               const float* __restrict__ Ms,
                                                               float* __restrict__ d_dec_w, WgAdam ad,
-                                                              const float* __restrict__ snap) {
-  compose_bwd_block((int)blockIdx.x, enc_w, dWx, dbx, d_enc_w, dec_w, Ms, d_dec_w, ad, snap);
+                                                              const float* snap, StepTail tl) {
+  const int blk = (int)blockIdx.x;
+  if (blk >= 128 + SW_DEC_COMPOSE_BLOCKS) {
+    step_tail_rider(blk - (128 + SW_DEC_COMPOSE_BLOCKS), ad, tl);
+    return;
+  }
+  compose_bwd_block(blk, enc_w, dWx, dbx, d_enc_w, dec_w, Ms, d_dec_w, ad, snap);
 }
 __global__ __launch_bounds__(256) void compose_bwd_part_kernel(const float* __restrict__ enc_w, const float* __restrict__ dWx,
                                                                const float* __restrict__ dbx, float* __restrict__ d_enc_w,
@@ -298,7 +366,7 @@
 static int gen_wgrad_impl(const float* enc_w, const float* dec_w, const float* gsave, const float* gdelta, const float* z,
                           const float* S_pool, int B, int To, int Tp, float* d_enc_w, float* d_dec_w, int part,
                           float* wgrad_ws, float* tmp, sw_wgrad_batch* pending, void* stream, WgAdam ad,
-                          const float* snap) {
+                          const float* snap, const StepTail& tl = StepTail()) {
   if (!enc_w || !dec_w || !gsave || !gdelta || !z || !S_pool || !d_enc_w || !d_dec_w || !wgrad_ws || !tmp || B < 1 || To < 2 ||
       Tp < 1 || part < 0 || part > 2)
     return SW_EARG;
@@ -335,8 +403,9 @@
   if (rc_add) return SW_ESHAPE;
   if (int rc = ad.w ? wg_launch_adam(wb, wgrad_ws, ad, st) : wg_launch(wb, wgrad_ws, st)) return rc;
   if (part != 1) {
-    SW_LAUNCH(enc_compose_bwd_kernel, dim3(128 + SW_DEC_COMPOSE_BLOCKS), dim3(256), 0, st, enc_w, dWx, dbx, d_enc_w,
-                       dec_w, dM, d_dec_w, ad, snap);
+    const int riders = (tl.img ? SW_IMG_BLOCKS - 2 : 0) + (tl.d_img ? SW_DIMG_BLOCKS : 0) + (tl.slot ? tl.stage_blocks : 0);
+    SW_LAUNCH(enc_compose_bwd_kernel, dim3(128 + SW_DEC_COMPOSE_BLOCKS + riders), dim3(256), 0, st, enc_w, dWx, dbx, d_enc_w,
+                       dec_w, dM, d_dec_w, ad, snap, tl);
     SW_CHECK_LAUNCH("enc_compose_bwd_kernel");
   }
   return SW_OK;
@@ -347,11 +416,11 @@
   return gen_wgrad_impl(enc_w, dec_w, gsave, gdelta, z, S_pool, B, To, Tp, d_enc_w, d_dec_w, part, wgrad_ws, tmp, pending,
                         stream, WgAdam(), nullptr);
 }
-extern "C" int sw_gen_wgrad_adam(const float* enc_w, const float* dec_w, const float* gsave, const float* gdelta,
-                                 const float* z, const float* S_pool, int B, int To, int Tp, float* d_enc_w, float* d_dec_w,
-                                 float* wgrad_ws, float* tmp, sw_wgrad_batch* pending, float* adam_w, float* adam_m,
-                                 float* adam_v, const float* adam_g, long long adam_n, const float* adam_step, double lr,
-                                 double beta1, double beta2, double eps, void* stream) {
+static int gen_wgrad_adam_impl(const float* enc_w, const float* dec_w, const float* gsave, const float* gdelta,
+                               const float* z, const float* S_pool, int B, int To, int Tp, float* d_enc_w, float* d_dec_w,
+                               float* wgrad_ws, float* tmp, sw_wgrad_batch* pending, float* adam_w, float* adam_m,
+                               float* adam_v, const float* adam_g, long long adam_n, const float* adam_step, double lr,
+                               double beta1, double beta2, double eps, const StepTail& tl, void* stream) {
   if (!adam_w || !adam_m || !adam_v || !adam_g || !adam_step || adam_n < 1 || !enc_w || !dec_w || !d_enc_w || !d_dec_w)
     return SW_EARG;
   if (enc_w - adam_w != d_enc_w - adam_g || dec_w - adam_w != d_dec_w - adam_g || enc_w < adam_w ||
@@ -363,7 +432,63 @@
   ad.w = adam_w; ad.m = adam_m; ad.v = adam_v; ad.g0 = adam_g; ad.step = adam_step; ad.n = (size_t)adam_n;
   ad.lr = lr; ad.beta1 = beta1; ad.beta2 = beta2; ad.eps = eps;
   return gen_wgrad_impl(enc_w, dec_w, gsave, gdelta, z, S_pool, B, To, Tp, d_enc_w, d_dec_w, 0, wgrad_ws, tmp, pending, stream,
-                        ad, img);
+                        ad, img, tl);
+}
+extern "C" int sw_gen_wgrad_adam(const float* enc_w, const float* dec_w, const float* gsave, const float* gdelta,
+                                 const float* z, const float* S_pool, int B, int To, int Tp, float* d_enc_w, float* d_dec_w,
+                                 float* wgrad_ws, float* tmp, sw_wgrad_batch* pending, float* adam_w, float* adam_m,
+                                 float* adam_v, const float* adam_g, long long adam_n, const float* adam_step, double lr,
+                                 double beta1, double beta2, double eps, void* stream) {
+  return gen_wgrad_adam_impl(enc_w, dec_w, gsave, gdelta, z, S_pool, B, To, Tp, d_enc_w, d_dec_w, wgrad_ws, tmp, pending, adam_w,
+                             adam_m, adam_v, adam_g, adam_n, adam_step, lr, beta1, beta2, eps, StepTail(), stream);
+}
+extern "C" int sw_gen_wgrad_adam_tail(const float* enc_w, const float* dec_w, const float* gsave, const float* gdelta,
+                                      const float* z, const float* S_pool, int B, int To, int Tp, float* d_enc_w,
+                                      float* d_dec_w, float* wgrad_ws, float* tmp, sw_wgrad_batch* pending, float* adam_w,
+                                      float* adam_m, float* adam_v, const float* adam_g, long long adam_n,
+                                      const float* adam_step, double lr, double beta1, double beta2, double eps,
+                                      const float* emb_w, const float* att_w, float* img, const float* d_w,
+                                      float* d_img, const int* d_tab, const float* slot_next, float* obsv_dst, float* pred_dst,
+                                      float* pred4_dst, float* targets_dst, float* z_dst, float* steps_dst, int n_d_updates,
+                                      int z_device, void* stream) {
+  StepTail tl;
+  if (img) {
+    if (!adam_w || img != sw_gen_images_for(enc_w, dec_w) || ((emb_w != nullptr) != (att_w != nullptr)))
+      return SW_EARG;
+    if (emb_w && (emb_w < adam_w || emb_w + swp::EMB_N > adam_w + adam_n || att_w < adam_w || att_w + swp::ATT_N > adam_w + adam_n))
+      return SW_EARG;
+    tl.img = img; tl.emb_w = emb_w; tl.att_w = att_w;
+    tl.enc_off = enc_w - adam_w; tl.dec_off = dec_w - adam_w;
+    if (emb_w) { tl.emb_off = emb_w - adam_w; tl.att_off = att_w - adam_w; }
+  }
+  if (d_img) {
+    if (!d_w || !d_tab || Tp > 64) return SW_EARG;
+    tl.d_w = d_w; tl.d_img = d_img; tl.d_tab = d_tab; tl.d_n = swp::disc(Tp).n;
+  }
+  if (slot_next) {
+    if (!obsv_dst || !pred_dst || !pred4_dst || !targets_dst || (z_device && !z_dst) || n_d_updates < 0 || n_d_updates > 254)
+      return SW_EARG;
+    tl.slot = slot_next; tl.B = B; tl.To = To; tl.Tp = Tp; tl.n_d_updates = n_d_updates; tl.z_device = z_device ? 1 : 0;
+    tl.obsv_dst = obsv_dst; tl.pred_dst = pred_dst; tl.pred4_dst = pred4_dst; tl.targets_dst = targets_dst;
+    tl.z_dst = z_dst; tl.steps_dst = steps_dst;
+    const int n = z_dst ? B * SW_Z / 4 : B * (To > Tp ? To : Tp);
+    const int blocks = (n + 255) / 256;
+    tl.stage_blocks = blocks < SW_TAIL_STAGE_BLOCKS ? blocks : SW_TAIL_STAGE_BLOCKS;
+  }
+  return gen_wgrad_adam_impl(enc_w, dec_w, gsave, gdelta, z, S_pool, B, To, Tp, d_enc_w, d_dec_w, wgrad_ws, tmp, pending, adam_w,
+                             adam_m, adam_v, adam_g, adam_n, adam_step, lr, beta1, beta2, eps, tl, stream);
+}
+static void gen_images_register(const float* enc_w, const float* dec_w, const float* emb_w, const float* att_w,
+                                const float* img);
+extern "C" int sw_images_register(const float* enc_w, const float* dec_w, const float* emb_w, const float* att_w,
+                                  const float* img, const float* d_w, const float* d_img, const int* d_tab, int Tp) {
+  if (img && (!enc_w || !dec_w || ((emb_w != nullptr) != (att_w != nullptr)))) return SW_EARG;
+  if (d_img && (!d_w || !d_tab || Tp < 1 || Tp > 64)) return SW_EARG;
+  if (img) gen_images_register(enc_w, dec_w, emb_w, att_w, img);
+  else gen_images_register(nullptr, nullptr, nullptr, nullptr, nullptr);
+  if (d_img) sw_disc_images_register(d_w, d_img, d_tab, Tp);
+  else sw_disc_images_register(nullptr, nullptr, nullptr, 0);
+  return SW_OK;
 }
 
 extern "C" int sw_enc_lstm_wgrad(const float* enc_w, const float* act, const float* x4s, const float* h0, const float* dgates,
@@ -743,90 +868,10 @@
   return SW_OK;
 }
 
-#define SW_IMG_BLOCKS 64
-__device__ __forceinline__ void gen_images_block(const float* __restrict__ enc_w, const float* __restrict__ dec_w,
-                                                 const float* __restrict__ emb_w, const float* __restrict__ att_w,
-                                                 float* __restrict__ img, int blk) {
-  using namespace swp;
-  if (blk == 0) {
-    lstm_prep_rows(enc_w + ENC_EMB_W, enc_w + ENC_EMB_B, enc_w + ENC_WIH, enc_w + ENC_BIH, enc_w + ENC_BHH, true,
-                   img + swimg::WX, img + swimg::BX);
-    return;
-  }
-  if (blk == 1) {
-    const int t = threadIdx.x;
-    if (t < 160) {
-      const int c = t / 80, k = t - c * 80;
-      const float* w4 = dec_w + DEC_W4 + c * 40;
-      float v0 = 0.f, v1 = 0.f, v2 = 0.f, v3 = 0.f;
-#pragma unroll
-      for (int m = 0; m < 40; m += 4) {
-        v0 = fmaf(w4[m], dec_w[DEC_W3 + m * 80 + k], v0);
-        v1 = fmaf(w4[m + 1], dec_w[DEC_W3 + (m + 1) * 80 + k], v1);
-        v2 = fmaf(w4[m + 2], dec_w[DEC_W3 + (m + 2) * 80 + k], v2);
-        v3 = fmaf(w4[m + 3], dec_w[DEC_W3 + (m + 3) * 80 + k], v3);
-      }
-      img[swimg::W43 + c * 80 + k] = (v0 + v1) + (v2 + v3);
-    } else if (t < 162) {
-      const int c = t - 160;
-      float v = dec_w[DEC_B4 + c];
-#pragma unroll
-      for (int m = 0; m < 40; m += 4) {
-        const f32x4 w = ld4(dec_w + DEC_W4 + c * 40 + m), bb = ld4(dec_w + DEC_B3 + m);
-        v = fmaf(w[0], bb[0], fmaf(w[1], bb[1], fmaf(w[2], bb[2], fmaf(w[3], bb[3], v))));
-      }
-      img[swimg::W43 + 160 + c] = v;
-    }
-    return;
-  }
-  const int nth = (SW_IMG_BLOCKS - 2) * 256, tid = (blk - 2) * 256 + threadIdx.x;
-  for (int i = tid; i < (swimg::RAW_END - swimg::RAW_WIH) / 4; i += nth) {
-    const int o = swimg::RAW_WIH + 4 * i;
-    const float* src = o < swimg::RAW_WE   ? enc_w + ENC_WIH + (o - swimg::RAW_WIH)
-                       : o < swimg::RAW_BE ? enc_w + ENC_EMB_W + (o - swimg::RAW_WE)
-                       : o < swimg::RAW_W3 ? enc_w + ENC_EMB_B + (o - swimg::RAW_BE)
-                       : o < swimg::RAW_B3 ? dec_w + DEC_W3 + (o - swimg::RAW_W3)
-                       : o < swimg::RAW_W4 ? dec_w + DEC_B3 + (o - swimg::RAW_B3)
-                                           : dec_w + DEC_W4 + (o - swimg::RAW_W4);
-    st4(img + o, ld4(src));
-  }
-  auto op_image = [&](int dst0, const float* W, int ldw, int c0, int KJ, int ntile) {
-    for (int f = tid; f < ntile * KJ * 64; f += nth) {
-      const int t = f / (KJ * 64), rem = f - t * (KJ * 64), j = rem >> 6, l = rem & 63;
-      st4(img + dst0 + 4 * (size_t)f, ld4(W + (size_t)(16 * t + (l & 15)) * ldw + c0 + 16 * j + 4 * (l >> 4)));
-    }
-  };
-  auto op_image_T = [&](int dst0, const float* W, int ldw, int KJ, int ntile) {
-    for (int f = tid; f < ntile * KJ * 64; f += nth) {
-      const int t = f / (KJ * 64), rem = f - t * (KJ * 64), j = rem >> 6, l = rem & 63;
-      const float* col = W + (size_t)(16 * j + 4 * (l >> 4)) * ldw + 16 * t + (l & 15);
-      st4(img + dst0 + 4 * (size_t)f, f32x4{col[0], col[ldw], col[2 * ldw], col[3 * ldw]});
-    }
-  };
-  op_image(swimg::OP_WHH, enc_w + ENC_WHH, 64, 0, 4, 16);
-  op_image(swimg::OP_W1H, dec_w + DEC_W1, 160, 0, 4, 10);
-  op_image(swimg::OP_W1SZ, dec_w + DEC_W1, 160, 64, 6, 10);
-  op_image(swimg::OP_W2, dec_w + DEC_W2, 160, 0, 10, 5);
-  op_image_T(swimg::OP_WHHT, enc_w + ENC_WHH, 64, 16, 4);
-  op_image_T(swimg::OP_W2T, dec_w + DEC_W2, 160, 5, 10);
-  op_image_T(swimg::OP_W1HT, dec_w + DEC_W1, 160, 10, 4);
-  for (int f = tid; f < 8 * 2 * 4 * 64; f += nth) {
-    const int l = f & 63, j = (f >> 6) & 3, tile = (f >> 8) & 1, w = f >> 9, m = l & 15;
-    const int row = (2 * tile + ((m & 3) >> 1)) * 64 + 8 * w + 2 * (m >> 2) + (m & 1);
-    st4(img + swimg::OP_WHH8 + 4 * (size_t)f, ld4(enc_w + ENC_WHH + (size_t)row * 64 + 16 * j + 4 * (l >> 4)));
-  }
-  if (emb_w) {
-    op_image(swimg::OP_E1, emb_w + EMB_W1, 32, 0, 2, 4);
-    op_image(swimg::OP_E2, emb_w + EMB_W2, 64, 0, 4, 4);
-    op_image_T(swimg::OP_E1T, emb_w + EMB_W1, 32, 4, 2);
-    op_image_T(swimg::OP_E2T, emb_w + EMB_W2, 64, 4, 4);
-    op_image_T(swimg::OP_ATT_T, att_w + ATT_W, 64, 4, 4);
-  }
-}
 __global__ __launch_bounds__(256) void gen_images_kernel(const float* __restrict__ enc_w, const float* __restrict__ dec_w,
                                                           const float* __restrict__ emb_w, const float* __restrict__ att_w,
                                                           float* __restrict__ img) {
-  gen_images_block(enc_w, dec_w, emb_w, att_w, img, blockIdx.x);
+  gen_images_block(enc_w, dec_w, emb_w, att_w, img, blockIdx.x, true);
 }
 static thread_local const float *g_img_enc = nullptr, *g_img_dec = nullptr, *g_img_emb = nullptr, *g_img_att = nullptr,
                                 *g_img = nullptr;
@@ -865,34 +910,16 @@
                                                           float* __restrict__ d_img, const int* __restrict__ d_tab, int d_n,
                                                           int dimg_blocks, int z_device) {
   if ((int)blockIdx.x >= (int)gridDim.x - img_blocks) {
-    gen_images_block(enc_w, dec_w, emb_w, att_w, img, (int)blockIdx.x - ((int)gridDim.x - img_blocks));
+    gen_images_block(enc_w, dec_w, emb_w, att_w, img, (int)blockIdx.x - ((int)gridDim.x - img_blocks), true);
     return;
   }
   if ((int)blockIdx.x >= (int)gridDim.x - img_blocks - dimg_blocks) {
     disc_images_scatter(d_w, d_img, d_tab, d_n, (int)blockIdx.x - ((int)gridDim.x - img_blocks - dimg_blocks), dimg_blocks);
     return;
   }
-  const unsigned long long* ptrs = reinterpret_cast<const unsigned long long*>(slot);
-  const float* obsv = reinterpret_cast<const float*>(ptrs[0]);
-  const float* pred = reinterpret_cast<const float*>(ptrs[1]);
-  const int gid = blockIdx.x * 256 + threadIdx.x, gsz = ((int)gridDim.x - img_blocks - dimg_blocks) * 256;
-  if (z_dst) {
-    const float* zs = z_device ? reinterpret_cast<const float*>(ptrs[4]) : slot + 8;
-    for (int i = gid; i < B * SW_Z / 4; i += gsz) st4(z_dst + 4 * (size_t)i, ld4(zs + 4 * (size_t)i));
-  }
-  if (gid < 2) targets_dst[gid] = slot[4 + gid];
-  if (steps_dst && gid <= n_d_updates) steps_dst[gid] = gid < n_d_updates ? slot[6] + 1.0f + (float)gid : slot[7] + 1.0f;
-  for (int i = gid; i < B * To; i += gsz)
-    *reinterpret_cast<float2*>(obsv_dst + 2 * (size_t)i) = *reinterpret_cast<const float2*>(obsv + 2 * (size_t)i);
-  for (int k = gid; k < B * Tp; k += gsz) {
-    const int b = k / Tp, t = k - b * Tp;
-    const float2 p = *reinterpret_cast<const float2*>(pred + 2 * (size_t)k);
-    const float2 q = *reinterpret_cast<const float2*>(t == 0 ? obsv + ((size_t)b * To + To - 1) * 2 : pred + 2 * (size_t)k - 2);
-    *reinterpret_cast<float2*>(pred_dst + 2 * (size_t)k) = p;
-    st4(pred4_dst + 4 * (size_t)k, f32x4{p.x, p.y, p.x - q.x, p.y - q.y});
-  }
-}
-#define SW_DIMG_BLOCKS 16
+  stage_inputs_block(slot, B, To, Tp, obsv_dst, pred_dst, pred4_dst, targets_dst, z_dst, steps_dst, n_d_updates, z_device,
+                     (int)blockIdx.x, (int)gridDim.x - img_blocks - dimg_blocks);
+}
 extern "C" int sw_stage_step_zdev(const float* slot, int B, int To, int Tp, float* obsv_dst, float* pred_dst,
                                   float* pred4_dst, float* targets_dst, float* z_dst, float* steps_dst, int n_d_updates,
                                   const float* enc_w, const float* dec_w, const float* emb_w, const float* att_w, float* img,
diff --git a/socialways_amd/ops.py b/socialways_amd/ops.py
--- a/socialways_amd/ops.py
+++ b/socialways_amd/ops.py
@@ -114,8 +114,13 @@
     return _check_obs_len_tensor(obs_len, B, device)
 
 
-def _enc_save(obsv, enc_w, B, To, hT, cT, gsave, x4s_ptr, obs_len, aux, st):
-    if obs_len is None:
+def _enc_save(obsv, enc_w, B, To, hT, cT, gsave, x4s_ptr, obs_len, aux, st, stale_img=None):
+    if stale_img is not None:
+        if obs_len is not None or gsave is None:
+            raise ValueError("stale_img: the dense training launch only")
+        L.call("sw_enc_lstm_fwd_aux_img", L.ptr(obsv), 0, L.ptr(enc_w), None, None, B, To, L.ptr(hT), L.ptr(cT), None,
+               L.ptr(gsave), x4s_ptr, 0, aux[0], aux[1], aux[2], L.ptr(stale_img[0]), L.ptr(stale_img[1]), st)
+    elif obs_len is None:
         L.call("sw_enc_lstm_fwd_aux", L.ptr(obsv), 0, L.ptr(enc_w), None, None, B, To, L.ptr(hT), L.ptr(cT), None,
                L.ptr(gsave), x4s_ptr, 0, aux[0], aux[1], aux[2], st)
     elif gsave is None:
@@ -126,7 +131,7 @@
 
 
 def gen_forward(enc_w, emb_w, att_w, dec_w, obsv, noise, scenes, n_next, use_social, save, ws=None, tag="g", ade=None,
-                noise_src=None, d_obs=None, obs_len=None):
+                noise_src=None, d_obs=None, stale_img=None, obs_len=None):
     obs_len = _ragged_arg(obs_len, obsv.shape[0], obsv.device, noise_src, d_obs)
     L.require_gpu(obsv)
     obsv = obsv.contiguous()
@@ -146,7 +151,8 @@
     x4s_off = (To + n_next - 1) * B * 384
     z_in_enc, z_in_soc, n_enc = noise_src, None, noise.numel() if noise_src else 0
     _enc_save(obsv, enc_w, B, To, hT, cT, gsave, (gsave.data_ptr() + 4 * x4s_off) if save else None, obs_len,
-              (z_in_enc, L.ptr(noise) if z_in_enc else None, n_enc), st)
+              (z_in_enc, L.ptr(noise) if z_in_enc else None, n_enc), st,
+              stale_img=(dec_w, stale_img) if stale_img is not None else None)
     attn = wh = ml = None
     if use_social:
         S = torch.empty(B, 64, device=dev)
@@ -172,11 +178,24 @@
     return pred4, ctx
 
 
+class StepTail:
+    __slots__ = ("gimg", "dimg", "stage")
+
+    def __init__(self, gimg=None, dimg=None, stage=None):
+        self.gimg, self.dimg, self.stage = gimg, dimg, stage
+
+    def args(self):
+        g = self.gimg or (None,) * 3
+        d = self.dimg or (None,) * 3
+        s = self.stage or (None,) * 7 + (0, 0)
+        return ([L.ptr(t) for t in g] + [L.ptr(t) for t in d] + [s[0]] + [L.ptr(t) for t in s[1:7]] + [int(s[7]), int(s[8])])
+
+
 DFUSE = True
 
 
 def gen_backward(enc_w, emb_w, att_w, dec_w, ctx, dpred4, d_enc, d_emb, d_att, d_dec, ws=None, tag="g", aux=None, adam=None,
-                 dfuse=None):
+                 dfuse=None, tail=None):
     dev = ctx.obsv.device
     ws = ws or default_ws(dev)
     B, To, Tp = ctx.B, ctx.To, ctx.Tp
@@ -217,9 +236,10 @@
            L.ptr(aux_late[2]) if aux_late else None, aux_late[1].numel() if aux_late else 0, L.stream())
     if adam is not None:
         w_all, g_all, m, v, step, lr, b1, b2, eps = adam
-        L.call("sw_gen_wgrad_adam", L.ptr(enc_w), L.ptr(dec_w), L.ptr(ctx.gsave), L.ptr(gdelta), L.ptr(ctx.noise), L.ptr(ctx.S),
+        L.call("sw_gen_wgrad_adam_tail" if tail is not None else "sw_gen_wgrad_adam",
+               L.ptr(enc_w), L.ptr(dec_w), L.ptr(ctx.gsave), L.ptr(gdelta), L.ptr(ctx.noise), L.ptr(ctx.S),
                B, To, Tp, L.ptr(d_enc), L.ptr(d_dec), L.ptr(wgrad), L.ptr(tmp), pending, L.ptr(w_all), L.ptr(m), L.ptr(v),
-               L.ptr(g_all), w_all.numel(), L.ptr(step), lr, b1, b2, eps, L.stream())
+               L.ptr(g_all), w_all.numel(), L.ptr(step), lr, b1, b2, eps, *(tail.args() if tail is not None else ()), L.stream())
         return
     L.call("sw_gen_wgrad", L.ptr(enc_w), L.ptr(dec_w), L.ptr(ctx.gsave), L.ptr(gdelta), L.ptr(ctx.noise), L.ptr(ctx.S), B, To, Tp,
            L.ptr(d_enc), L.ptr(d_dec), 0, L.ptr(wgrad), L.ptr(tmp), pending, L.stream())
diff --git a/socialways_amd/trainer.py b/socialways_amd/trainer.py
--- a/socialways_amd/trainer.py
+++ b/socialways_amd/trainer.py
@@ -249,6 +249,8 @@
         self._lin_mask = None
         self._lin_maskf = None
         self._noise_src = None
+        self._stage_next = None
+        self._stale_img = False
 
     @property
     def use_social(self):
@@ -435,6 +437,19 @@
         parts = self._step_graph(batches, sub_batches, float(ss), Bg)
         return parts if out is False else [q.sum(1, dtype=torch.float64) for q in parts]
 
+    def _fuse_d(self):
+        return (self._fuse_d_adam and isinstance(self.D_optimizer, PackedAdam) and self.D_optimizer.fusable
+                and not (self.world > 1 or self._force_dist))
+
+    def _fuse_g(self, scenes):
+        return (self._fuse_g_adam and self._gimg is not None and isinstance(self.predictor_optimizer, PackedAdam)
+                and self.predictor_optimizer.fusable and not (self.world > 1 or self._force_dist)
+                and (not self.G.use_social or scenes.P > 0 or scenes.NB > 0))
+
+    def _stage_ahead(self, scenes, B, K):
+        return (K > 1 and self._fuse_d() and self._fuse_g(scenes) and self._dimg is not None
+                and (B + 15) // 16 <= ops.D_OBS_MAX_TILES and os.environ.get("SW_ENC8", "1") != "0")
+
     def _step_graph(self, batches, sub_batches, ss, Bg):
         K = len(batches)
         B, To, Tp = batches[0][0].shape[0], batches[0][0].shape[1], self.n_next
@@ -446,10 +461,11 @@
         HDR = 8
         if st is None:
             st = self._graphs[key] = dict(
-                n=0, graph=None, flip=0, scenes=scenes, obsv=torch.empty(B, To, 2, device=dev),
-                pred=torch.empty(B, Tp, 2, device=dev), pred4=torch.empty(B, Tp, 4, device=dev),
-                targets=torch.empty(4, device=dev), noise=torch.zeros(B, self.Z_COLS, device=dev),
-                steps=torch.zeros(self.n_unrolling_steps + 2, device=dev),
+                n=0, graph=None, flip=0, scenes=scenes, ahead=self._stage_ahead(scenes, B, K),
+                sets=[dict(obsv=torch.empty(B, To, 2, device=dev), pred=torch.empty(B, Tp, 2, device=dev),
+                           pred4=torch.empty(B, Tp, 4, device=dev), targets=torch.empty(4, device=dev),
+                           noise=torch.zeros(B, self.Z_COLS, device=dev),
+                           steps=torch.zeros(self.n_unrolling_steps + 2, device=dev)) for _ in range(2)],
                 outs=[torch.zeros(self.n_unrolling_steps + 3, (B + 15) // 16, 3, device=dev) for _ in range(K)],
                 slots=[[torch.zeros(HDR + B * self.Z_COLS, dtype=torch.float32).pin_memory() for _ in range(K)]
                        for _ in range(2)],
@@ -475,20 +491,34 @@
             np.copyto(hn[HDR:].reshape(B, self.Z_COLS)[:, :self.noise_len], (noise.cpu() if noise.is_cuda else noise).numpy())
         st["keep"][k] = keep
 
-        def stage(kk, j):
-            slot = st["slots"][kk][j]
-            L.call("sw_stage_step_zdev", slot.data_ptr(), B, To, Tp, L.ptr(st["obsv"]), L.ptr(st["pred"]),
-                   L.ptr(st["pred4"]), L.ptr(st["targets"]), L.ptr(st["noise"]) if zdev else None, L.ptr(st["steps"]),
-                   self.n_unrolling_steps + 1,
-                   L.ptr(self.G.encoder._flat), L.ptr(self.G.decoder._flat), L.ptr(self.G.feature_embedder._flat),
-                   L.ptr(self.G.attention._flat), L.ptr(self._gimg),
-                   L.ptr(self.D._flat) if self._dimg is not None else None, L.ptr(self._dimg), L.ptr(self._dtab), int(zdev),
-                   L.stream())
+        ahead = st["ahead"]
+        G, D = self.G, self.D
+
+        def bufs(j):
+            return st["sets"][j & 1 if ahead else 0]
+
+        def stage(kk, j, eager=False):
+            slot, s = st["slots"][kk][j], bufs(j)
+            images = (L.ptr(G.encoder._flat), L.ptr(G.decoder._flat), L.ptr(G.feature_embedder._flat), L.ptr(G.attention._flat),
+                      L.ptr(self._gimg), L.ptr(D._flat) if self._dimg is not None else None, L.ptr(self._dimg), L.ptr(self._dtab))
+            self._stale_img = bool(ahead and j >= 1 and not eager)
+            if self._stale_img:
+                L.call("sw_images_register", *images, Tp)
+            else:
+                L.call("sw_stage_step_zdev", slot.data_ptr(), B, To, Tp, L.ptr(s["obsv"]), L.ptr(s["pred"]),
+                       L.ptr(s["pred4"]), L.ptr(s["targets"]), L.ptr(s["noise"]) if zdev else None, L.ptr(s["steps"]),
+                       self.n_unrolling_steps + 1, *images, int(zdev), L.stream())
             self._noise_src = None if zdev else slot.data_ptr() + 4 * HDR
+            self._stage_next = None
+            if ahead and j + 1 < K and not eager:
+                n = bufs(j + 1)
+                self._stage_next = (st["slots"][kk][j + 1].data_ptr(), n["obsv"], n["pred"], n["pred4"], n["targets"],
+                                    n["noise"] if zdev else None, n["steps"], self.n_unrolling_steps + 1, int(zdev))
 
         def args(j):
-            return (st["obsv"], st["pred"], st["pred4"], scenes, st["targets"], st["noise"], ss, Bg, st["outs"][j],
-                    st["steps"] if packed else None)
+            s = bufs(j)
+            return (s["obsv"], s["pred"], s["pred4"], scenes, s["targets"], s["noise"], ss, Bg, st["outs"][j],
+                    s["steps"] if packed else None)
 
         def body(kk):
             for j in range(K):
@@ -502,7 +532,7 @@
         elif st["n"] < 2:
             st["n"] += 1
             for j in range(K):
-                stage(0, j)
+                stage(0, j, eager=True)
                 self._step_impl(*args(j))
         else:
             torch.cuda.synchronize()
@@ -576,6 +606,8 @@
         g_label = 1.0 / Bg
         g_code = (self.loss_info_w if self.use_info_loss else 0.0) / (2.0 * Bg)
         noise_src, self._noise_src = self._noise_src, None
+        stage_next, self._stage_next = self._stage_next, None
+        stale_img, self._stale_img = self._stale_img, False
         ol = getattr(self, "_obs_len", None)
         if pred4 is None:
             pred4 = torch.empty(B, Tp, 4, device=dev)
@@ -596,14 +628,13 @@
             pred_hat, gctx = ops.gen_forward(enc._flat, emb._flat, att._flat, dec._flat, obsv, noise, scenes, Tp,
                                              G.use_social, save=True, ws=ws, ade=(pred, 1.0 / float(ss), out[U + 2]),
                                              noise_src=noise_src, d_obs=(D._flat, d_pre) if d_pre is not None else None,
-                                             obs_len=ol)
+                                             obs_len=ol, stale_img=self._gimg if stale_img else None)
         d_gflat = D.grad_views()
         backup = None
         for u in range(self.n_unrolling_steps + 1):
             if u == 1:
                 backup = ws.get("d_backup", D._flat.numel())
-            fuse = (self._fuse_d_adam and isinstance(self.D_optimizer, PackedAdam) and self.D_optimizer.fusable
-                    and not (self.world > 1 or self._force_dist))
+            fuse = self._fuse_d()
             adam = self.D_optimizer.fused_args(None if steps is None else steps[u]) if fuse else None
             if ol is None and obsv.shape[2] == 2 and ops.disc_update_supported(D._flat, B, obsv.shape[1], Tp):
                 ops.disc_update(D._flat, obsv, [pred_hat, pred4], targets, (0, 1), noise, g_label, g_code, d_gflat, ws,
@@ -655,9 +686,13 @@
                 self._lin_maskf = D.linear_mask().float().contiguous()
             restore = (backup[:D._flat.numel()], D._flat, self._lin_maskf)
         G.grad_views()
-        fuse = (KV == 1 and self._fuse_g_adam and self._gimg is not None and isinstance(self.predictor_optimizer, PackedAdam)
-                and self.predictor_optimizer.fusable and not (self.world > 1 or self._force_dist)
-                and (not G.use_social or gctx.scenes.P > 0 or gctx.scenes.NB > 0))
+        fuse = KV == 1 and self._fuse_g(gctx.scenes)
+        if stage_next is not None and not fuse:
+            raise L.SocialWaysHipError("a sub-step without a staging launch needs the fused generator update in front of it")
+        tail = None
+        if fuse:
+            tail = ops.StepTail(gimg=(emb._flat, att._flat, self._gimg),
+                                dimg=(D._flat, self._dimg, self._dtab) if self._dimg is not None else None, stage=stage_next)
         adam = None
         if fuse:
             opt = self.predictor_optimizer
@@ -667,7 +702,7 @@
                                dec._gflat, ws=ws, aux=restore)
         else:
             ops.gen_backward(enc._flat, emb._flat, att._flat, dec._flat, gctx, dpred, enc._gflat, emb._gflat, att._gflat,
-                             dec._gflat, ws=ws, aux=restore, tag="g", adam=adam, dfuse=dfuse)
+                             dec._gflat, ws=ws, aux=restore, tag="g", adam=adam, dfuse=dfuse, tail=tail)
         if self._exchange_adam(self.predictor_optimizer, G._gflat_all):
             self._direct.adam(G._gflat_all, self.predictor_optimizer, None if steps is None else steps[U + 1])
         else:
```

Result: no change. 2809 steps/s (median of 4 runs) (+0.3%).
